# amathislab/HOISDF

Hardware: AMD Instinct MI355X
Metric: samples/sec (img + 2048 SDF queries) fwd+bwd at 1/2/4/8 MI355X (higher is better)
Workload: dtype f32 (emulated contractions, f32 accumulate, f16x2 form: operands as scaled hi + lo f16 pieces x 3 products - 22 operand bits, one power-of-two scale per ROW of a linear layer's row operand, per (sample, head) of the attention operands, per weight matrix; the attention backward's dS as three pieces x

## Files before the change

hoisdf_amd/_lib.py:

```python
from __future__ import annotations

import ctypes as C
import os
from typing import Dict, List

_HERE = os.path.dirname(os.path.abspath(__file__))
LIB_PATH = os.environ.get("HOISDF_LIB", os.path.join(_HERE, "libhoisdf_hip.so"))
HEADER_PATH = os.path.join(os.path.dirname(_HERE), "include", "hoisdf.h")
MAX_LEVELS = 8


class HoisdfLibraryError(RuntimeError):
    pass


class HoisdfError(RuntimeError):
    def __init__(self, code: int, msg: str):
        super().__init__(f"libhoisdf_hip status {code}: {msg}")
        self.code = code


class Pyramid(C.Structure):
    _fields_ = [("n_levels", C.c_int), ("B", C.c_int), ("data", C.c_void_p * MAX_LEVELS),
                ("C", C.c_int * MAX_LEVELS), ("H", C.c_int * MAX_LEVELS), ("W", C.c_int * MAX_LEVELS)]
# ... 56 lines not shown
class Mlp(C.Structure):
    _fields_ = [("n_layers", C.c_int), ("act_last", C.c_int), ("dims", C.c_int * (MLP_MAX_LAYERS + 1)),
                ("w", C.c_void_p * MLP_MAX_LAYERS), ("b", C.c_void_p * MLP_MAX_LAYERS),
                ("img", C.c_void_p * MLP_MAX_LAYERS), ("img_t", C.c_void_p * MLP_MAX_LAYERS)]


class EmuPrepItem(C.Structure):
    _fields_ = [("W", C.c_void_p), ("image", C.c_void_p), ("first_block", C.c_long), ("ldw", C.c_int), ("N", C.c_int),
                ("K", C.c_int), ("transpose", C.c_int)]


class MlpGrads(C.Structure):
    _fields_ = [("dw", C.c_void_p * MLP_MAX_LAYERS), ("db", C.c_void_p * MLP_MAX_LAYERS)]


POSE_MAX_LAYERS = 12


class PoseDesc(C.Structure):
    _fields_ = [("B", C.c_int), ("num_samp_hand", C.c_int), ("num_samp_obj", C.c_int), ("bins_n", C.c_int), ("img_h", C.c_int),
                ("img_w", C.c_int), ("hand_sdf_scale", C.c_float), ("obj_sdf_scale", C.c_float), ("clamping_distance", C.c_float),
                ("hidden_dim", C.c_int), ("nheads", C.c_int), ("dim_feedforward", C.c_int), ("enc_layers", C.c_int),
                ("dec_layers", C.c_int), ("C", C.c_int), ("use_inverse_kinematics", C.c_int), ("pre_norm", C.c_int),
                ("classifier_branch", C.c_int), ("attention", C.c_int)]


class SdfDecoderParams(C.Structure):
    _fields_ = [("weight_v", C.c_void_p * 4), ("weight_g", C.c_void_p * 4), ("bias", C.c_void_p * 4),
                ("linh4_weight", C.c_void_p), ("linh4_bias", C.c_void_p)]


class PoseWeights(C.Structure):
    _fields_ = [("linear_sdfin", Mlp), ("hand_sdf_decoder", SdfDecoderParams), ("obj_sdf_decoder", SdfDecoderParams),
                ("linear_transformerin", Mlp), ("hand_sigmoid_beta", C.c_void_p), ("obj_sigmoid_beta", C.c_void_p),
                ("hand_encoder", EncoderLayerWeights * POSE_MAX_LAYERS), ("obj_encoder", EncoderLayerWeights * POSE_MAX_LAYERS),
                ("hand_decoder", DecoderLayerWeights * POSE_MAX_LAYERS), ("mano_query_embed", C.c_void_p),
                ("linear_pose", Mlp), ("linear_shape", Mlp), ("linear_handvote", Mlp), ("linear_handcls", Mlp),
                ("linear_obj_rot", Mlp), ("linear_obj_rel_trans", Mlp),
                ("mano_shapedirs", C.c_void_p), ("mano_posedirs", C.c_void_p), ("mano_weights", C.c_void_p),
                ("mano_v_template", C.c_void_p), ("mano_j_regressor", C.c_void_p), ("mano_hands_mean", C.c_void_p)]


class EncoderDesc(C.Structure):
    _fields_ = [("B", C.c_int), ("img_h", C.c_int), ("img_w", C.c_int), ("resnet_type", C.c_int), ("big_decoder", C.c_int)]


_POSE_OUT = ("hand_joints_out", "obj_rot_out", "obj_trans_out", "mano_mesh_out", "mano_joints_out", "mano_shape_out",
             "hand_points_out", "obj_points_out", "hand_sdf_out", "obj_sdf_out")


class PoseOutputs(C.Structure):
    _fields_ = [(n, C.c_void_p) for n in _POSE_OUT]


_P, _I, _L, _F, _U64, _D = C.c_void_p, C.c_int, C.c_long, C.c_float, C.c_uint64, C.c_double
_PYR = C.POINTER(Pyramid)
_SDFW = C.POINTER(SdfWeights)

SIGNATURES: Dict[str, List] = {
    "hoisdf_project_gather_fwd": [_PYR, _P, _P, _L, _I, _P, _P, _F, _I, _I, _P, _I, _P, _P, _P],
    "hoisdf_project_gather_bwd": [_PYR, _P, _P, _L, _I, _P, _P, _F, _I, _I, _P, _I, _P],
    "hoisdf_linear_fwd": [_P, _I, _P, _I, _P, _P, _I, _L, _I, _I, _I, _F, _U64, _P, _P],
    "hoisdf_linear_bwd_input": [_P, _I, _P, _F, _P, _I, _P, _I, _L, _I, _I, _I, _P],
    "hoisdf_linear_bwd_weight": [_P, _I, _P, _F, _P, _I, _P, _I, _P, _L, _I, _I, _P, _L, _P],
    "hoisdf_linear_emu_prepare": [_P, _I, _I, _I, _I, _P, _P],
    "hoisdf_linear_emu_prepare_batch": [_P, _I, _L, _P],
    "hoisdf_linear_fwd_emu": [_P, _I, _P, _P, _P, _I, _L, _I, _I, _I, _F, _U64, _P, _P],
    "hoisdf_mag_measure": [_P, _L, _L, _I, _P, _P],
    "hoisdf_head_mag_measure": [_P, _L, _L, _I, _I, _P, _P],
    "hoisdf_linear_fwd_emu_heads": [_P, _I, _P, _P, _P, _I, _L, _I, _I, _P, _P, _P, _I, _P],
    "hoisdf_linear_bwd_input_emu_heads": [_P, _I, _P, _P, _I, _L, _I, _I, _P, _P, _P, _I, _P],
    "hoisdf_linear_fwd_emu_mag": [_P, _I, _P, _P, _P, _I, _L, _I, _I, _I, _F, _U64, _P, _P, _P, _P],
    "hoisdf_linear_bwd_input_emu": [_P, _I, _P, _F, _P, _P, _I, _L, _I, _I, _I, _P],
    "hoisdf_linear_bwd_input_emu_mag": [_P, _I, _P, _F, _P, _P, _I, _L, _I, _I, _I, _P, _P, _P],
    "hoisdf_linear_fwd_emu_small": [_P, _I, _P, _I, _P, _P, _I, _L, _I, _I, _I, _F, _U64, _P, _P],
    "hoisdf_linear_bwd_input_emu_small": [_P, _I, _P, _F, _P, _I, _P, _I, _L, _I, _I, _I, _P],
    "hoisdf_linear_bwd_weight_emu_small": [_P, _I, _P, _F, _P, _I, _P, _I, _P, _L, _I, _I, _P],
    "hoisdf_linear_bwd_weight_emu": [_P, _I, _P, _F, _P, _I, _P, _I, _P, _L, _I, _I, _P, _L, _P],
    "hoisdf_linear_bwd_weight_emu_mag": [_P, _I, _P, _F, _P, _I, _P, _I, _P, _L, _I, _I, _P, _L, _P, _P, _P],
    "hoisdf_relu_dropout_bwd": [_P, _I, _P, _I, _P, _I, _L, _I, _F, _P],
    "hoisdf_posenc_fwd": [_P, _L, _P, _I, _I, _P, _P],
    "hoisdf_sdf_query_fwd": [_PYR, _P, _P, _L, _I, _P, _P, _F, _I, _I, _P, _P, _SDFW, _F, _F, _U64, _P, _P, _P, _P, _P, _L, _P],
    "hoisdf_weightnorm_fwd": [_P, _P, _P, _I, _P, _I, _I, _P],
    "hoisdf_weightnorm_bwd": [_P, _P, _P, _I, _P, _P, _I, _I, _P],
    "hoisdf_sdf_head_fwd": [_P, _I, _P, _P, _P, _P, _L, _I, _F, _P],
    "hoisdf_sdf_head_bwd": [_P, _P, _P, _I, _P, _P, _I, _P, _P, _L, _I, _F, _P],
    "hoisdf_lattice_count": [_P, _P, _P, _F, _I, _I, _P, _P],
    "hoisdf_lattice_fill": [_P, _P, _P, _F, _I, _I, _P, _P, _P, _P, _P],
    "hoisdf_select_smallest_abs": [_P, _P, _P, _I, _I, _P, _P],
    "hoisdf_gather_rows": [_P, _I, _P, _L, _I, _P, _I, _P],
    "hoisdf_sdf_sample_keys": [_P, _I, _P, _P, _P, _P, _I, _I, _F, _U64, _P, _P, _P],
    "hoisdf_adamw_step": [_P, _I, _D, _D, _D, _D, _D, _L, _F, _P],
    "hoisdf_aux_image_losses_fwd": [_P, _L, _L, _L, _L, _P, _P, _P, _I, _I, _I, _I, _F, _P, _P, _P, _P, _P],
    "hoisdf_aux_image_losses_bwd": [_P, _L, _L, _L, _L, _P, _P, _P, _P, _P, _P, _I, _I, _I, _P, _P],
    "hoisdf_bn_stats": [_P, _L, _L, _I, _P, _P, _P, _P, _F, _F, _P, _L, _P],
    "hoisdf_bn_apply_fwd": [_P, _L, _P, _L, _P, _P, _I, _F, _P, _P, _I, _P, _P, _L, _I, _P],
    "hoisdf_bn_bwd": [_P, _L, _P, _L, _P, _P, _P, _P, _P, _P, _P, _P, _L, _I, _P, _L, _P],
    "hoisdf_token_build_fwd": [_P, _P, _P, _P, _I, _P, _P, _P, _I, _I, _I, _I, _I, _P],
    "hoisdf_token_build_bwd": [_P, _P, _I, _P, _P, _P, _I, _P, _I, _I, _I, _I, _I, _P],
    "hoisdf_token_build_bwd_ordered": [_P, _P, _I, _P, _P, _P, _I, _P, _P, _I, _I, _I, _I, _I, _P],
    "hoisdf_attention_fwd": [_P, _I, _P, _I, _P, _I, _P, _I, _P, _I, _I, _I, _I, _I, _F, _U64, _P],
    "hoisdf_attention_bwd": [_P, _I, _P, _I, _P, _I, _P, _I, _P, _I, _P, _P, _P, _P, _P, _I, _I, _I, _I,
                             _I, _F, _U64, _P],
    "hoisdf_attention_fwd_bf16x2": [_P, _I, _P, _I, _P, _I, _P, _I, _I, _I, _I, _I, _I, _P, _L, _P],
    "hoisdf_attention_fwd_emu": [_P, _I, _P, _I, _P, _I, _P, _I, _P, _I, _I, _I, _I, _I, _F, _U64, _P, _L, _I, _P],
    "hoisdf_attention_fwd_emu_mag": [_P, _I, _P, _I, _P, _I, _P, _I, _P, _I, _I, _I, _I, _I, _F, _U64, _P, _L, _I, _P, _P, _P, _P, _P],
    "hoisdf_attention_bwd_emu": [_P, _I, _P, _I, _P, _I, _P, _I, _P, _I, _P, _P, _P, _P, _P, _I, _I, _I, _I, _I, _F, _U64, _P, _P,
                                 _L, _P],
    "hoisdf_attention_bwd_emu_mag": [_P, _I, _P, _I, _P, _I, _P, _I, _P, _I, _P, _P, _P, _P, _P, _I, _I, _I, _I, _I, _F, _U64, _P, _P,
                                 _L, _P, _P, _P, _P, _P, _P],
    "hoisdf_attention_small_fwd": [_P, _I, _P, _I, _P, _I, _P, _P, _I, _P, _I, _I, _I, _I, _F, _U64, _P],
    "hoisdf_attention_small_bwd": [_P, _I, _P, _I, _P, _I, _P, _P, _I, _P, _P, _P, _I, _I, _I, _I, _F,
                                   _U64, _P],
    "hoisdf_add_layernorm_fwd": [_P, _P, _P, _P, _P, _P, _P, _L, _I, _F, _F, _U64, _P],
    "hoisdf_add_layernorm_bwd": [_P, _P, _P, _P, _P, _P, _P, _P, _P, _P, _P, _L, _I, _F, _U64, _P],
    "hoisdf_residual_dropout": [_P, _P, _P, _L, _I, _F, _U64, _P],
    "hoisdf_layernorm_rows_fwd": [_P, _P, _P, _P, _P, _P, _L, _I, _I, _I, _F, _P],
    "hoisdf_layernorm_rows_bwd": [_P, _P, _P, _P, _P, _P, _P, _P, _P, _L, _I, _I, _I, _P],
    "hoisdf_sdf_query_train_fwd": [_PYR, _P, _P, _L, _I, _P, _P, _F, _I, _I, _SDFW, _F, _F, _U64, _P, _P, _P, _P, _L, _P, _L, _P],
    "hoisdf_sdf_query_bwd": [_PYR, _P, _P, _L, _I, _P, _P, _F, _I, _I, _SDFW, _F, _F, _P, _L, _P, _P, _P, _L, _P],
    "hoisdf_sdf_infer_count": [_P, _P, _P, _F, _I, _I, _P, _P, _P, _P],
    "hoisdf_sdf_infer_count_begin": [_P, _P, _P, _F, _I, _I, _P, _P, _P],
    "hoisdf_sdf_infer": [_PYR, _P, _P, _P, _F, _I, _I, _P, _P, _I, _I, _I, _SDFW, _F, _F, _U64, _P, _P, _P, _P, _L, _P],
    "hoisdf_decoder_layer_fwd": [_P, _P, _P, _P, _P, _P, _P, _P, _P, _L, _P, _L, _P],
    "hoisdf_decoder_layer_bwd": [_P, _P, _P, _P, _P, _P, _P, _L, _P, _P, _P, _P, _I, _P, _P, _P, _L, _P],
    "hoisdf_encoder_layer_fwd": [_P, _P, _P, _P, _P, _P, _L, _P, _L, _P],
    "hoisdf_encoder_layer_bwd": [_P, _P, _P, _P, _P, _L, _P, _P, _P, _P, _P, _L, _P],
    "hoisdf_mano_prepare": [_P, _P, _P, _P, _P],
    "hoisdf_mano_head_fwd": [_P, _I, _I, _P, _I, _I, _P, _P, _P, _P, _P, _P, _P, _P, _P, _I, _I, _P, _P, _P, _P, _P],
    "hoisdf_mano_head_bwd": [_P, _P, _I, _P, _P, _P, _P, _P, _P, _P, _P, _P, _I, _I, _P, _P, _P, _P, _P, _P, _P],
    "hoisdf_vote_fwd": [_P, _P, _P, _P, _P, _I, _I, _I, _I, _P],
    "hoisdf_vote_bwd": [_P, _P, _P, _P, _P, _P, _P, _P, _I, _I, _I, _I, _P],
    "hoisdf_vote_loss_fwd": [_P, _P, _P, _P, _F, _P, _P, _P, _P, _P, _I, _I, _I, _I, _P],
    "hoisdf_vote_loss_bwd": [_P, _P, _P, _P, _F, _P, _P, _P, _P, _P, _P, _P, _I, _I, _I, _I, _P],
    "hoisdf_tokens_fwd": [_P, _P, _P, _P, _F, _I, _I, _P, _P, _P, _P, _P, _P, _P, _P, _P, _I, _I, _I, _I, _I, _P, _L, _P, _L, _P],
    "hoisdf_tokens_bwd": [_P, _P, _P, _P, _F, _I, _I, _P, _P, _P, _P, _P, _P, _L, _P, _P, _I, _P, _I, _I, _I, _I, _I, _P, _L, _P],
    "hoisdf_heads_vote_fwd": [_P, _P, _P, _P, _P, _F, _P, _P, _P, _P, _I, _I, _I, _I, _P, _L, _P, _L, _P],
    "hoisdf_heads_vote_bwd": [_P, _P, _P, _P, _P, _F, _P, _P, _L, _P, _P, _P, _P, _P, _P, _I, _I, _I, _I, _P, _L, _P],
    "hoisdf_point_loss_fwd": [_P, _P, _L, _L, _I, _L, _I, _F, _F, _F, _P, _P, _P],
    "hoisdf_point_loss_bwd": [_P, _P, _L, _L, _I, _L, _I, _F, _F, _F, _P, _P, _P],
    "hoisdf_pose_prepare": [_P, _P, _P, _L, _P],
    "hoisdf_pose_infer_begin": [_P, _P, _P, _P, _P, _P, _P, _P, _P],
    "hoisdf_pose_infer": [_P, _P, _PYR, _P, _P, _P, _P, _P, _P, _P, _P, _P, _L, _P, _P],
    "hoisdf_conv_pack_weight": [_P, _P, _P, _P, _P, _P, _F, _I, _I, _I, _I, _I, _P, _P, _P],
    "hoisdf_conv_plan": [_L, _I, _I, _I, _P, _P],
    "hoisdf_conv2d_fwd": [_P, _I, _P, _P, _P, _I, _P, _I, _I, _I, _I, _I, _I, _I, _I, _I, _I, _I, _I, _P, _L, _P],
    "hoisdf_conv_transpose2d_fwd": [_P, _I, _P, _P, _P, _I, _I, _I, _I, _I, _I, _I, _I, _P, _L, _P],
    "hoisdf_maxpool2d_fwd": [_P, _I, _P, _I, _I, _I, _I, _I, _P],
    "hoisdf_encoder_prepare": [_P, _P, _I, _P, _L, _P],
    "hoisdf_encoder_pyramid_shape": [_P, _PYR],
    "hoisdf_encoder_infer": [_P, _P, _P, _P, _P, _P, _L, _P],
}
_RET = {"hoisdf_version": C.c_char_p, "hoisdf_last_error": C.c_char_p}
_OTHER = {"hoisdf_set_deterministic": ([_I], None), "hoisdf_set_gemm_emu": ([_I], None), "hoisdf_get_gemm_emu": ([], C.c_int), "hoisdf_get_deterministic": ([], C.c_int),
          "hoisdf_mano_dirs_image_floats": ([], C.c_long),
          "hoisdf_point_loss_blocks": ([_L], C.c_int),
          "hoisdf_bn_workspace_floats": ([_L, _I], C.c_long),
          "hoisdf_token_build_bwd_partials": ([], C.c_int),
          "hoisdf_tokens_saved_bytes": ([_P, _L, _I], C.c_long),
          "hoisdf_tokens_workspace_bytes": ([_P, _L, _I], C.c_long),
          "hoisdf_heads_vote_saved_bytes": ([_P, _P, _I, _I, _I, _I], C.c_long),
          "hoisdf_heads_vote_workspace_bytes": ([_P, _P, _I, _I, _I, _I, _I], C.c_long),
          "hoisdf_sdf_infer_workspace": ([_L, _I, _I], C.c_long),
          "hoisdf_sdf_query_train_saved_bytes": ([_L, _I], C.c_long),
          "hoisdf_sdf_query_train_workspace_bytes": ([_L, _I, _I], C.c_long),
          "hoisdf_decoder_layer_saved_bytes": ([_P], C.c_long),
          "hoisdf_decoder_layer_workspace_bytes": ([_P, _I], C.c_long),
          "hoisdf_encoder_layer_saved_bytes": ([_P], C.c_long),
          "hoisdf_encoder_layer_out_mag": ([_P, _P], C.c_void_p),
          "hoisdf_encoder_layer_workspace_bytes": ([_P, _I], C.c_long),
          "hoisdf_sdf_query_workspace": ([_L, _I, _I], C.c_long),
          "hoisdf_linear_bwd_weight_workspace": ([_L, _I, _I], C.c_long),
          "hoisdf_linear_emu_image_bytes": ([_I, _I], C.c_long),
          "hoisdf_linear_emu_prepare_blocks": ([_I, _I, _I], C.c_long),
          "hoisdf_linear_bwd_weight_emu_workspace": ([_L, _I, _I], C.c_long),
          "hoisdf_linear_emu_supported": ([_P, _L, _I], C.c_int),
          "hoisdf_linear_emu_small_max_rows": ([], C.c_int),
          "hoisdf_linear_emu_pieces": ([], C.c_int),
          "hoisdf_mag_words": ([_L], C.c_long),
          "hoisdf_head_mag_words": ([_L, _I, _I], C.c_long),
          "hoisdf_linear_emu_small_supported": ([_P, _L, _P, _L, _L, _I, _I], C.c_int),
          "hoisdf_attention_bf16x2_workspace": ([_I, _I, _I, _I], C.c_long),
          "hoisdf_attention_emu_workspace": ([_I, _I, _I, _I, _I], C.c_long),
          "hoisdf_attention_bwd_emu_workspace": ([_I, _I, _I, _I, _I], C.c_long),
          "hoisdf_conv_packed_floats": ([_I, _I, _I, _I], C.c_long),
          "hoisdf_conv_workspace_bytes": ([_L, _I, _I, _I], C.c_long),
          "hoisdf_encoder_tensor_count": ([_P], C.c_int),
          "hoisdf_encoder_tensor_name": ([_P, _I], C.c_char_p),
          "hoisdf_encoder_tensor_numel": ([_P, _I], C.c_long),
          "hoisdf_encoder_prepared_bytes": ([_P], C.c_long),
          "hoisdf_encoder_infer_workspace": ([_P], C.c_long),
          "hoisdf_encoder_launch_count": ([_P], C.c_int),
          "hoisdf_pose_prepared_bytes": ([_P], C.c_long),
          "hoisdf_pose_infer_workspace": ([_P, _P], C.c_long)}

_lib = None


def lib() -> C.CDLL:
    global _lib
    if _lib is None:
        if not os.path.exists(LIB_PATH):
            raise HoisdfLibraryError(
                f"{LIB_PATH} not found: the HIP extension is not built (make -C hoisdf_amd/csrc). "
                "There is no CPU fallback for the hot path.")
        L = C.CDLL(LIB_PATH)
        for name, args in SIGNATURES.items():
            fn = getattr(L, name)
            fn.argtypes = args
            fn.restype = C.c_int
        for name, ret in _RET.items():
            fn = getattr(L, name)
            fn.argtypes = []
            fn.restype = ret
        for name, (args, ret) in _OTHER.items():
            fn = getattr(L, name)
            fn.argtypes = args
            fn.restype = ret
        _lib = L
    return _lib


_timer = None


def set_timer(timer) -> None:
    global _timer
    _timer = timer


def call(name: str, *args) -> None:
    t = _timer
    timed = t is not None and name in t.names
    if timed:
        t.begin(name, args)
    rc = getattr(lib(), name)(*args)
    if timed:
        t.end(name)
    if rc != 0:
        raise HoisdfError(rc, lib().hoisdf_last_error().decode())


def exported_symbols() -> List[str]:
    return list(SIGNATURES) + list(_RET) + list(_OTHER)
```

hoisdf_amd/csrc/attention_emu.h:

```cpp
#pragma once
#include "common.h"

namespace hoisdf {
namespace emu_attn {

struct EmuAttn {
  const __bf16 *q[3];
  const __bf16 *k[3];
  const __bf16 *v[3], *vt[3];
  const __bf16 *d[3];
  const float* lse_in; const float* delta;
  float* out; float* lse; float* dq_part; float* dk; float* dv;
  int ldo, ldk, ldv;
  int B, H, Lq, Lk, Lqp, Lkp, kv_len;
  float drop_p, inv_keep;
  uint32_t thresh;
  uint64_t seed;
  const uint32_t *q_hm, *k_hm, *v_hm, *d_hm;
  float* dq_scale;
  uint32_t* mag;
};

__device__ __forceinline__ bool emu_block(int nx, int nbh, int& tile, int& bh) {
  const int L = blockIdx.x, slot = L >> 3;
  bh = (slot / nx) * 8 + (L & 7);
  tile = slot % nx;
  return bh < nbh;
}

}

int attention_bwd4_emu_launch(const emu_attn::EmuAttn& a, hipStream_t st);
int attention_bwd4h_emu_launch(const emu_attn::EmuAttn& a, hipStream_t st);
}
```

hoisdf_amd/csrc/attention_emu.hip:

```cpp
#include <stdlib.h>

#include "attention_emu.h"

namespace hoisdf {
using emu_attn::EmuAttn;
using emu_attn::emu_block;

namespace {
typedef float f32x16 __attribute__((ext_vector_type(16)));
typedef float f32x4 __attribute__((ext_vector_type(4)));
typedef __bf16 bf16x8 __attribute__((ext_vector_type(8)));
typedef __bf16 bf16x4 __attribute__((ext_vector_type(4)));
typedef unsigned int u32x4 __attribute__((ext_vector_type(4)));
typedef unsigned int u32x2 __attribute__((ext_vector_type(2)));

constexpr int D = 64;
constexpr int RP = 72;
constexpr int TPH = 36;
constexpr int ROWS_T = 32 * RP;
constexpr int TRN_T = 64 * TPH;
constexpr float QS2 = 0.125f * 1.4426950408889634f;
#define CR(r, h) (((r) & 3) + 8 * ((r) >> 2) + 4 * (h))
#define MB(a, b, c) __builtin_amdgcn_mfma_f32_32x32x16_bf16((a), (b), (c), 0, 0, 0)
#define MB6(acc, x0, x1, x2, y0, y1, y2) \
  do {                                   \
    acc = MB(x2, y0, acc);               \
    acc = MB(x0, y2, acc);               \
    acc = MB(x1, y1, acc);               \
    acc = MB(x1, y0, acc);               \
    acc = MB(x0, y1, acc);               \
    acc = MB(x0, y0, acc);               \
  } while (0)

#define SPLIT1(x, i)                             \
  do {                                           \
    const __bf16 a_ = (__bf16)(x);               \
    const float r1_ = (x) - (float)a_;           \
    const __bf16 b_ = (__bf16)r1_;               \
    const float r2_ = r1_ - (float)b_;           \
    p0[i] = a_; p1[i] = b_; p2[i] = (__bf16)r2_; \
  } while (0)

__device__ __forceinline__ u32x4 ld_rows(const __bf16* base, size_t row0, int tid) {
  return *reinterpret_cast<const u32x4*>(base + (row0 + (tid >> 3)) * D + (tid & 7) * 8);
}
__device__ __forceinline__ void st_rows(__bf16* lds, const u32x4 v, int tid) {
  *reinterpret_cast<u32x4*>(lds + (tid >> 3) * RP + (tid & 7) * 8) = v;
}
__device__ __forceinline__ u32x4 ld_trn(const __bf16* base, size_t Lp, size_t col0, int tid) {
  return *reinterpret_cast<const u32x4*>(base + (size_t)(tid >> 2) * Lp + col0 + (tid & 3) * 8);
}
__device__ __forceinline__ void st_trn(__bf16* lds, const u32x4 v, int tid) {
  u32x2* p = reinterpret_cast<u32x2*>(lds + (tid >> 2) * TPH + (tid & 3) * 8);
  p[0] = u32x2{v.x, v.y};
  p[1] = u32x2{v.z, v.w};
}
__device__ __forceinline__ bf16x8 frag_trn(const __bf16* tile, int row, int jj, int h) {
  const bf16x4 a = *reinterpret_cast<const bf16x4*>(tile + row * TPH + 16 * jj + 4 * h);
  const bf16x4 b = *reinterpret_cast<const bf16x4*>(tile + row * TPH + 16 * jj + 8 + 4 * h);
  return bf16x8{a[0], a[1], a[2], a[3], b[0], b[1], b[2], b[3]};
}
}

typedef _Float16 f16x8 __attribute__((ext_vector_type(8)));
typedef _Float16 f16x2 __attribute__((ext_vector_type(2)));
template <bool F16>
__global__ __launch_bounds__(256) void emu_attn_convert_kernel(const float* __restrict__ src, int ld, int L, int Lp, int B, int H,
                                                               float scale, __bf16* __restrict__ r0, __bf16* __restrict__ r1,
                                                               __bf16* __restrict__ r2, __bf16* __restrict__ t0,
                                                               __bf16* __restrict__ t1, __bf16* __restrict__ t2,
                                                               const uint32_t* __restrict__ mag) {
  constexpr int TP = 72;
  __shared__ __attribute__((aligned(16))) __bf16 tile[3][64 * TP];
  const int tid = threadIdx.x;
  const int nb = Lp / 64;
  const int kb = blockIdx.x % nb, bh = blockIdx.x / nb, b = bh / H, head = bh - b * H;
  if (F16) { f16_saturate_on(); scale *= mag_scale(mag[head * B + b]); }
  const int r = tid >> 2, dc = (tid & 3) * 16;
  const int row = kb * 64 + r;
  const bool valid = row < L;
  const float* sr = src + ((size_t)b * L + (valid ? row : 0)) * ld + head * D + dc;
  bf16x8 pa[2][3];
#pragma unroll
  for (int i = 0; i < 2; ++i) {
    float4 u = valid ? *reinterpret_cast<const float4*>(sr + 8 * i) : make_float4(0.f, 0.f, 0.f, 0.f);
    float4 w = valid ? *reinterpret_cast<const float4*>(sr + 8 * i + 4) : make_float4(0.f, 0.f, 0.f, 0.f);
    u.x *= scale; u.y *= scale; u.z *= scale; u.w *= scale;
    w.x *= scale; w.y *= scale; w.z *= scale; w.w *= scale;
    if (F16) {
      const float e_[8] = {u.x, u.y, u.z, u.w, w.x, w.y, w.z, w.w};
      f16x8 hi, lo;
#pragma unroll
      for (int j = 0; j < 8; ++j) { hi[j] = (_Float16)e_[j]; lo[j] = (_Float16)(e_[j] - (float)hi[j]); }
      pa[i][0] = __builtin_bit_cast(bf16x8, hi); pa[i][1] = __builtin_bit_cast(bf16x8, lo); pa[i][2] = pa[i][1];
    } else {
      bf16x8 p0, p1, p2;
      SPLIT1(u.x, 0); SPLIT1(u.y, 1); SPLIT1(u.z, 2); SPLIT1(u.w, 3);
      SPLIT1(w.x, 4); SPLIT1(w.y, 5); SPLIT1(w.z, 6); SPLIT1(w.w, 7);
      pa[i][0] = p0; pa[i][1] = p1; pa[i][2] = p2;
    }
  }
  if (r0) {
    const size_t o = ((size_t)bh * Lp + row) * D + dc;
#pragma unroll
    for (int i = 0; i < 2; ++i) {
      *reinterpret_cast<bf16x8*>(r0 + o + 8 * i) = pa[i][0];
      *reinterpret_cast<bf16x8*>(r1 + o + 8 * i) = pa[i][1];
      if (!F16 && r2) *reinterpret_cast<bf16x8*>(r2 + o + 8 * i) = pa[i][2];
    }
  }
  if (t0) {
#pragma unroll
    for (int i = 0; i < 2; ++i)
#pragma unroll
      for (int e = 0; e < 8; ++e) {
        tile[0][(dc + 8 * i + e) * TP + r] = pa[i][0][e];
        tile[1][(dc + 8 * i + e) * TP + r] = pa[i][1][e];
        if (!F16) tile[2][(dc + 8 * i + e) * TP + r] = pa[i][2][e];
      }
    __syncthreads();
    const int d = tid >> 2, rc = (tid & 3) * 16;
    const size_t o = ((size_t)bh * D + d) * Lp + kb * 64 + rc;
#pragma unroll
    for (int i = 0; i < 2; ++i) {
      *reinterpret_cast<u32x4*>(t0 + o + 8 * i) = *reinterpret_cast<const u32x4*>(&tile[0][d * TP + rc + 8 * i]);
      *reinterpret_cast<u32x4*>(t1 + o + 8 * i) = *reinterpret_cast<const u32x4*>(&tile[1][d * TP + rc + 8 * i]);
      if (!F16 && t2) *reinterpret_cast<u32x4*>(t2 + o + 8 * i) = *reinterpret_cast<const u32x4*>(&tile[2][d * TP + rc + 8 * i]);
    }
  }
}

typedef float f32x2 __attribute__((ext_vector_type(2)));
typedef __bf16 bf16x2 __attribute__((ext_vector_type(2)));
template <bool DROP, int NPL, bool F16>
__global__ __launch_bounds__(256, 2) void emu_attn_fwd2_kernel(EmuAttn a) {
  static_assert(!F16 || NPL == 2, "the f16 form has two planes");
  __shared__ __attribute__((aligned(16))) __bf16 Kb0[3 * ROWS_T];
  __shared__ __attribute__((aligned(16))) __bf16 Kb1[3 * ROWS_T];
  __shared__ __attribute__((aligned(16))) __bf16 Vb0[3 * TRN_T];
  __shared__ __attribute__((aligned(16))) __bf16 Vb1[3 * TRN_T];
  const int tid = threadIdx.x, lane = tid & 63, wave = tid >> 6;
  const int h = lane >> 5, c = lane & 31;
  int qtile, bh;
  if (!emu_block((a.Lq + 127) / 128, a.B * a.H, qtile, bh)) return;
  const int b = bh / a.H, head = bh - b * a.H;
  const int qrow = qtile * 128 + wave * 32 + c;
  const __bf16* kp[3] = {a.k[0] + (size_t)bh * a.Lkp * D, a.k[1] + (size_t)bh * a.Lkp * D, a.k[NPL == 3 ? 2 : 1] + (size_t)bh * a.Lkp * D};
  const __bf16* vp[3] = {a.vt[0] + (size_t)bh * D * a.Lkp, a.vt[1] + (size_t)bh * D * a.Lkp, a.vt[NPL == 3 ? 2 : 1] + (size_t)bh * D * a.Lkp};
  float cs = 1.f, vinv = 1.f;
  constexpr float PB = F16 ? 6.f : 0.f;
  if (F16) {
    f16_saturate_on();
    const float iq_ = mag_inv_scale(a.q_hm[head * a.B + b]), ik_ = mag_inv_scale(a.k_hm[head * a.B + b]);
    cs = fmaxf(iq_ * ik_, 0x1p-100f); vinv = mag_inv_scale(a.v_hm[head * a.B + b]);
  }
  const float thr8 = F16 ? 8.f / cs : 8.f;
  float mneg = INFINITY;

  bf16x8 qf[4][3];
#pragma unroll
  for (int p = 0; p < NPL; ++p) {
    const __bf16* sq = a.q[p] + ((size_t)bh * a.Lqp + qrow) * D;
#pragma unroll
    for (int j = 0; j < 4; ++j) qf[j][p] = *reinterpret_cast<const bf16x8*>(sq + 16 * j + 8 * h);
  }
  const uint32_t rowkey = drop_rowkey(a.seed, (uint32_t)(bh * a.Lq + qrow));
  const uint32_t dthr = a.thresh & 0xffff0000u;
  float m = -INFINITY, lsum = 0.f, ps = 0.f;
  f32x16 o[2], s_cur, s_nxt;
  float dsc[16];
#pragma unroll
  for (int t = 0; t < 2; ++t)
#pragma unroll
    for (int r = 0; r < 16; ++r) o[t][r] = 0.f;
#pragma unroll
  for (int r = 0; r < 16; ++r) dsc[r] = 1.f;
  const int ntiles = (a.kv_len + 31) / 32;
  const int lastt = ntiles - 1;
  u32x4 rk[3], rv[3];
  bf16x8 kf[2][3], vf[2][3], pw[2][3];
  uint32_t w0[8], w1[8], w2[8], hx[8];
  f32x2 e_[8], f_[8];
  float mt = -INFINITY;
#define KFRAG(KB, p, j) (*reinterpret_cast<const bf16x8*>(&(KB)[(p) * ROWS_T + c * RP + 16 * (j) + 8 * h]))
#define VFRAG(VB, p, dt, jj) frag_trn((VB) + (p) * TRN_T, (dt) * 32 + c, jj, h)
#define SB() __builtin_amdgcn_sched_barrier(0)
#define PK_SUB(d, x, y) asm("v_pk_add_f32 %0, %1, %2 neg_lo:[0,1] neg_hi:[0,1]" : "=v"(d) : "v"(x), "v"(y))
#define PE1(pr)                                                                                                        \
  do {                                                                                                                 \
    if constexpr (F16) e_[pr] = f32x2{__builtin_amdgcn_exp2f(__builtin_fmaf(s_cur[2 * (pr)], cs, mneg)),               \
                                     __builtin_amdgcn_exp2f(__builtin_fmaf(s_cur[2 * (pr) + 1], cs, mneg))};           \
    else e_[pr] = f32x2{__builtin_amdgcn_exp2f(s_cur[2 * (pr)] - m), __builtin_amdgcn_exp2f(s_cur[2 * (pr) + 1] - m)}; \
  } while (0)
#define PE2(pr)                                                                                                        \
  do {                                                                                                                 \
    ps += e_[pr].x + e_[pr].y;                                                                                         \
    if (DROP) e_[pr] = f32x2{e_[pr].x * dsc[2 * (pr)], e_[pr].y * dsc[2 * (pr) + 1]};                                   \
    if constexpr (F16) {                                                                                               \
      const f16x2 hh_ = __builtin_convertvector(e_[pr], f16x2);                                                        \
      w0[pr] = __builtin_bit_cast(uint32_t, hh_);                                                                      \
      f_[pr] = __builtin_convertvector(hh_, f32x2);                                                                    \
    } else {                                                                                                           \
      const uint32_t h_ = __builtin_bit_cast(uint32_t, __builtin_convertvector(e_[pr], bf16x2));                       \
      w0[pr] = h_;                                                                                                     \
      f_[pr] = f32x2{__builtin_bit_cast(float, h_ << 16), __builtin_bit_cast(float, h_ & 0xffff0000u)};                \
    }                                                                                                                  \
  } while (0)
#define PE3(pr)                                                                                                        \
  do {                                                                                                                 \
    PK_SUB(e_[pr], e_[pr], f_[pr]);                                                                                    \
    const uint32_t h_ = __builtin_bit_cast(uint32_t, __builtin_convertvector(e_[pr], bf16x2));                         \
    w1[pr] = h_;                                                                                                       \
    f_[pr] = f32x2{__builtin_bit_cast(float, h_ << 16), __builtin_bit_cast(float, h_ & 0xffff0000u)};                  \
  } while (0)
#define PE4(pr)                                                                                                        \
  do {                                                                                                                 \
    f32x2 r_; PK_SUB(r_, e_[pr], f_[pr]);                                                                              \
    w2[pr] = __builtin_bit_cast(uint32_t, __builtin_convertvector(r_, bf16x2));                                        \
    if (((pr) & 3) == 3) {                                      \
      pw[(pr) >> 2][0] = __builtin_bit_cast(bf16x8, u32x4{w0[(pr) - 3], w0[(pr) - 2], w0[(pr) - 1], w0[pr]});          \
      pw[(pr) >> 2][1] = __builtin_bit_cast(bf16x8, u32x4{w1[(pr) - 3], w1[(pr) - 2], w1[(pr) - 1], w1[pr]});          \
      pw[(pr) >> 2][2] = __builtin_bit_cast(bf16x8, u32x4{w2[(pr) - 3], w2[(pr) - 2], w2[(pr) - 1], w2[pr]});          \
    }                                                                                                                  \
  } while (0)
#define PE3B(pr)                                                                                                       \
  do {                                                                                                                 \
    f32x2 r_; PK_SUB(r_, e_[pr], f_[pr]);                                                                              \
    if constexpr (F16) w1[pr] = __builtin_bit_cast(uint32_t, __builtin_convertvector(r_, f16x2));                      \
    else w1[pr] = __builtin_bit_cast(uint32_t, __builtin_convertvector(r_, bf16x2));                                   \
    if (((pr) & 3) == 3) {                                                                                             \
      pw[(pr) >> 2][0] = __builtin_bit_cast(bf16x8, u32x4{w0[(pr) - 3], w0[(pr) - 2], w0[(pr) - 1], w0[pr]});          \
      pw[(pr) >> 2][1] = __builtin_bit_cast(bf16x8, u32x4{w1[(pr) - 3], w1[(pr) - 2], w1[(pr) - 1], w1[pr]});          \
    }                                                                                                                  \
  } while (0)
#define PM(i)                                                                                                          \
  do {                                                                                                                 \
    float t_;                                                                                                          \
    asm volatile("v_max3_f32 %0, %1, %2, %3" : "=v"(t_) : "v"(s_nxt[4 * (i)]), "v"(s_nxt[4 * (i) + 1]), "v"(s_nxt[4 * (i) + 2])); \
    asm volatile("v_max3_f32 %0, %0, %1, %2" : "+v"(mt) : "v"(t_), "v"(s_nxt[4 * (i) + 3]));                           \
  } while (0)
#define PH1(pr) do { if (DROP) { uint32_t x_ = hbase + (uint32_t)(CR(2 * (pr), 0) >> 1) * 0x9E3779B9U; x_ ^= x_ >> 15; hx[pr] = x_ * 0x2C1B3C6DU; asm volatile("" : "+v"(hx[pr])); } } while (0)
#define PH2(pr) do { if (DROP) { hx[pr] ^= hx[pr] >> 12; asm volatile("" : "+v"(hx[pr])); } } while (0)
#define PH3(pr) do { if (DROP) { dsc[2 * (pr)] = (hx[pr] << 16) >= dthr ? a.inv_keep : 0.f; dsc[2 * (pr) + 1] = hx[pr] >= dthr ? a.inv_keep : 0.f; asm volatile("" : "+v"(dsc[2 * (pr)]), "+v"(dsc[2 * (pr) + 1])); } } while (0)
#define STK(p) st_rows(kw + (p) * ROWS_T, rk[p], tid)
#define STV(p) st_trn(vw + (p) * TRN_T, rv[p], tid)
#define LDK(p) rk[p] = ld_rows(kp[p], (size_t)ktn * 32, tid)
#define LDV(p) rv[p] = ld_trn(vp[p], a.Lkp, (size_t)vtn * 32, tid)
#ifndef FWD2_ABL
#define FWD2_ABL 0
#endif
#if FWD2_ABL & 1
#undef PE1
#undef PE2
#undef PE3
#undef PE4
#undef PE3B
#undef PM
#undef PH1
#undef PH2
#undef PH3
#define PE1(pr) ((void)0)
#define PE2(pr) ((void)0)
#define PE3(pr) ((void)0)
#define PE4(pr) ((void)0)
#define PE3B(pr) ((void)0)
#define PM(i) ((void)0)
#define PH1(pr) ((void)0)
#define PH2(pr) ((void)0)
#define PH3(pr) ((void)0)
#endif
#if FWD2_ABL & 8
#undef PE1
#define PE1(pr) do { e_[pr] = f32x2{s_cur[2 * (pr)], s_cur[2 * (pr) + 1]}; } while (0)
#endif
#if FWD2_ABL & 16
#undef PE2
#undef PE3
#undef PE4
#define PE2(pr) do { ps += e_[pr].x + e_[pr].y; w0[pr] = __builtin_bit_cast(uint32_t, e_[pr].x); } while (0)
#define PE3(pr) do { w1[pr] = __builtin_bit_cast(uint32_t, e_[pr].y); } while (0)
#define PE4(pr)                                                                                                        \
  do {                                                                                                                 \
    w2[pr] = w0[pr] ^ w1[pr];                                                                                          \
    if (((pr) & 3) == 3) {                                                                                             \
      pw[(pr) >> 2][0] = __builtin_bit_cast(bf16x8, u32x4{w0[(pr) - 3], w0[(pr) - 2], w0[(pr) - 1], w0[pr]});          \
      pw[(pr) >> 2][1] = __builtin_bit_cast(bf16x8, u32x4{w1[(pr) - 3], w1[(pr) - 2], w1[(pr) - 1], w1[pr]});          \
      pw[(pr) >> 2][2] = __builtin_bit_cast(bf16x8, u32x4{w2[(pr) - 3], w2[(pr) - 2], w2[(pr) - 1], w2[pr]});          \
    }                                                                                                                  \
  } while (0)
#endif
#if FWD2_ABL & 32
#undef PM
#define PM(i) ((void)0)
#endif
#if FWD2_ABL & 2
#undef STK
#undef STV
#undef LDK
#undef LDV
#define STK(p) ((void)0)
#define STV(p) ((void)0)
#define LDK(p) ((void)0)
#define LDV(p) ((void)0)
#endif
#if FWD2_ABL & 4
#define FWD2_SYNC() ((void)0)
#else
#define FWD2_SYNC() __syncthreads()
#endif
#pragma push_macro("MB")
#undef MB
#define MB(a_, b_, c_)                                                                                                             \
  (F16 ? __builtin_amdgcn_mfma_f32_32x32x16_f16(__builtin_bit_cast(f16x8, (a_)), __builtin_bit_cast(f16x8, (b_)), (c_), 0, 0, 0) \
       : __builtin_amdgcn_mfma_f32_32x32x16_bf16((a_), (b_), (c_), 0, 0, 0))
#include "attn_fwd2_phase.inc"

#pragma unroll
  for (int p = 0; p < NPL; ++p) { rk[p] = ld_rows(kp[p], 0, tid); rv[p] = ld_trn(vp[p], a.Lkp, 0, tid); }
#pragma unroll
  for (int p = 0; p < NPL; ++p) { st_rows(Kb0 + p * ROWS_T, rk[p], tid); st_trn(Vb0 + p * TRN_T, rv[p], tid); }
#pragma unroll
  for (int p = 0; p < NPL; ++p) rk[p] = ld_rows(kp[p], (size_t)min(1, lastt) * 32, tid);
#pragma unroll
  for (int p = 0; p < NPL; ++p) st_rows(Kb1 + p * ROWS_T, rk[p], tid);
#pragma unroll
  for (int p = 0; p < NPL; ++p) { rk[p] = ld_rows(kp[p], (size_t)min(2, lastt) * 32, tid); rv[p] = ld_trn(vp[p], a.Lkp, (size_t)min(1, lastt) * 32, tid); }
  __syncthreads();
#pragma unroll
  for (int r = 0; r < 16; ++r) s_nxt[r] = 0.f;
#pragma unroll
  for (int j = 0; j < 4; ++j) {
    const bf16x8 k0 = KFRAG(Kb0, 0, j), k1 = KFRAG(Kb0, 1, j);
    if constexpr (NPL == 3) {
      const bf16x8 k2 = KFRAG(Kb0, 2, j);
      MB6(s_nxt, k0, k1, k2, qf[j][0], qf[j][1], qf[j][2]);
    } else {
      s_nxt = MB(k1, qf[j][0], s_nxt); s_nxt = MB(k0, qf[j][1], s_nxt); s_nxt = MB(k0, qf[j][0], s_nxt);
    }
  }
  uint32_t hbase = rowkey + (uint32_t)(2 * h) * 0x9E3779B9U;
#define FWD2_TILE_STATS(KT, DO_HASH)                                                                                   \
  do {                                                                                                                 \
    if ((KT) == lastt) {                                                                                               \
      _Pragma("unroll") for (int r = 0; r < 16; ++r) if ((KT) * 32 + CR(r, h) >= a.kv_len) s_nxt[r] = -INFINITY;       \
      mt = -INFINITY;                                                                                                  \
      PM(0); PM(1); PM(2); PM(3);                                                                                      \
    }                                                                                                                  \
    mt = fmaxf(mt, __shfl_xor(mt, 32, 64));                                                                            \
    if (__any(mt > m + thr8)) {                                                                                        \
      const float mn = fmaxf(m, mt);                                                                                   \
      const float alpha = __builtin_amdgcn_exp2f(F16 ? (m - mn) * cs : m - mn);                                        \
      lsum *= alpha;                                                                                                   \
      m = mn;                                                                                                          \
      mneg = PB - m * cs;                                                                                              \
      _Pragma("unroll") for (int t_ = 0; t_ < 2; ++t_) _Pragma("unroll") for (int r = 0; r < 16; ++r) o[t_][r] *= alpha; \
    }                                                                                                                  \
    if (DO_HASH) { _Pragma("unroll") for (int pr = 0; pr < 8; ++pr) { PH1(pr); PH2(pr); PH3(pr); } }                    \
  } while (0)
#pragma unroll
  for (int r = 0; r < 16; ++r) mt = fmaxf(mt, s_nxt[r]);
  FWD2_TILE_STATS(0, true);
  s_cur = s_nxt;
  __syncthreads();
#define FWD2_ITER(t, KR, KW, VR, VW)                                                                                   \
  do {                                                                                                                 \
    __bf16* kw = (KW); __bf16* vw = (VW);                                                                              \
    const int ktn = min((t) + 3, lastt), vtn = min((t) + 2, lastt);                                                    \
    kf[0][0] = KFRAG(KR, 0, 0); kf[0][1] = KFRAG(KR, 1, 0); if constexpr (NPL == 3) kf[0][2] = KFRAG(KR, 2, 0);        \
    _Pragma("unroll") for (int r = 0; r < 16; ++r) s_nxt[r] = 0.f;                                                     \
    ps = 0.f;                                                                                                          \
    SB();                                                                                                              \
    if constexpr (NPL == 3) FWD2_S(KR); else FWD2_S2(KR);                                                              \
    lsum += ps;                                                                                                        \
    vf[0][0] = VFRAG(VR, 0, 0, 0); vf[0][1] = VFRAG(VR, 1, 0, 0); if constexpr (NPL == 3) vf[0][2] = VFRAG(VR, 2, 0, 0); \
    mt = -INFINITY;                                                                                                    \
    hbase += 16u * 0x9E3779B9U;                                                                                        \
    SB();                                                                                                              \
    if constexpr (NPL == 3) FWD2_PV(VR); else FWD2_PV2(VR);                                                            \
    if ((t) + 1 <= lastt) FWD2_TILE_STATS((t) + 1, false);                \
    s_cur = s_nxt;                                                                                                     \
    FWD2_SYNC();                                                                                                       \
  } while (0)
  int t = 0;
  for (; t + 1 < ntiles; t += 2) {
    FWD2_ITER(t, Kb1, Kb0, Vb0, Vb1);
    FWD2_ITER(t + 1, Kb0, Kb1, Vb1, Vb0);
  }
  if (t < ntiles) FWD2_ITER(t, Kb1, Kb0, Vb0, Vb1);
#undef KFRAG
#undef VFRAG
#undef SB
#undef PK_SUB
#undef PE1
#undef PE2
#undef PE3
#undef PE4
#undef PM
#undef PH1
#undef PH2
#undef PH3
#undef STK
#undef STV
#undef LDK
#undef LDV
#undef FWD2_S
#undef FWD2_PV
#undef FWD2_S2
#undef FWD2_PV2
#undef PE3B
#undef FWD2_TILE_STATS
#undef FWD2_ITER
  const float ltot = lsum + __shfl_xor(lsum, 32, 64);
  uint32_t omax = 0u;
  if (qrow < a.Lq) {
    const float inv = vinv / ltot;
    float* op = a.out + ((size_t)b * a.Lq + qrow) * a.ldo + head * D;
#pragma unroll
    for (int tt = 0; tt < 2; ++tt)
#pragma unroll
      for (int g = 0; g < 4; ++g) {
        const float4 ov = make_float4(o[tt][4 * g + 0] * inv, o[tt][4 * g + 1] * inv, o[tt][4 * g + 2] * inv, o[tt][4 * g + 3] * inv);
        *reinterpret_cast<float4*>(op + 32 * tt + 8 * g + 4 * h) = ov;
        omax = max(omax, mag_bits4(ov));
      }
    if (h == 0 && a.lse) a.lse[(size_t)bh * a.Lq + qrow] = (F16 ? m * cs - PB : m) + log2f(ltot);
  }
  if (a.mag) {
    omax = max(omax, (uint32_t)__shfl_xor((int)omax, 32, 64));
    if (h == 0 && qrow < a.Lq) atomicMax(a.mag + (size_t)b * a.Lq + qrow, omax);
  }
}
#pragma pop_macro("MB")

__global__ __launch_bounds__(256) void emu_attn_delta_kernel(const float* __restrict__ o, int ldo, const float* __restrict__ dout,
                                                             int lddo, float* __restrict__ delta, int B, int H, int Lq) {
  const long g = ((long)blockIdx.x * 256 + threadIdx.x) >> 4;
  const int l16 = threadIdx.x & 15;
  if (g >= (long)B * Lq * H) return;
  const int head = (int)(g % H);
  const long bq = g / H;
  const int q = (int)(bq % Lq), b = (int)(bq / Lq);
  const float4 x = *reinterpret_cast<const float4*>(o + ((size_t)b * Lq + q) * ldo + head * D + l16 * 4);
  const float4 y = *reinterpret_cast<const float4*>(dout + ((size_t)b * Lq + q) * lddo + head * D + l16 * 4);
  float s = x.x * y.x + x.y * y.y + x.z * y.z + x.w * y.w;
#pragma unroll
  for (int off = 8; off > 0; off >>= 1) s += __shfl_xor(s, off, 16);
  if (l16 == 0) delta[((size_t)b * H + head) * Lq + q] = s;
}

__global__ __launch_bounds__(256) void emu_attn_dq_reduce_kernel(const float* __restrict__ part, int nkb, float* __restrict__ dq,
                                                                 int ldq, int B, int H, int Lq, uint32_t* __restrict__ mag,
                                                                 const float* __restrict__ scale) {
  const long i = (long)(gridDim.x - 1 - blockIdx.x) * 256 + threadIdx.x;
  const long n = (long)B * H * Lq * 16;
  uint32_t qmax = 0u;
  if (i < n) {
    const int d4 = (int)(i & 15);
    const long bq = i >> 4;
    const int q = (int)(bq % Lq);
    const int bh = (int)(bq / Lq), b = bh / H, head = bh - b * H;
    const size_t stride = (size_t)B * H * Lq * D;
    const float* p = part + ((size_t)bh * Lq + q) * D + d4 * 4;
    float4 s = *reinterpret_cast<const float4*>(p);
    for (int k0 = 1; k0 < nkb; k0 += 8) {
      f32x4 v[8];
#pragma unroll
      for (int j = 0; j < 8; ++j)
        v[j] = k0 + j < nkb ? __builtin_nontemporal_load(reinterpret_cast<const f32x4*>(p + (size_t)(k0 + j) * stride)) : f32x4{0.f, 0.f, 0.f, 0.f};
#pragma unroll
      for (int j = 0; j < 8; ++j)
        if (k0 + j < nkb) { s.x += v[j].x; s.y += v[j].y; s.z += v[j].z; s.w += v[j].w; }
    }
    const float sc = scale ? scale[bh] : 0.125f;
    const float4 r = make_float4(s.x * sc, s.y * sc, s.z * sc, s.w * sc);
    *reinterpret_cast<float4*>(dq + ((size_t)b * Lq + q) * ldq + head * D + d4 * 4) = r;
    qmax = mag_bits4(r);
    if (mag) {
      qmax = group_max_u32<16>(qmax);
      if (d4 == 0) atomicMax(mag + (size_t)b * Lq + q, qmax);
    }
  }
}

}

using namespace hoisdf;

namespace {
inline long pad128(long L) { return (L + 127) / 128 * 128; }
inline size_t plane_elems(int B, int H, long Lp) { return (size_t)B * H * Lp * 64; }

struct Planes { __bf16 *r[3], *t[3]; };
inline Planes carve(__bf16*& w, size_t n, bool rows, bool trn) {
  Planes p{};
  for (int i = 0; i < 3; ++i) { p.r[i] = rows ? w : nullptr; if (rows) w += n; }
  for (int i = 0; i < 3; ++i) { p.t[i] = trn ? w : nullptr; if (trn) w += n; }
  return p;
}
int convert(const float* src, int ld, int L, int Lp, int B, int H, float scale, const Planes& p, hipStream_t st, const uint32_t* mag = nullptr) {
  const long nblk = (long)B * H * (Lp / 64);
  if (mag) hipLaunchKernelGGL(emu_attn_convert_kernel<true>, dim3((unsigned)nblk), dim3(256), 0, st, src, ld, L, Lp, B, H, scale, p.r[0], p.r[1],
                              p.r[2], p.t[0], p.t[1], p.t[2], mag);
  else hipLaunchKernelGGL(emu_attn_convert_kernel<false>, dim3((unsigned)nblk), dim3(256), 0, st, src, ld, L, Lp, B, H, scale, p.r[0], p.r[1],
                          p.r[2], p.t[0], p.t[1], p.t[2], mag);
  return check_launch("attention_emu_convert");
}
int check_emu(const void* q, const void* k, const void* v, int ldq, int ldk, int ldv, int B, int H, int Lq, int Lk, int kv_len,
              float drop_p, const char* who) {
  HOISDF_REQUIRE(q && k && v, HOISDF_ERR_INVALID, "%s: null pointer", who);
  HOISDF_REQUIRE(B > 0 && H > 0 && Lq > 0 && Lk > 0 && kv_len > 0 && kv_len <= Lk, HOISDF_ERR_INVALID,
                 "%s: bad sizes B=%d H=%d Lq=%d Lk=%d kv_len=%d", who, B, H, Lq, Lk, kv_len);
  HOISDF_REQUIRE(ldq >= H * 64 && ldk >= H * 64 && ldv >= H * 64 && ((ldq | ldk | ldv) & 3) == 0 &&
                     (((uintptr_t)q | (uintptr_t)k | (uintptr_t)v) & 15) == 0,
                 HOISDF_ERR_INVALID, "%s: leading dims must be multiples of 4 and >= H*64, pointers 16-byte aligned", who);
  HOISDF_REQUIRE(drop_p >= 0.f && drop_p < 1.f, HOISDF_ERR_INVALID, "%s: drop_p=%f", who, drop_p);
  return HOISDF_OK;
}
}

extern "C" long hoisdf_attention_emu_workspace(int B, int H, int Lq, int Lk, int mode) {
  if (B <= 0 || H <= 0 || Lq <= 0 || Lk <= 0) return 0;
  const size_t q = plane_elems(B, H, pad128(Lq)), k = plane_elems(B, H, pad128(Lk));
  const size_t planes = mode == 0 ? 3 * q + 6 * k : 3 * q + 9 * k;
  return (long)(planes * sizeof(__bf16));
}

namespace {
int fwd_over_planes(float* o, int ldo, float* lse, int B, int H, int Lq, int Lk, int kv_len, float drop_p, uint64_t seed,
                    void* workspace, int keep, hipStream_t st, uint32_t* o_mag, const uint32_t* q_hm = nullptr, const uint32_t* k_hm = nullptr,
                    const uint32_t* v_hm = nullptr) {
  const int Lqp = (int)pad128(Lq), Lkp = (int)pad128(Lk);
  __bf16* w = reinterpret_cast<__bf16*>(workspace);
  const size_t nq = plane_elems(B, H, Lqp), nk = plane_elems(B, H, Lkp);
  const Planes pq = carve(w, nq, true, false);
  const Planes pk = carve(w, nk, true, false);
  const Planes pv = carve(w, nk, keep != 0, true);
  EmuAttn a{};
  for (int i = 0; i < 3; ++i) { a.q[i] = pq.r[i]; a.k[i] = pk.r[i]; a.vt[i] = pv.t[i]; }
  a.out = o; a.lse = lse; a.ldo = ldo; a.mag = o_mag; a.q_hm = q_hm; a.k_hm = k_hm; a.v_hm = v_hm;
  a.B = B; a.H = H; a.Lq = Lq; a.Lk = Lk; a.Lqp = Lqp; a.Lkp = Lkp; a.kv_len = kv_len;
  a.drop_p = drop_p; a.inv_keep = 1.f / (1.f - drop_p); a.thresh = drop_threshold(drop_p); a.seed = seed;
  const dim3 fgrid(cdiv(Lq, 128) * 8 * cdiv(B * H, 8));
  if (q_hm) {
    HOISDF_REQUIRE(drop_p < 0.75f, HOISDF_ERR_INVALID, "attention_fwd_emu (f16x2 form): drop_p = %f, must be below 0.75", drop_p);
    if (drop_p > 0.f) hipLaunchKernelGGL((emu_attn_fwd2_kernel<true, 2, true>), fgrid, dim3(256), 0, st, a);
    else hipLaunchKernelGGL((emu_attn_fwd2_kernel<false, 2, true>), fgrid, dim3(256), 0, st, a);
  } else if (drop_p > 0.f) hipLaunchKernelGGL((emu_attn_fwd2_kernel<true, 3, false>), fgrid, dim3(256), 0, st, a);
  else hipLaunchKernelGGL((emu_attn_fwd2_kernel<false, 3, false>), fgrid, dim3(256), 0, st, a);
  return check_launch("attention_fwd_emu");
}
}

extern "C" int hoisdf_attention_fwd_emu(const float* q, int ldq, const float* k, int ldk, const float* v, int ldv, float* o,
                                        int ldo, float* lse, int B, int H, int Lq, int Lk, int kv_len, float drop_p,
                                        uint64_t seed, void* workspace, long workspace_bytes, int keep, void* stream) {
  return attention_fwd_emu_mag(q, ldq, k, ldk, v, ldv, o, ldo, lse, B, H, Lq, Lk, kv_len, drop_p, seed, workspace, workspace_bytes, keep,
                               nullptr, stream, nullptr, nullptr, nullptr);
}
extern "C" int hoisdf_attention_fwd_emu_mag(const float* q, int ldq, const float* k, int ldk, const float* v, int ldv, float* o,
                                            int ldo, float* lse, int B, int H, int Lq, int Lk, int kv_len, float drop_p,
                                            uint64_t seed, void* workspace, long workspace_bytes, int keep, const uint32_t* q_mag,
                                            const uint32_t* k_mag, const uint32_t* v_mag, uint32_t* o_mag, void* stream) {
  HOISDF_REQUIRE(q_mag && k_mag && v_mag, HOISDF_ERR_INVALID, "attention_fwd_emu_mag: the head magnitudes of q, k and v are required (hoisdf_head_mag_measure)");
  return attention_fwd_emu_mag(q, ldq, k, ldk, v, ldv, o, ldo, lse, B, H, Lq, Lk, kv_len, drop_p, seed, workspace, workspace_bytes, keep,
                               o_mag, stream, q_mag, k_mag, v_mag);
}
int hoisdf::attention_fwd_emu_mag(const float* q, int ldq, const float* k, int ldk, const float* v, int ldv, float* o, int ldo, float* lse,
                                  int B, int H, int Lq, int Lk, int kv_len, float drop_p, uint64_t seed, void* workspace,
                                  long workspace_bytes, int keep, uint32_t* o_mag, void* stream, const uint32_t* q_hm, const uint32_t* k_hm,
                                  const uint32_t* v_hm) {
  if (int rc = check_emu(q, k, v, ldq, ldk, ldv, B, H, Lq, Lk, kv_len, drop_p, "attention_fwd_emu")) return rc;
  HOISDF_REQUIRE(o && workspace && ldo >= H * 64 && (ldo & 3) == 0 && (((uintptr_t)o | (uintptr_t)workspace) & 15) == 0,
                 HOISDF_ERR_INVALID, "attention_fwd_emu: bad output / workspace");
  HOISDF_REQUIRE((!q_hm && !k_hm && !v_hm) || (q_hm && k_hm && v_hm), HOISDF_ERR_INVALID, "attention_fwd_emu: head magnitudes of all of q, k, v or of none");
  const long need = hoisdf_attention_emu_workspace(B, H, Lq, Lk, keep ? 2 : 0);
  HOISDF_REQUIRE(workspace_bytes >= need, HOISDF_ERR_WORKSPACE, "attention_fwd_emu: workspace %ld < %ld bytes", workspace_bytes, need);
  const int Lqp = (int)pad128(Lq), Lkp = (int)pad128(Lk);
  hipStream_t st = as_stream(stream);
  __bf16* w = reinterpret_cast<__bf16*>(workspace);
  const size_t nq = plane_elems(B, H, Lqp), nk = plane_elems(B, H, Lkp);
  const Planes pq = carve(w, nq, true, false);
  const Planes pk = carve(w, nk, true, false);
  const Planes pv = carve(w, nk, keep != 0, true);
  if (int rc = convert(q, ldq, Lq, Lqp, B, H, QS2, pq, st, q_hm)) return rc;
  if (int rc = convert(k, ldk, Lk, Lkp, B, H, 1.f, pk, st, k_hm)) return rc;
  if (int rc = convert(v, ldv, Lk, Lkp, B, H, 1.f, pv, st, v_hm)) return rc;
  return fwd_over_planes(o, ldo, lse, B, H, Lq, Lk, kv_len, drop_p, seed, workspace, keep, st, o_mag, q_hm, k_hm, v_hm);
}

extern "C" long hoisdf_attention_bf16x2_workspace(int B, int H, int Lq, int Lk) {
  if (B <= 0 || H <= 0 || Lq <= 0 || Lk <= 0) return 0;
  return (long)((2 * plane_elems(B, H, pad128(Lq)) + 4 * plane_elems(B, H, pad128(Lk))) * sizeof(__bf16));
}

extern "C" int hoisdf_attention_fwd_bf16x2(const float* q, int ldq, const float* k, int ldk, const float* v, int ldv, float* o, int ldo,
                                           int B, int H, int Lq, int Lk, int kv_len, void* workspace, long workspace_bytes, void* stream) {
  if (int rc = check_emu(q, k, v, ldq, ldk, ldv, B, H, Lq, Lk, kv_len, 0.f, "attention_fwd_bf16x2")) return rc;
  HOISDF_REQUIRE(o && workspace && ldo >= H * 64 && (ldo & 3) == 0 && (((uintptr_t)o | (uintptr_t)workspace) & 15) == 0,
                 HOISDF_ERR_INVALID, "attention_fwd_bf16x2: bad output / workspace");
  const long need = hoisdf_attention_bf16x2_workspace(B, H, Lq, Lk);
  HOISDF_REQUIRE(workspace_bytes >= need, HOISDF_ERR_WORKSPACE, "attention_fwd_bf16x2: workspace %ld < %ld bytes", workspace_bytes, need);
  const int Lqp = (int)pad128(Lq), Lkp = (int)pad128(Lk);
  hipStream_t st = as_stream(stream);
  __bf16* w = reinterpret_cast<__bf16*>(workspace);
  const size_t nq = plane_elems(B, H, Lqp), nk = plane_elems(B, H, Lkp);
  Planes pq{}, pk{}, pv{};
  pq.r[0] = w; pq.r[1] = w + nq; w += 2 * nq;
  pk.r[0] = w; pk.r[1] = w + nk; w += 2 * nk;
  pv.t[0] = w; pv.t[1] = w + nk;
  if (int rc = convert(q, ldq, Lq, Lqp, B, H, QS2, pq, st)) return rc;
  if (int rc = convert(k, ldk, Lk, Lkp, B, H, 1.f, pk, st)) return rc;
  if (int rc = convert(v, ldv, Lk, Lkp, B, H, 1.f, pv, st)) return rc;
  EmuAttn a{};
  for (int i = 0; i < 2; ++i) { a.q[i] = pq.r[i]; a.k[i] = pk.r[i]; a.vt[i] = pv.t[i]; }
  a.out = o; a.lse = nullptr; a.ldo = ldo;
  a.B = B; a.H = H; a.Lq = Lq; a.Lk = Lk; a.Lqp = Lqp; a.Lkp = Lkp; a.kv_len = kv_len;
  a.drop_p = 0.f; a.inv_keep = 1.f; a.thresh = 0; a.seed = 0;
  const dim3 fgrid(cdiv(Lq, 128) * 8 * cdiv(B * H, 8));
  hipLaunchKernelGGL((emu_attn_fwd2_kernel<false, 2, false>), fgrid, dim3(256), 0, st, a);
  return check_launch("attention_fwd_bf16x2");
}

void hoisdf::attention_emu_plane_targets(void* workspace, int B, int H, int Lq, int Lk, int keep, QkvPlanes& qp, QkvPlanes& kvp) {
  const int Lqp = (int)pad128(Lq), Lkp = (int)pad128(Lk);
  __bf16* w = reinterpret_cast<__bf16*>(workspace);
  const size_t nq = plane_elems(B, H, Lqp), nk = plane_elems(B, H, Lkp);
  const Planes pq = carve(w, nq, true, false);
  const Planes pk = carve(w, nk, true, false);
  const Planes pv = carve(w, nk, keep != 0, true);
  qp = QkvPlanes{}; kvp = QkvPlanes{};
  qp.on = kvp.on = 1; qp.H = kvp.H = H; qp.E = kvp.E = H * 64; qp.qscale = kvp.qscale = QS2;
  qp.L = Lq; qp.Lp = Lqp; kvp.L = Lk; kvp.Lp = Lkp;
  for (int i = 0; i < 3; ++i) {
    qp.r[0][i] = pq.r[i];
    kvp.r[1][i] = pk.r[i]; kvp.r[2][i] = pv.r[i]; kvp.vt[i] = pv.t[i];
    if (Lq == Lk) { kvp.r[0][i] = pq.r[i]; qp.r[1][i] = pk.r[i]; qp.r[2][i] = pv.r[i]; qp.vt[i] = pv.t[i]; }
  }
}

int hoisdf::attention_fwd_emu_planes(float* o, int ldo, float* lse, int B, int H, int Lq, int Lk, int kv_len, float drop_p,
                                     uint64_t seed, void* workspace, int keep, void* stream, uint32_t* o_mag) {
  HOISDF_REQUIRE(o && workspace && ldo >= H * 64 && (ldo & 3) == 0 && (((uintptr_t)o | (uintptr_t)workspace) & 15) == 0 && B > 0 &&
                     H > 0 && Lq > 0 && Lk > 0 && kv_len > 0 && kv_len <= Lk && drop_p >= 0.f && drop_p < 1.f,
                 HOISDF_ERR_INVALID, "attention_fwd_emu_planes: bad arguments");
  return fwd_over_planes(o, ldo, lse, B, H, Lq, Lk, kv_len, drop_p, seed, workspace, keep, as_stream(stream), o_mag);
}

extern "C" long hoisdf_attention_bwd_emu_workspace(int B, int H, int Lq, int Lk, int kept) {
  if (B <= 0 || H <= 0 || Lq <= 0 || Lk <= 0) return 0;
  const size_t q = plane_elems(B, H, pad128(Lq)), k = plane_elems(B, H, pad128(Lk));
  size_t bytes = 3 * q * sizeof(__bf16) + (size_t)cdiv(Lk, 128) * B * H * Lq * 64 * sizeof(float);
  if (!kept) bytes += (3 * q + 6 * k) * sizeof(__bf16);
  return (long)bytes;
}

extern "C" int hoisdf_attention_bwd_emu(const float* q, int ldq, const float* k, int ldk, const float* v, int ldv, const float* o,
                                        int ldo, const float* dout, int lddo, const float* lse, float* delta, float* dq, float* dk,
                                        float* dv, int B, int H, int Lq, int Lk, int kv_len, float drop_p, uint64_t seed,
                                        const void* fwd_workspace, void* workspace, long workspace_bytes, void* stream) {
  return attention_bwd_emu_mag(q, ldq, k, ldk, v, ldv, o, ldo, dout, lddo, lse, delta, dq, dk, dv, B, H, Lq, Lk, kv_len, drop_p, seed,
                               fwd_workspace, workspace, workspace_bytes, nullptr, stream, nullptr, nullptr, nullptr, nullptr);
}
extern "C" int hoisdf_attention_bwd_emu_mag(const float* q, int ldq, const float* k, int ldk, const float* v, int ldv, const float* o,
                                            int ldo, const float* dout, int lddo, const float* lse, float* delta, float* dq, float* dk,
                                            float* dv, int B, int H, int Lq, int Lk, int kv_len, float drop_p, uint64_t seed,
                                            const void* fwd_workspace, void* workspace, long workspace_bytes, const uint32_t* q_mag,
                                            const uint32_t* k_mag, const uint32_t* v_mag, const uint32_t* do_mag, uint32_t* g_mag, void* stream) {
  HOISDF_REQUIRE(q_mag && k_mag && v_mag && do_mag, HOISDF_ERR_INVALID, "attention_bwd_emu_mag: the head magnitudes of q, k, v and of dout are required");
  return attention_bwd_emu_mag(q, ldq, k, ldk, v, ldv, o, ldo, dout, lddo, lse, delta, dq, dk, dv, B, H, Lq, Lk, kv_len, drop_p, seed,
                               fwd_workspace, workspace, workspace_bytes, g_mag, stream, q_mag, k_mag, v_mag, do_mag);
}
int hoisdf::attention_bwd_emu_mag(const float* q, int ldq, const float* k, int ldk, const float* v, int ldv, const float* o, int ldo,
                                  const float* dout, int lddo, const float* lse, float* delta, float* dq, float* dk, float* dv, int B,
                                  int H, int Lq, int Lk, int kv_len, float drop_p, uint64_t seed, const void* fwd_workspace,
                                  void* workspace, long workspace_bytes, uint32_t* g_mag, void* stream, const uint32_t* q_hm,
                                  const uint32_t* k_hm, const uint32_t* v_hm, const uint32_t* do_hm) {
  const bool h2 = q_hm && k_hm && v_hm && do_hm;
  HOISDF_REQUIRE(h2 || (!q_hm && !k_hm && !v_hm && !do_hm), HOISDF_ERR_INVALID, "attention_bwd_emu: head magnitudes of all of q, k, v, dout or of none");
  HOISDF_REQUIRE(!g_mag || Lq == Lk, HOISDF_ERR_INVALID, "attention_bwd_emu: one row-magnitude array for dq, dk, dv needs Lq == Lk");
  HOISDF_REQUIRE(!h2 || drop_p < 0.75f, HOISDF_ERR_INVALID, "attention_bwd_emu (f16x2 form): drop_p = %f, must be below 0.75 (as in the forward)", drop_p);
  if (int rc = check_emu(fwd_workspace && !q ? o : q, fwd_workspace && !k ? o : k, fwd_workspace && !v ? o : v, ldq, ldk, ldv, B, H, Lq,
                         Lk, kv_len, drop_p, "attention_bwd_emu")) return rc;
  HOISDF_REQUIRE(o && dout && lse && delta && dq && dk && dv && workspace, HOISDF_ERR_INVALID, "attention_bwd_emu: null pointer");
  HOISDF_REQUIRE(ldo >= H * 64 && lddo >= H * 64 && ((ldo | lddo) & 3) == 0 &&
                     (((uintptr_t)o | (uintptr_t)dout | (uintptr_t)dq | (uintptr_t)dk | (uintptr_t)dv | (uintptr_t)workspace |
                       (uintptr_t)fwd_workspace) & 15) == 0,
                 HOISDF_ERR_INVALID, "attention_bwd_emu: bad leading dims / alignment");
  const long need = hoisdf_attention_bwd_emu_workspace(B, H, Lq, Lk, fwd_workspace ? 1 : 0);
  HOISDF_REQUIRE(workspace_bytes >= need, HOISDF_ERR_WORKSPACE, "attention_bwd_emu: workspace %ld < %ld bytes", workspace_bytes, need);
  const int Lqp = (int)pad128(Lq), Lkp = (int)pad128(Lk);
  hipStream_t st = as_stream(stream);
  const size_t nq = plane_elems(B, H, Lqp), nk = plane_elems(B, H, Lkp);
  __bf16* w = reinterpret_cast<__bf16*>(workspace);
  const Planes pd = carve(w, nq, true, false);
  float* part = reinterpret_cast<float*>(w);
  w += (size_t)cdiv(Lk, 128) * B * H * Lq * 64 * 2;
  Planes pq, pk, pv;
  if (fwd_workspace) {
    __bf16* f = reinterpret_cast<__bf16*>(const_cast<void*>(fwd_workspace));
    pq = carve(f, nq, true, false); pk = carve(f, nk, true, false); pv = carve(f, nk, true, true);
  } else {
    pq = carve(w, nq, true, false); pk = carve(w, nk, true, false); pv = carve(w, nk, true, false);
    if (int rc = convert(q, ldq, Lq, Lqp, B, H, QS2, pq, st, q_hm)) return rc;
    if (int rc = convert(k, ldk, Lk, Lkp, B, H, 1.f, pk, st, k_hm)) return rc;
    if (int rc = convert(v, ldv, Lk, Lkp, B, H, 1.f, pv, st, v_hm)) return rc;
  }
  if (int rc = convert(dout, lddo, Lq, Lqp, B, H, 1.f, pd, st, do_hm)) return rc;
  const long ng = (long)B * Lq * H;
  hipLaunchKernelGGL(emu_attn_delta_kernel, dim3((unsigned)((ng * 16 + 255) / 256)), dim3(256), 0, st, o, ldo, dout, lddo, delta, B, H, Lq);
  if (int rc = check_launch("attention_emu_delta")) return rc;
  EmuAttn a{};
  for (int i = 0; i < 3; ++i) {
    a.q[i] = pq.r[i]; a.k[i] = pk.r[i]; a.v[i] = pv.r[i]; a.d[i] = pd.r[i];
  }
  a.lse_in = lse; a.delta = delta; a.dq_part = part; a.dk = dk; a.dv = dv; a.ldk = ldk; a.ldv = ldv; a.mag = g_mag;
  a.B = B; a.H = H; a.Lq = Lq; a.Lk = Lk; a.Lqp = Lqp; a.Lkp = Lkp; a.kv_len = kv_len;
  a.drop_p = drop_p; a.inv_keep = 1.f / (1.f - drop_p); a.thresh = drop_threshold(drop_p); a.seed = seed;
  if (h2) {
    a.q_hm = q_hm; a.k_hm = k_hm; a.v_hm = v_hm; a.d_hm = do_hm;
    a.dq_scale = reinterpret_cast<float*>(pd.r[2]);
    if (int rc = attention_bwd4h_emu_launch(a, st)) return rc;
    const long n4h = (long)B * H * Lq * 16;
    hipLaunchKernelGGL(emu_attn_dq_reduce_kernel, dim3((unsigned)((n4h + 255) / 256)), dim3(256), 0, st, part, cdiv(kv_len, 128), dq, ldq,
                       B, H, Lq, g_mag, (const float*)a.dq_scale);
    return check_launch("attention_bwd_emu dq reduce");
  }
  if (int rc = attention_bwd4_emu_launch(a, st)) return rc;
  const long n4 = (long)B * H * Lq * 16;
  hipLaunchKernelGGL(emu_attn_dq_reduce_kernel, dim3((unsigned)((n4 + 255) / 256)), dim3(256), 0, st, part, cdiv(kv_len, 128), dq, ldq,
                     B, H, Lq, g_mag, (const float*)nullptr);
  return check_launch("attention_bwd_emu dq reduce");
}
```

hoisdf_amd/csrc/attention_emu_bwd4h.hip:

```cpp
#include <stdlib.h>

#include "attention_emu.h"

namespace hoisdf {
using emu_attn::EmuAttn;
using emu_attn::emu_block;

namespace {
typedef float f32x16 __attribute__((ext_vector_type(16)));
typedef float f32x4 __attribute__((ext_vector_type(4)));
typedef float f32x2 __attribute__((ext_vector_type(2)));
typedef __bf16 bf16x8 __attribute__((ext_vector_type(8)));
typedef __bf16 bf16x2 __attribute__((ext_vector_type(2)));
typedef unsigned int u32x4 __attribute__((ext_vector_type(4)));
typedef unsigned int u32x2 __attribute__((ext_vector_type(2)));
typedef short s16x4 __attribute__((ext_vector_type(4)));

constexpr int D = 64;
constexpr float LN2 = 0.6931471805599453f;
constexpr int QD_PLANE = 32 * 64;
constexpr int QD_BUF = 4 * QD_PLANE;
constexpr int TT_PLANE = 128 * 32;
constexpr int TT_BUF = 3 * TT_PLANE;
constexpr int X_BUF = 2 * 32 * 64;
constexpr int TT0 = 3 * QD_BUF;
constexpr int X0_BYTES = (3 * QD_BUF + 2 * TT_BUF) * 2;
constexpr int ST0_BYTES = X0_BYTES + 2 * X_BUF * 4;
constexpr unsigned B4H_LDS_BYTES = ST0_BYTES + 3 * 64 * 4;

#define SB() __builtin_amdgcn_sched_barrier(0)

__device__ __forceinline__ int qd_swz(int r) { return ((r >> 1) & 3) | ((((r >> 1) ^ (r >> 3)) & 1) << 2); }
__device__ __forceinline__ int qd_off(int r, int ch) { return r * 64 + ((ch ^ qd_swz(r)) << 3); }

__device__ __forceinline__ bf16x8 tr8(const __bf16* lo, const __bf16* hi) {
  const s16x4 x = __builtin_amdgcn_ds_read_tr16_b64_v4i16((s16x4 __attribute__((address_space(3)))*)(lo));
  const s16x4 y = __builtin_amdgcn_ds_read_tr16_b64_v4i16((s16x4 __attribute__((address_space(3)))*)(hi));
  return __builtin_bit_cast(bf16x8, __builtin_shufflevector(x, y, 0, 1, 2, 3, 4, 5, 6, 7));
}
typedef _Float16 f16x2 __attribute__((ext_vector_type(2)));
__device__ __forceinline__ uint32_t cvt2(f32x2 v) { return __builtin_bit_cast(uint32_t, __builtin_convertvector(v, f16x2)); }
__device__ __forceinline__ f32x2 unpack2(uint32_t w) { return __builtin_convertvector(__builtin_bit_cast(f16x2, w), f32x2); }
}

template <bool DROP>
__global__ __launch_bounds__(256, 1) void emu_attn_bwd4h_kernel(EmuAttn a) {
  extern __shared__ __attribute__((aligned(16))) __bf16 lds[];
  float* const xbuf = reinterpret_cast<float*>(reinterpret_cast<char*>(lds) + X0_BYTES);
  float* const stats = reinterpret_cast<float*>(reinterpret_cast<char*>(lds) + ST0_BYTES);
  const int tid = threadIdx.x, lane = tid & 63, wave = tid >> 6;
  const int c = lane & 31, h = lane >> 5, jq = lane & 15, b1 = (jq >> 3) & 1;
  int ktile, bh;
  const int nkb = (a.Lk + 127) / 128;
  if (!emu_block(nkb, a.B * a.H, ktile, bh)) return;
  const int b = bh / a.H, head = bh - b * a.H;
  const int key = ktile * 128 + wave * 32 + c;
  const bool kvalid = key < a.kv_len;
  const int nq = ktile * 128 < a.kv_len ? (a.Lq + 31) / 32 : 0;
  const int dhalf = wave & 1, khalf = wave >> 1;
  f16_saturate_on();
  const int hw_ = head * a.B + b;
  const uint32_t aq_ = a.q_hm[hw_], ak_ = a.k_hm[hw_], av_ = a.v_hm[hw_], ad_ = a.d_hm[hw_];
  const float iq = mag_inv_scale(aq_), ik = mag_inv_scale(ak_), iv = mag_inv_scale(av_), id = mag_inv_scale(ad_);
  const float cs = fmaxf(iq * ik, 0x1p-100f);
  constexpr float PBIAS = 13.f;
  constexpr float K1 = 0x1p-36f;
  const float k2a = mag_scale(ad_) * 0x1p-18f, k2b = mag_scale(av_) * 0x1p-18f;
  const float dk_scale = (LN2 * 0x1p23f * id) * (iv * iq);
  const float dv_scale = 0x1p-13f * id;
  if (ktile == 0 && tid == 0 && a.dq_scale) a.dq_scale[bh] = (0.125f * 0x1p23f * id) * (ik * iv);

  bf16x8 kf[4][2], vf[4][2], ktf[4][2];
  {
    const size_t ro = ((size_t)bh * a.Lkp + key) * D;
#pragma unroll
    for (int p = 0; p < 2; ++p)
#pragma unroll
      for (int j = 0; j < 4; ++j) {
        kf[j][p] = *reinterpret_cast<const bf16x8*>(a.k[p] + ro + 16 * j + 8 * h);
        vf[j][p] = *reinterpret_cast<const bf16x8*>(a.v[p] + ro + 16 * j + 8 * h);
      }
    const size_t ko = ((size_t)bh * a.Lkp + ktile * 128 + 64 * khalf + 8 * h) * D + 32 * dhalf + c;
#pragma unroll
    for (int p = 0; p < 2; ++p)
#pragma unroll
      for (int ks = 0; ks < 4; ++ks) {
        bf16x8 t;
#pragma unroll
        for (int i = 0; i < 8; ++i)
          t[i] = ktile * 128 + 64 * khalf + 16 * ks + 8 * h + i < a.kv_len ? a.k[p][ko + (size_t)(16 * ks + i) * D] : (__bf16)0.f;
        ktf[ks][p] = t;
      }
  }
#pragma unroll
  for (int p = 0; p < 2; ++p)
#pragma unroll
    for (int j = 0; j < 4; ++j) {
      asm volatile("" : "+a"(kf[j][p]));
      asm volatile("" : "+a"(vf[j][p]));
      asm volatile("" : "+a"(ktf[j][p]));
    }
  f32x16 dk[2], dv[2];
#pragma unroll
  for (int t = 0; t < 2; ++t)
#pragma unroll
    for (int r = 0; r < 16; ++r) { dk[t][r] = 0.f; dv[t][r] = 0.f; }

  const int fswz = qd_swz(c);
  int aoff[4];
#pragma unroll
  for (int j = 0; j < 4; ++j) aoff[j] = c * 64 + (((2 * j + h) ^ fswz) << 3);
  int trb[2];
  {
    const int low2 = ((((c >> 4) ^ h) & 1) << 1) | ((((jq >> 1) & 1) ^ b1) & 1);
#pragma unroll
    for (int e = 0; e < 2; ++e) trb[e] = (4 * h + (jq >> 2)) * 64 + ((e ^ b1) << 5) + (low2 << 3) + (jq & 1) * 4;
  }
  int tqb[2];
#pragma unroll
  for (int s2 = 0; s2 < 2; ++s2) {
    const int kr = 64 * khalf + 8 * h + 4 * s2 + (jq >> 2);
    tqb[s2] = kr * 32 + (((4 * (c >> 4) + (jq & 3)) ^ ((kr >> 1) & 7)) << 2);
  }
  const int tw0 = (32 * wave + c) * 32 + ((h ^ ((c >> 1) & 7)) << 2);
  const int xw0 = khalf * 2048 + c * 64 + (8 * dhalf << 2) + ((h ^ (c & 7)) << 2);
  const int xr0 = (8 * wave + (lane >> 4)) * 64 + (((lane & 15) ^ (lane >> 4)) << 2);
  const int xr1 = (xr0 + 256) ^ 16;
  const int st_o = qd_off(tid >> 3, tid & 7);

  u32x4 sg[4];
  float rstat = 0.f;
  const size_t rowbase = (size_t)bh * a.Lqp * D;
  const __bf16* const qb0 = a.q[0] + rowbase; const __bf16* const qb1 = a.q[1] + rowbase;
  const __bf16* const db0 = a.d[0] + rowbase; const __bf16* const db1 = a.d[1] + rowbase;
  unsigned goff = (unsigned)((tid >> 3) * D + (tid & 7) * 8);
  const float* const stat_src = (tid < 32 ? a.lse_in : a.delta) + (size_t)bh * a.Lq;
#define B4_LOADP(i_) do { sg[i_] = *reinterpret_cast<const u32x4*>(((i_) == 0 ? qb0 : (i_) == 1 ? qb1 : (i_) == 2 ? db0 : db1) + goff); } while (0)
#define B4_LOADS(QT_, GHOST_)                                                                                          \
  do {                                                                                                                 \
    if (tid < 64) {                                                                                                    \
      const int q_ = (QT_) * 32 + (tid & 31);                                                                          \
      rstat = (q_ < a.Lq && !(GHOST_)) ? stat_src[q_] : (tid < 32 ? INFINITY : 0.f);                                   \
    }                                                                                                                  \
  } while (0)
#define B4_STOREP(i_, BUF_) do { *reinterpret_cast<u32x4*>(lds + (BUF_) + (i_) * QD_PLANE + st_o) = sg[i_]; } while (0)
#define B4_STORES(SB_) do { if (tid < 64) stats[(SB_) + tid] = rstat; } while (0)

  float* const part = a.dq_part + ((size_t)ktile * a.B * a.H + bh) * a.Lq * D;
  if (nq > 0) {
#pragma unroll
    for (int pt = 0; pt < 2; ++pt) {
      const int qt = min(pt, nq - 1);
      goff = (unsigned)(qt * 32 * D + (tid >> 3) * D + (tid & 7) * 8);
#pragma unroll
      for (int i = 0; i < 4; ++i) B4_LOADP(i);
      B4_LOADS(qt, pt >= nq);
#pragma unroll
      for (int i = 0; i < 4; ++i) B4_STOREP(i, pt * QD_BUF);
      B4_STORES(pt * 64);
    }
    int qt_next = min(2, nq - 1);
    goff = (unsigned)(qt_next * 32 * D + (tid >> 3) * D + (tid & 7) * 8);
#pragma unroll
    for (int i = 0; i < 4; ++i) B4_LOADP(i);
    B4_LOADS(qt_next, 2 >= nq);
    __syncthreads();

    int qd_cur = 0, qd_nxt = QD_BUF, qd_fre = 2 * QD_BUF;
    int st_cur = 0, st_nxt = 64, st_fre = 128;
    int tt_w = TT0, tt_r = TT0 + TT_BUF;
    int x_a = 0, x_b = X_BUF;
    uint32_t hb = 0;
    const uint32_t dthr = a.thresh & 0xffff0000u;
    const int hsh = (key & 1) ? 0 : 16;
    const bool kodd = (key & 1) != 0;
    if (DROP) hb = drop_rowkey(a.seed, (uint32_t)(bh * a.Lq + 4 * h)) + (uint32_t)(key >> 1) * 0x9E3779B9U + (kodd ? 16u * 0x85EBCA77U : 0u);

    f32x16 s, dp, dq;
    f32x4 xo0[2], xo1[2];
    bf16x8 fr[2][2], ft[4][3];
    u32x4 pwv[2][2], gwv[3][2];
    f32x2 pe[8], pd[8], xx[8], ff[8];
    float dsc[16], lq[16], dl[16];
    uint32_t hy[8];
    float dmine[8], dsend[8];
#pragma unroll
    for (int r = 0; r < 16; ++r) dsc[r] = 1.f;
#pragma unroll
    for (int p = 0; p < 3; ++p)
#pragma unroll
      for (int i = 0; i < 2; ++i) { if (p < 2) pwv[p][i] = u32x4{0u, 0u, 0u, 0u}; gwv[p][i] = u32x4{0u, 0u, 0u, 0u}; }

#define MFMA_SP(acc_, a_, b_) asm volatile("v_mfma_f32_32x32x16_f16 %0, %1, %2, %0" : "+v"(acc_) : "v"(a_), "a"(b_))
#define MFMA_SP0(acc_, a_, b_) asm volatile("v_mfma_f32_32x32x16_f16 %0, %1, %2, 0" : "=&v"(acc_) : "v"(a_), "a"(b_))
#define MFMA_Q(acc_, a_, b_) asm volatile("v_mfma_f32_32x32x16_f16 %0, %1, %2, %0" : "+v"(acc_) : "a"(a_), "v"(b_))
#define MFMA_Q0(acc_, a_, b_) asm volatile("v_mfma_f32_32x32x16_f16 %0, %1, %2, 0" : "=&v"(acc_) : "a"(a_), "v"(b_))
#define MFMA_VK(acc_, a_, b_) asm volatile("v_mfma_f32_32x32x16_f16 %0, %1, %2, %0" : "+a"(acc_) : "v"(a_), "v"(b_))
#define FRQ(p_, j_) (*reinterpret_cast<const bf16x8*>(lds + qd_cur + aoff[j_] + (p_) * QD_PLANE))
#define FRD(p_, j_) (*reinterpret_cast<const bf16x8*>(lds + qd_cur + aoff[j_] + (2 + (p_)) * QD_PLANE))
#define FRQN(p_, j_) (*reinterpret_cast<const bf16x8*>(lds + qd_nxt + aoff[j_] + (p_) * QD_PLANE))
#define FRDN(p_, j_) (*reinterpret_cast<const bf16x8*>(lds + qd_nxt + aoff[j_] + (2 + (p_)) * QD_PLANE))
#define FRA(pl_, jj_, mt_) tr8(lds + qd_cur + trb[(mt_)] + (pl_) * QD_PLANE + (16 * (jj_)) * 64, \
                               lds + qd_cur + trb[(mt_) ^ 1] + (pl_) * QD_PLANE + (16 * (jj_) + 8) * 64)
#define FRT(p_, ks_) tr8(lds + tt_r + tqb[0] + (p_) * TT_PLANE + (16 * (ks_)) * 32, lds + tt_r + tqb[1] + (p_) * TT_PLANE + (16 * (ks_)) * 32)
#define PWF(p_, jj_) __builtin_bit_cast(bf16x8, pwv[p_][jj_])
#define GWF(p_, jj_) __builtin_bit_cast(bf16x8, gwv[p_][jj_])
#define PIN2(x_) asm volatile("" : "+v"(x_))
#define XOL(i_)                                                                                                        \
  do {                                                                                                                 \
    xo0[i_] = *reinterpret_cast<const f32x4*>(xbuf + x_a + ((i_) ? xr1 : xr0));                                        \
    xo1[i_] = *reinterpret_cast<const f32x4*>(xbuf + x_a + 2048 + ((i_) ? xr1 : xr0));                                 \
  } while (0)
#define XOS(i_)                                                                                                        \
  do {                                                                                                                 \
    const int q_ = (t - 2) * 32 + 8 * wave + 4 * (i_) + (lane >> 4);                                                   \
    if (t >= 2 && q_ < a.Lq) *reinterpret_cast<f32x4*>(part + (unsigned)(q_ * D + 4 * (lane & 15))) = xo0[i_] + xo1[i_]; \
  } while (0)
#define CRC(r_) (((r_) & 3) + 8 * ((r_) >> 2))
#define HA(q_) do { if (DROP) { _Pragma("unroll") for (int i_ = 0; i_ < 4; ++i_) { const int e_ = 4 * (q_) + i_; uint32_t x_ = hbn + (uint32_t)CRC(e_) * 0x85EBCA77U; x_ ^= x_ >> 15; hy[e_] = x_; PIN2(hy[e_]); } } } while (0)
#define HB(q_) do { if (DROP) { _Pragma("unroll") for (int i_ = 0; i_ < 4; ++i_) { const int e_ = 4 * (q_) + i_; hy[e_] *= 0x2C1B3C6DU; PIN2(hy[e_]); } } } while (0)
#define HC(q_)                                                                                                         \
  do {                                                                                                                 \
    if (DROP) {                                                                                                        \
      _Pragma("unroll") for (int i_ = 0; i_ < 4; ++i_) {                                                               \
        const int e_ = 4 * (q_) + i_;                                                                                  \
        const uint32_t x_ = hy[e_] ^ (hy[e_] >> 12);                                                                   \
        dmine[e_] = (x_ << hsh) >= dthr ? a.inv_keep : 0.f;                                                            \
        dsend[e_] = (x_ << (hsh ^ 16)) >= dthr ? a.inv_keep : 0.f;                                                     \
        PIN2(dmine[e_]); PIN2(dsend[e_]);                                                                              \
      }                                                                                                                \
    }                                                                                                                  \
  } while (0)
#define HD(q_)                                                                                                         \
  do {                                                                                                                 \
    if (DROP) {                                                                                                        \
      _Pragma("unroll") for (int i_ = 0; i_ < 4; ++i_) {                                                               \
        const int e_ = 4 * (q_) + i_;                                                                                  \
        const float got_ = __builtin_bit_cast(float, __builtin_amdgcn_mov_dpp(__builtin_bit_cast(int, dsend[e_]), 0xB1, 0xF, 0xF, true));    \
        dsc[e_] = kodd ? got_ : dmine[e_];                                                                             \
        dsc[8 + e_] = kodd ? dmine[e_] : got_;                                                                         \
        PIN2(dsc[e_]); PIN2(dsc[8 + e_]);                                                                              \
      }                                                                                                                \
    }                                                                                                                  \
  } while (0)
#define LQ(g_) do { const f32x4 v_ = *reinterpret_cast<const f32x4*>(stats + st_cur + 8 * (g_) + 4 * h); lq[4 * (g_)] = PBIAS - v_.x; lq[4 * (g_) + 1] = PBIAS - v_.y; lq[4 * (g_) + 2] = PBIAS - v_.z; lq[4 * (g_) + 3] = PBIAS - v_.w; } while (0)
#define DL(g_) do { const f32x4 v_ = *reinterpret_cast<const f32x4*>(stats + st_cur + 32 + 8 * (g_) + 4 * h); dl[4 * (g_)] = v_.x * k2a * k2b; dl[4 * (g_) + 1] = v_.y * k2a * k2b; dl[4 * (g_) + 2] = v_.z * k2a * k2b; dl[4 * (g_) + 3] = v_.w * k2a * k2b; } while (0)
#define PA(q_)                                                                                                         \
  do {                                                                                                                 \
    _Pragma("unroll") for (int i_ = 0; i_ < 2; ++i_) {                                                                 \
      const int m_ = 2 * (q_) + i_;                                                                                    \
      const float e0_ = __builtin_amdgcn_exp2f(__builtin_fmaf(s[2 * m_], cs, lq[2 * m_])), e1_ = __builtin_amdgcn_exp2f(__builtin_fmaf(s[2 * m_ + 1], cs, lq[2 * m_ + 1])); \
      pe[m_] = f32x2{e0_, e1_};                                                                                        \
      PIN2(pe[m_]);                                                                                                    \
    }                                                                                                                  \
  } while (0)
#define PB(q_)                                                                                                         \
  do {                                                                                                                 \
    _Pragma("unroll") for (int i_ = 0; i_ < 2; ++i_) {                                                                 \
      const int m_ = 2 * (q_) + i_;                                                                                    \
      pd[m_] = DROP ? f32x2{pe[m_].x * dsc[2 * m_], pe[m_].y * dsc[2 * m_ + 1]} : pe[m_];                              \
      const uint32_t w_ = cvt2(pd[m_]);                                                                                \
      pwv[0][m_ >> 2][m_ & 3] = w_;                                                                                    \
      PIN2(pwv[0][m_ >> 2][m_ & 3]);                                                                                   \
    }                                                                                                                  \
  } while (0)
#define PC(q_)                                                                                                         \
  do {                                                                                                                 \
    _Pragma("unroll") for (int i_ = 0; i_ < 2; ++i_) {                                                                 \
      const int m_ = 2 * (q_) + i_;                                                                                    \
      xx[m_] = pd[m_] - unpack2(pwv[0][m_ >> 2][m_ & 3]);                                                              \
      PIN2(xx[m_]);                                                                                                    \
    }                                                                                                                  \
  } while (0)
#define PD(q_)                                                                                                         \
  do {                                                                                                                 \
    _Pragma("unroll") for (int i_ = 0; i_ < 2; ++i_) {                                                                 \
      const int m_ = 2 * (q_) + i_;                                                                                    \
      pwv[1][m_ >> 2][m_ & 3] = cvt2(xx[m_]);                                                                          \
      PIN2(pwv[1][m_ >> 2][m_ & 3]);                                                                                   \
    }                                                                                                                  \
  } while (0)
#define QA(q_)                                                                                                         \
  do {                                                                                                                 \
    _Pragma("unroll") for (int i_ = 0; i_ < 2; ++i_) {                                                                 \
      const int m_ = 2 * (q_) + i_;                                                                                    \
      const f32x2 t_ = pe[m_] * f32x2{dl[2 * m_], dl[2 * m_ + 1]};                                                     \
      xx[m_] = pd[m_] * (f32x2{dp[2 * m_], dp[2 * m_ + 1]} * K1) - t_;                                                 \
      const uint32_t w_ = cvt2(xx[m_]);                                                                                \
      gwv[0][m_ >> 2][m_ & 3] = w_;                                                                                    \
      PIN2(gwv[0][m_ >> 2][m_ & 3]);                                                                                   \
    }                                                                                                                  \
  } while (0)
#define QB(q_)                                                                                                         \
  do {                                                                                                                 \
    _Pragma("unroll") for (int i_ = 0; i_ < 2; ++i_) {                                                                 \
      const int m_ = 2 * (q_) + i_;                                                                                    \
      xx[m_] = xx[m_] - unpack2(gwv[0][m_ >> 2][m_ & 3]);                                                              \
      PIN2(xx[m_]);                                                                                                    \
    }                                                                                                                  \
  } while (0)
#define QC(q_)                                                                                                         \
  do {                                                                                                                 \
    _Pragma("unroll") for (int i_ = 0; i_ < 2; ++i_) {                                                                 \
      const int m_ = 2 * (q_) + i_;                                                                                    \
      const uint32_t w_ = cvt2(xx[m_]);                                                                                \
      gwv[1][m_ >> 2][m_ & 3] = w_;                                                                                    \
      ff[m_] = unpack2(w_);                                                                                            \
      PIN2(ff[m_]);                                                                                                    \
    }                                                                                                                  \
  } while (0)
#define QD(q_)                                                                                                         \
  do {                                                                                                                 \
    _Pragma("unroll") for (int i_ = 0; i_ < 2; ++i_) {                                                                 \
      const int m_ = 2 * (q_) + i_;                                                                                    \
      gwv[2][m_ >> 2][m_ & 3] = cvt2(xx[m_] - ff[m_]);                                                                 \
      PIN2(gwv[2][m_ >> 2][m_ & 3]);                                                                                   \
    }                                                                                                                  \
  } while (0)
#define TW(g_)                                                                                                         \
  do {                                                                                                                 \
    _Pragma("unroll") for (int p_ = 0; p_ < 3; ++p_)                                                                   \
      *reinterpret_cast<u32x2*>(lds + tt_w + p_ * TT_PLANE + (tw0 ^ (8 * (g_)))) =                                      \
          u32x2{gwv[p_][(g_) >> 1][2 * ((g_) & 1)], gwv[p_][(g_) >> 1][2 * ((g_) & 1) + 1]};                            \
  } while (0)
#define STQ(i_) B4_STOREP(i_, qd_fre)
#define STS() do { B4_STORES(st_fre); qt_next = min(t + 3, nq - 1); goff = (unsigned)(qt_next * 32 * D + (tid >> 3) * D + (tid & 7) * 8); } while (0)
#define LDG(i_) B4_LOADP(i_)
#define LDS_() B4_LOADS(qt_next, t + 3 >= nq)
#define XW(g_) do { *reinterpret_cast<f32x4*>(xbuf + x_b + (xw0 ^ (8 * (g_)))) = f32x4{dq[4 * (g_)], dq[4 * (g_) + 1], dq[4 * (g_) + 2], dq[4 * (g_) + 3]}; } while (0)
#define B4_SYNC() __syncthreads()
#ifndef BWD4H_INC
#define BWD4H_INC "attn_bwd4h_phase.inc"
#endif
#include BWD4H_INC

    uint32_t hbn = hb;
    HA(0); HA(1); HB(0); HB(1); HC(0); HC(1); HD(0); HD(1);
#pragma unroll
    for (int p = 0; p < 2; ++p) fr[0][p] = FRQ(p, 0);
    for (int t = 0; t <= nq; ++t) {
      hbn += 32u * 0x85EBCA77U;
      SB();
      BWD4H_ITER();
      { const int t_ = qd_cur; qd_cur = qd_nxt; qd_nxt = qd_fre; qd_fre = t_; }
      { const int t_ = st_cur; st_cur = st_nxt; st_nxt = st_fre; st_fre = t_; }
      { const int t_ = tt_w; tt_w = tt_r; tt_r = t_; }
      { const int t_ = x_a; x_a = x_b; x_b = t_; }
      B4_SYNC();
    }
    {
      const int t = nq + 1;
      XOL(0); XOL(1);
      XOS(0); XOS(1);
    }
  }
  uint32_t gmax = 0u;
  if (key < a.Lk) {
    float* pk = a.dk + ((size_t)b * a.Lk + key) * a.ldk + head * D;
    float* pv = a.dv + ((size_t)b * a.Lk + key) * a.ldv + head * D;
#pragma unroll
    for (int mt = 0; mt < 2; ++mt)
#pragma unroll
      for (int g = 0; g < 4; ++g) {
        const float zk = kvalid ? dk_scale : 0.f, zv = kvalid ? dv_scale : 0.f;
        const float4 gk = make_float4(dk[mt][4 * g] * zk, dk[mt][4 * g + 1] * zk, dk[mt][4 * g + 2] * zk, dk[mt][4 * g + 3] * zk);
        const float4 gv = make_float4(dv[mt][4 * g] * zv, dv[mt][4 * g + 1] * zv, dv[mt][4 * g + 2] * zv, dv[mt][4 * g + 3] * zv);
        *reinterpret_cast<float4*>(pk + 32 * mt + 8 * g + 4 * h) = gk;
        *reinterpret_cast<float4*>(pv + 32 * mt + 8 * g + 4 * h) = gv;
        gmax = max(gmax, max(mag_bits4(gk), mag_bits4(gv)));
      }
  }
  if (a.mag) {
    gmax = max(gmax, (uint32_t)__shfl_xor((int)gmax, 32, 64));
    if (h == 0 && key < a.Lk) atomicMax(a.mag + (size_t)b * a.Lk + key, gmax);
  }
}

int attention_bwd4h_emu_launch(const EmuAttn& a, hipStream_t st) {
  static bool attr_set = false;
  if (!attr_set) {
    const void* ks[2] = {reinterpret_cast<const void*>(emu_attn_bwd4h_kernel<true>), reinterpret_cast<const void*>(emu_attn_bwd4h_kernel<false>)};
    for (const void* kf : ks)
      if (hipFuncSetAttribute(kf, hipFuncAttributeMaxDynamicSharedMemorySize, (int)B4H_LDS_BYTES) != hipSuccess) {
        set_error("attention_bwd_emu (f16x2): cannot raise the dynamic LDS limit to %u bytes", B4H_LDS_BYTES);
        return HOISDF_ERR_LAUNCH;
      }
    attr_set = true;
  }
  const dim3 grid(cdiv(a.Lk, 128) * 8 * cdiv(a.B * a.H, 8));
  if (a.drop_p > 0.f) hipLaunchKernelGGL((emu_attn_bwd4h_kernel<true>), grid, dim3(256), B4H_LDS_BYTES, st, a);
  else hipLaunchKernelGGL((emu_attn_bwd4h_kernel<false>), grid, dim3(256), B4H_LDS_BYTES, st, a);
  return check_launch("attention_bwd_emu (bwd4h)");
}

}
```

hoisdf_amd/csrc/attn_bwd4h_phase.inc:

```
#define BWD4H_ITER()                                                                          \
  do {                                                                                        \
    MFMA_SP0(s, fr[0][0], kf[0][1]); XOL(0); SB();                                            \
    MFMA_SP(s, fr[0][1], kf[0][0]); fr[1][0] = FRQ(0, 1); XOL(1); SB();                       \
    MFMA_SP(s, fr[0][0], kf[0][0]); fr[1][1] = FRQ(1, 1); SB();                               \
    MFMA_SP(s, fr[1][0], kf[1][1]); STQ(0); SB();                                             \
    MFMA_SP(s, fr[1][1], kf[1][0]); fr[0][0] = FRQ(0, 2); SB();                               \
    MFMA_SP(s, fr[1][0], kf[1][0]); fr[0][1] = FRQ(1, 2); SB();                               \
    MFMA_SP(s, fr[0][0], kf[2][1]); STQ(1); SB();                                             \
    MFMA_SP(s, fr[0][1], kf[2][0]); fr[1][0] = FRQ(0, 3); STQ(2); SB();                       \
    MFMA_SP(s, fr[0][0], kf[2][0]); fr[1][1] = FRQ(1, 3); LQ(0); SB();                        \
    MFMA_SP(s, fr[1][0], kf[3][1]); fr[0][0] = FRD(0, 0); LQ(1); SB();                        \
    MFMA_SP(s, fr[1][1], kf[3][0]); fr[0][1] = FRD(1, 0); LQ(2); LQ(3); SB();                 \
    MFMA_SP(s, fr[1][0], kf[3][0]); STQ(3); STS(); SB();                                      \
    MFMA_SP0(dp, fr[0][1], vf[0][0]); ft[0][0] = FRT(0, 0); LDG(0); SB();                     \
    MFMA_SP(dp, fr[0][0], vf[0][1]); fr[1][0] = FRD(0, 1); ft[0][1] = FRT(1, 0); SB();        \
    MFMA_SP(dp, fr[0][0], vf[0][0]); fr[1][1] = FRD(1, 1); ft[0][2] = FRT(2, 0); PA(0); SB(); \
    MFMA_SP(dp, fr[1][1], vf[1][0]); ft[1][0] = FRT(0, 1); LDG(1); SB();                      \
    MFMA_SP(dp, fr[1][0], vf[1][1]); fr[0][0] = FRD(0, 2); ft[1][1] = FRT(1, 1); PA(1); SB(); \
    MFMA_SP(dp, fr[1][0], vf[1][0]); fr[0][1] = FRD(1, 2); ft[1][2] = FRT(2, 1); PB(0); SB(); \
    MFMA_SP(dp, fr[0][1], vf[2][0]); ft[2][0] = FRT(0, 2); LDG(2); SB();                      \
    MFMA_SP(dp, fr[0][0], vf[2][1]); fr[1][0] = FRD(0, 3); ft[2][1] = FRT(1, 2); PB(1); SB(); \
    MFMA_SP(dp, fr[0][0], vf[2][0]); fr[1][1] = FRD(1, 3); ft[2][2] = FRT(2, 2); SB();        \
    MFMA_SP(dp, fr[1][1], vf[3][0]); ft[3][0] = FRT(0, 3); LDG(3); SB();                      \
    MFMA_SP(dp, fr[1][0], vf[3][1]); ft[3][1] = FRT(1, 3); LDS_(); SB();                      \
    MFMA_SP(dp, fr[1][0], vf[3][0]); ft[3][2] = FRT(2, 3); DL(0); SB();                       \
    MFMA_Q0(dq, ktf[0][1], ft[0][1]); PC(0); DL(1); DL(2); DL(3); SB();                       \
    MFMA_Q(dq, ktf[0][0], ft[0][2]); XOS(0); SB();                                            \
    MFMA_Q(dq, ktf[0][1], ft[0][0]); fr[0][0] = FRA(2 + 0, 0, 0); SB();                       \
    MFMA_Q(dq, ktf[0][0], ft[0][1]); fr[0][1] = FRA(2 + 1, 0, 0); SB();                       \
    MFMA_Q(dq, ktf[1][1], ft[1][1]); XOS(1); SB();                                            \
    MFMA_Q(dq, ktf[1][0], ft[1][2]); PC(1); SB();                                             \
    MFMA_Q(dq, ktf[1][1], ft[1][0]); PD(0); SB();                                             \
    MFMA_Q(dq, ktf[1][0], ft[1][1]); PD(1); QA(0); SB();                                      \
    MFMA_Q(dq, ktf[2][1], ft[2][1]); PA(2); SB();                                             \
    MFMA_Q(dq, ktf[2][0], ft[2][2]); PA(3); SB();                                             \
    MFMA_Q(dq, ktf[2][1], ft[2][0]); PB(2); SB();                                             \
    MFMA_Q(dq, ktf[2][0], ft[2][1]); PB(3); SB();                                             \
    MFMA_Q(dq, ktf[3][1], ft[3][1]); PC(2); QA(1); SB();                                      \
    MFMA_Q(dq, ktf[3][0], ft[3][2]); PC(3); QB(0); SB();                                      \
    MFMA_Q(dq, ktf[3][1], ft[3][0]); PD(2); QB(1); SB();                                      \
    MFMA_Q(dq, ktf[3][0], ft[3][1]); PD(3); QC(0); SB();                                      \
    MFMA_Q(dq, ktf[0][0], ft[0][0]); QC(1); SB();                                             \
    MFMA_Q(dq, ktf[1][0], ft[1][0]); QD(0); SB();                                             \
    MFMA_Q(dq, ktf[2][0], ft[2][0]); QD(1); SB();                                             \
    MFMA_Q(dq, ktf[3][0], ft[3][0]); TW(0); SB();                                             \
    MFMA_VK(dv[0], fr[0][1], PWF(0, 0)); TW(1); SB();                                         \
    MFMA_VK(dv[0], fr[0][0], PWF(1, 0)); fr[1][0] = FRA(2 + 0, 0, 1); QA(2); SB();            \
    MFMA_VK(dv[0], fr[0][0], PWF(0, 0)); fr[1][1] = FRA(2 + 1, 0, 1); QA(3); SB();            \
    MFMA_VK(dv[1], fr[1][1], PWF(0, 0)); QB(2); XW(0); SB();                                  \
    MFMA_VK(dv[1], fr[1][0], PWF(1, 0)); fr[0][0] = FRA(2 + 0, 1, 0); QB(3); SB();            \
    MFMA_VK(dv[1], fr[1][0], PWF(0, 0)); fr[0][1] = FRA(2 + 1, 1, 0); QC(2); SB();            \
    MFMA_VK(dv[0], fr[0][1], PWF(0, 1)); QC(3); XW(1); SB();                                  \
    MFMA_VK(dv[0], fr[0][0], PWF(1, 1)); fr[1][0] = FRA(2 + 0, 1, 1); QD(2); XW(2); SB();     \
    MFMA_VK(dv[0], fr[0][0], PWF(0, 1)); fr[1][1] = FRA(2 + 1, 1, 1); QD(3); SB();            \
    MFMA_VK(dv[1], fr[1][1], PWF(0, 1)); fr[0][0] = FRA(0, 0, 0); TW(2); SB();                \
    MFMA_VK(dv[1], fr[1][0], PWF(1, 1)); fr[0][1] = FRA(1, 0, 0); TW(3); SB();                \
    MFMA_VK(dv[1], fr[1][0], PWF(0, 1)); XW(3); SB();                                         \
    MFMA_VK(dk[0], fr[0][1], GWF(1, 0)); SB();                                                \
    MFMA_VK(dk[0], fr[0][0], GWF(2, 0)); fr[1][0] = FRA(0, 0, 1); SB();                       \
    MFMA_VK(dk[0], fr[0][1], GWF(0, 0)); fr[1][1] = FRA(1, 0, 1); SB();                       \
    MFMA_VK(dk[0], fr[0][0], GWF(1, 0)); HA(0); SB();                                         \
    MFMA_VK(dk[0], fr[0][0], GWF(0, 0)); HA(1); SB();                                         \
    MFMA_VK(dk[1], fr[1][1], GWF(1, 0)); HB(0); SB();                                         \
    MFMA_VK(dk[1], fr[1][0], GWF(2, 0)); fr[0][0] = FRA(0, 1, 0); SB();                       \
    MFMA_VK(dk[1], fr[1][1], GWF(0, 0)); fr[0][1] = FRA(1, 1, 0); SB();                       \
    MFMA_VK(dk[1], fr[1][0], GWF(1, 0)); HB(1); SB();                                         \
    MFMA_VK(dk[1], fr[1][0], GWF(0, 0)); HC(0); SB();                                         \
    MFMA_VK(dk[0], fr[0][1], GWF(1, 1)); HC(1); SB();                                         \
    MFMA_VK(dk[0], fr[0][0], GWF(2, 1)); fr[1][0] = FRA(0, 1, 1); SB();                       \
    MFMA_VK(dk[0], fr[0][1], GWF(0, 1)); fr[1][1] = FRA(1, 1, 1); SB();                       \
    MFMA_VK(dk[0], fr[0][0], GWF(1, 1)); HD(0); SB();                                         \
    MFMA_VK(dk[0], fr[0][0], GWF(0, 1)); HD(1); SB();                                         \
    MFMA_VK(dk[1], fr[1][1], GWF(1, 1)); SB();                                                \
    MFMA_VK(dk[1], fr[1][0], GWF(2, 1)); fr[0][0] = FRQN(0, 0); SB();                         \
    MFMA_VK(dk[1], fr[1][1], GWF(0, 1)); fr[0][1] = FRQN(1, 0); SB();                         \
    MFMA_VK(dk[1], fr[1][0], GWF(1, 1)); SB();                                                \
    MFMA_VK(dk[1], fr[1][0], GWF(0, 1)); SB();                                                \
  } while (0)
```

hoisdf_amd/csrc/layers.hip:

```cpp
#include <stdlib.h>

#include <mutex>
#include <unordered_map>

#include "chain.h"

namespace hoisdf {
namespace {

__global__ void rows_copy_add_kernel(float* __restrict__ dst, long dst_gs, const float* __restrict__ src, long src_gs, int rows, int E4,
                                     long total, int add) {
  const long i = (long)blockIdx.x * blockDim.x + threadIdx.x;
  if (i >= total) return;
  const long per = (long)rows * E4;
  const long g = i / per, r = i - g * per;
  float4* d = reinterpret_cast<float4*>(dst + g * dst_gs) + r;
  const float4 s = reinterpret_cast<const float4*>(src + g * src_gs)[r];
  if (add) { float4 t = *d; t.x += s.x; t.y += s.y; t.z += s.z; t.w += s.w; *d = t; }
  else *d = s;
}
int rows_copy_add(float* dst, long dst_gs, const float* src, long src_gs, int groups, int rows, int E, int add, hipStream_t st) {
  const long total = (long)groups * rows * (E / 4);
  if (total == 0) return HOISDF_OK;
  hipLaunchKernelGGL(rows_copy_add_kernel, dim3((unsigned)cdiv(total, 256)), dim3(256), 0, st, dst, dst_gs, src, src_gs, rows, E / 4, total, add);
// ... 49 lines not shown
  void* planes; long planes_bytes;
  uint32_t* mag; long mag_bytes;
};
enum { MAG_O = 0, MAG_X1 = 1, MAG_H = 2, MAG_XOUT = 3, MAG_ROWS = 4 };
void carve_saved(const Geo& g, Bump& b, Saved& s) {
  const int E = g.E;
  s.qkv = s.qbuf = s.kvbuf = s.xq = nullptr;
  if (g.full) { if (!g.fused_qkv) s.qkv = b.floats(g.Ms * 3 * E); }
  else {
    if (!g.fused_qkv) { s.qbuf = b.floats(g.M * E); s.kvbuf = b.floats(g.Ms * 2 * E); }
    s.xq = b.floats(g.M * E);
  }
  s.o = b.floats(g.M * E); s.lse = b.floats((long)g.B * g.H * g.nq); s.a = b.floats(g.M * E); s.x1 = b.floats(g.M * E);
  s.h = b.floats(g.M * g.F); s.bits = static_cast<uint32_t*>(b.take(g.M * ((g.F + 31) / 32) * 4)); s.f = b.floats(g.M * E);
  s.st = b.floats(6 * g.M);
  s.planes_bytes = g.att_bwd_emu ? hoisdf_attention_emu_workspace(g.B, g.H, g.nq, g.S, 2) : 0;
  s.planes = s.planes_bytes ? b.take(s.planes_bytes) : nullptr;
  s.mag_bytes = ((long)MAG_ROWS * g.M + 3L * g.H * g.B) * 4;
  s.mag = static_cast<uint32_t*>(b.take(s.mag_bytes));
}
uint32_t* head_q(const Geo& g, uint32_t* mag) { return mag ? mag + (long)MAG_ROWS * g.M : nullptr; }
uint32_t* head_k(const Geo& g, uint32_t* mag) { return mag ? head_q(g, mag) + (long)g.H * g.B : nullptr; }
uint32_t* head_v(const Geo& g, uint32_t* mag) { return mag ? head_q(g, mag) + 2L * g.H * g.B : nullptr; }
bool layer_mags(const Ctx& c, const Geo& g) { return c.emu && emu_form_h2() && g.M >= EMU_MIN_ROWS; }

int forward(const float* x, const hoisdf_encoder_layer_weights* w, const hoisdf_encoder_layer_desc* d, const Geo& g, float* x_out, float* y_out,
            Bump& saved, Bump& ws, bool dry, void* stream) {
  Ctx c{as_stream(stream), stream, &ws, dry, gemm_emu_mode()};
  Saved s;
  carve_saved(g, d->training ? saved : ws, s);
  const int E = g.E, F = g.F;
  const float *q = nullptr, *k = nullptr, *v = nullptr; int ldq = 0, ldkv = 0;
  const float* xq2 = x;
  void* aw = s.planes; long ab = s.planes_bytes;
  if (g.att == 2 && !aw) { ab = hoisdf_attention_emu_workspace(g.B, g.H, g.nq, g.S, 0); aw = ws.take(ab); }
  const bool mags = layer_mags(c, g) && (dry || s.mag);
  auto mg = [&](int i) -> uint32_t* { return mags && s.mag ? s.mag + (long)i * g.M : nullptr; };
  uint32_t* const smag = mags ? s.mag : nullptr;
  const uint32_t* xm = mags ? d->x_mag : nullptr;
  if (mags && !dry && c.ok() && hipMemsetAsync(s.mag, 0, (size_t)s.mag_bytes, c.st) != hipSuccess) c.rc = HOISDF_ERR_LAUNCH;
  if (g.fused_qkv) {
    QkvPlanes pq{}, pkv{};
    const void* im = nullptr; const void* im_q = nullptr; const void* im_kv = nullptr;
    if (g.full) im = image_of(c, w->img_in, w->w_in, E, 3 * E, E, 0);
    else {
      if (!dry && c.ok()) c.rc = rows_copy_add(s.xq, (long)g.nq * E, x, (long)g.S * E, g.B, g.nq, E, 0, c.st);
      xq2 = s.xq;
      im_q = image_of(c, w->img_in_q, w->w_in, E, E, E, 0);
      im_kv = image_of(c, w->img_in_kv, w->w_in + (size_t)E * E, E, 2 * E, E, 0);
    }
    if (!dry && c.ok()) {
      if (!aw) c.rc = HOISDF_ERR_WORKSPACE;
      else {
        attention_emu_plane_targets(aw, g.B, g.H, g.nq, g.S, s.planes ? 1 : 0, pq, pkv);
        if (g.full) c.rc = linear_fwd_emu_qkv(x, E, im, w->b_in, g.Ms, 3 * E, E, pq, stream, xm);
        else {
          c.rc = linear_fwd_emu_qkv(s.xq, E, im_q, w->b_in, g.M, E, E, pq, stream, nullptr);
          pkv.col0 = E;
          if (c.ok()) c.rc = linear_fwd_emu_qkv(x, E, im_kv, w->b_in ? w->b_in + E : nullptr, g.Ms, 2 * E, E, pkv, stream, xm);
        }
      }
    }
  } else if (g.full) {
    lin_fwd(c, x, E, w->w_in, E, w->img_in, w->b_in, s.qkv, 3 * E, g.Ms, 3 * E, E, 0, 0.f, 0, nullptr, 0, xm, nullptr,
            g.att_h2 ? head_q(g, smag) : nullptr, g.S);
    q = s.qkv; k = s.qkv + E; v = s.qkv + 2 * E; ldq = ldkv = 3 * E;
  } else {
    if (!dry && c.ok()) c.rc = rows_copy_add(s.xq, (long)g.nq * E, x, (long)g.S * E, g.B, g.nq, E, 0, c.st);
    xq2 = s.xq;
    lin_fwd(c, s.xq, E, w->w_in, E, w->img_in_q, w->b_in, s.qbuf, E, g.M, E, E, 0, 0.f, 0, nullptr, 0, nullptr, nullptr,
            g.att_h2 ? head_q(g, smag) : nullptr, g.nq);
    lin_fwd(c, x, E, w->w_in + (size_t)E * E, E, w->img_in_kv, w->b_in ? w->b_in + E : nullptr, s.kvbuf, 2 * E, g.Ms, 2 * E, E, 0, 0.f, 0, nullptr, 0, xm, nullptr,
            g.att_h2 ? head_k(g, smag) : nullptr, g.S);
    q = s.qbuf; k = s.kvbuf; v = s.kvbuf + E; ldq = E; ldkv = 2 * E;
  }
  const uint32_t* o_mag = g.att == 2 ? mg(MAG_O) : nullptr;
  if (g.fused_qkv) {
    if (!dry && c.ok())
      c.rc = attention_fwd_emu_planes(s.o, E, s.lse, g.B, g.H, g.nq, g.S, g.S, g.p, d->seed[0], aw, s.planes ? 1 : 0, stream, mg(MAG_O));
  } else if (g.att == 2) {
    if (!dry && c.ok()) {
      if (!aw) c.rc = HOISDF_ERR_WORKSPACE;
      else {
        const bool hm = g.att_h2 && smag;
        c.rc = attention_fwd_emu_mag(q, ldq, k, ldkv, v, ldkv, s.o, E, s.lse, g.B, g.H, g.nq, g.S, g.S, g.p, d->seed[0], aw, ab,
                                     s.planes ? 1 : 0, mg(MAG_O), stream, hm ? head_q(g, smag) : nullptr, hm ? head_k(g, smag) : nullptr,
                                     hm ? head_v(g, smag) : nullptr);
      }
    }
  } else if (!dry && c.ok()) {
    c.rc = hoisdf_attention_fwd(q, ldq, k, ldkv, v, ldkv, s.o, E, s.lse, g.B, g.H, g.nq, g.S, g.S, g.p, d->seed[0], stream);
  }
  lin_fwd(c, s.o, E, w->w_out, E, w->img_out, w->b_out, s.a, E, g.M, E, E, 0, 0.f, 0, nullptr, 0, o_mag, nullptr);
  float* st = s.st;
  if (!dry && c.ok()) c.rc = add_layernorm_fwd_mag(xq2, s.a, w->g1, w->be1, s.x1, st, st + g.M, g.M, E, g.eps, g.p, d->seed[1], mg(MAG_X1), stream);
  lin_fwd(c, s.x1, E, w->w1, E, w->img_1, w->b1, s.h, F, g.M, F, E, 1, g.p, d->seed[2], s.bits, 0, mg(MAG_X1), mg(MAG_H));
  lin_fwd(c, s.h, F, w->w2, F, w->img_2, w->b2, s.f, E, g.M, E, F, 0, 0.f, 0, nullptr, 0, mg(MAG_H), nullptr);
  if (!dry && c.ok()) c.rc = add_layernorm_fwd_mag(s.x1, s.f, w->g2, w->be2, x_out, st + 2 * g.M, st + 3 * g.M, g.M, E, g.eps, g.p, d->seed[3], mg(MAG_XOUT), stream);
  if (w->g3 && !dry && c.ok()) {
    if (g.ni == g.nq) c.rc = hoisdf_add_layernorm_fwd(x_out, nullptr, w->g3, w->be3, y_out, st + 4 * g.M, st + 5 * g.M, g.M, E, g.eps, 0.f, 0, stream);
    else c.rc = hoisdf_layernorm_rows_fwd(x_out, w->g3, w->be3, y_out, st + 4 * g.M, st + 5 * g.M, g.B, g.nq, g.ni, E, g.eps, stream);
  }
  if (c.ok() && !dry && (ws.overflow || saved.overflow)) { set_error("encoder_layer_fwd: workspace / saved buffer too small"); return HOISDF_ERR_WORKSPACE; }
  return c.rc;
}

int backward(const float* x, const float* x_out, const hoisdf_encoder_layer_weights* w, const hoisdf_encoder_layer_desc* d, const Geo& g,
             Bump& saved, const float* g_x_out, const float* g_y, float* dx, const hoisdf_encoder_layer_grads* G, Bump& ws, bool dry,
             void* stream, bool fwd_mags = true) {
  Ctx c{as_stream(stream), stream, &ws, dry, gemm_emu_mode()};
  Saved s;
  carve_saved(g, saved, s);
  const int E = g.E, F = g.F;
  const long M = g.M, Ms = g.Ms;
  const float* st = s.st;
  const float* dx2 = g_x_out;
  if (g_y && w->g3) {
    float* t = ws.floats(M * E);
    if (!dry && c.ok()) {
      if (!t) c.rc = HOISDF_ERR_WORKSPACE;
      else if (g.ni == g.nq) c.rc = hoisdf_add_layernorm_bwd(g_y, x_out, nullptr, w->g3, st + 4 * M, st + 5 * M, g_x_out, t, nullptr, G->dg3, G->dbe3, M, E, 0.f, 0, stream);
      else c.rc = hoisdf_layernorm_rows_bwd(g_y, x_out, w->g3, st + 4 * M, st + 5 * M, g_x_out, t, G->dg3, G->dbe3, g.B, g.nq, g.ni, E, stream);
    }
    dx2 = t;
  }
  float* dx1 = ws.floats(M * E); float* df = ws.floats(M * E); float* dh = ws.floats(M * F);
  float* dxq = g.full ? dx : ws.floats(M * E);
  float* da = ws.floats(M * E); float* dO = ws.floats(M * E);
  float* delta = ws.floats((long)g.B * g.H * g.nq);
  if (!dry && (!dx1 || !df || !dh || !dxq || !da || !dO || !delta)) { set_error("encoder_layer_bwd: workspace too small"); return HOISDF_ERR_WORKSPACE; }
  if (!dry && !dx2) { set_error("encoder_layer_bwd: no upstream gradient (g_x_out and g_y both null)"); return HOISDF_ERR_INVALID; }
  enum { MAG_DF = 0, MAG_DH = 1, MAG_DA = 2, MAG_BROWS = 3 };
  const long bmag_bytes = ((long)MAG_BROWS * M + Ms + (long)g.H * g.B) * 4;
  uint32_t* bmag = static_cast<uint32_t*>(ws.take(bmag_bytes));
  const bool mags = layer_mags(c, g) && (dry || bmag);
  auto mg = [&](int i) -> uint32_t* { return mags && bmag ? bmag + (long)i * M : nullptr; };
  uint32_t* const mag_dqkv = mags && bmag ? bmag + (long)MAG_BROWS * M : nullptr;
  uint32_t* const head_do = mags && bmag ? bmag + (long)MAG_BROWS * M + Ms : nullptr;
  auto fm = [&](int i) -> const uint32_t* { return mags && fwd_mags && s.mag ? s.mag + (long)i * M : nullptr; };
  uint32_t* const smag = mags && fwd_mags ? s.mag : nullptr;
  if (mags && !dry && c.ok() && hipMemsetAsync(bmag, 0, (size_t)bmag_bytes, c.st) != hipSuccess) c.rc = HOISDF_ERR_LAUNCH;
  if (!dry && c.ok()) c.rc = add_layernorm_bwd_mag(dx2, s.x1, s.f, w->g2, st + 2 * M, st + 3 * M, nullptr, dx1, df, G->dg2, G->dbe2, M, E, g.p, d->seed[3], nullptr, mg(MAG_DF), stream);
  lin_bwd_input(c, df, E, nullptr, 0.f, w->w2, F, w->img_t_2, dh, F, M, E, F, 0, mg(MAG_DF), mg(MAG_DH));
  lin_bwd_weight(c, df, E, nullptr, 0.f, s.h, F, G->dw2, G->db2, M, E, F, 0, mg(MAG_DF), fm(MAG_H));
  lin_bwd_input(c, dh, F, s.bits, g.p, w->w1, E, w->img_t_1, dx1, E, M, F, E, 1, mg(MAG_DH), nullptr);
  lin_bwd_weight(c, dh, F, s.bits, g.p, s.x1, E, G->dw1, G->db1, M, F, E, 0, mg(MAG_DH), fm(MAG_X1));
  const float* xq2 = g.full ? x : s.xq;
  if (!dry && c.ok()) c.rc = add_layernorm_bwd_mag(dx1, xq2, s.a, w->g1, st, st + M, nullptr, dxq, da, G->dg1, G->dbe1, M, E, g.p, d->seed[1], nullptr, mg(MAG_DA), stream);
  lin_bwd_input(c, da, E, nullptr, 0.f, w->w_out, E, w->img_t_out, dO, E, M, E, E, 0, mg(MAG_DA), nullptr, g.att_h2 ? head_do : nullptr, g.nq);
  lin_bwd_weight(c, da, E, nullptr, 0.f, s.o, E, G->dw_out, G->db_out, M, E, E, 0, mg(MAG_DA), g.att == 2 ? fm(MAG_O) : nullptr);
  const bool amag = mags && g.att_bwd_emu && g.full;
  auto attn_bwd = [&](const float* q, int ldq, const float* k, const float* v, int ldkv, float* dq, float* dk, float* dv) {
    if (g.att_bwd_emu) {
      const long ab = hoisdf_attention_bwd_emu_workspace(g.B, g.H, g.nq, g.S, s.planes ? 1 : 0);
      void* aw = ws.take(ab);
      if (dry || !c.ok()) return;
      if (!aw) { c.rc = HOISDF_ERR_WORKSPACE; return; }
      const bool hm = g.att_h2 && smag && head_do;
      if (g.att_h2 && !hm) { set_error("encoder_layer_bwd: the forward ran the f16x2 attention but the head magnitudes are not available"); c.rc = HOISDF_ERR_INVALID; return; }
      c.rc = attention_bwd_emu_mag(q, ldq, k, ldkv, v, ldkv, s.o, E, dO, E, s.lse, delta, dq, dk, dv, g.B, g.H, g.nq, g.S, g.S, g.p, d->seed[0],
                                   s.planes, aw, ab, amag ? mag_dqkv : nullptr, stream, hm ? head_q(g, smag) : nullptr,
                                   hm ? head_k(g, smag) : nullptr, hm ? head_v(g, smag) : nullptr, hm ? head_do : nullptr);
    } else if (!dry && c.ok()) {
      c.rc = hoisdf_attention_bwd(q, ldq, k, ldkv, v, ldkv, s.o, E, dO, E, s.lse, delta, dq, dk, dv, g.B, g.H, g.nq, g.S, g.S, g.p, d->seed[0], stream);
    }
  };
  if (g.full) {
    float* dqkv = ws.floats(Ms * 3 * E);
    if (!dry && !dqkv) { set_error("encoder_layer_bwd: workspace too small"); return HOISDF_ERR_WORKSPACE; }
    if (g.fused_qkv) attn_bwd(nullptr, 3 * E, nullptr, nullptr, 3 * E, dqkv, dqkv + E, dqkv + 2 * E);
    else attn_bwd(s.qkv, 3 * E, s.qkv + E, s.qkv + 2 * E, 3 * E, dqkv, dqkv + E, dqkv + 2 * E);
    lin_bwd_input(c, dqkv, 3 * E, nullptr, 0.f, w->w_in, E, w->img_t_in, dxq, E, Ms, 3 * E, E, 1, amag ? mag_dqkv : nullptr, nullptr);
    lin_bwd_weight(c, dqkv, 3 * E, nullptr, 0.f, x, E, G->dw_in, G->db_in, Ms, 3 * E, E, 0, amag ? mag_dqkv : nullptr, amag ? d->x_mag : nullptr);
  } else {
    float* dq = ws.floats(M * E); float* dkv = ws.floats(Ms * 2 * E);
    if (!dry && (!dq || !dkv)) { set_error("encoder_layer_bwd: workspace too small"); return HOISDF_ERR_WORKSPACE; }
    if (g.fused_qkv) attn_bwd(nullptr, E, nullptr, nullptr, 2 * E, dq, dkv, dkv + E);
    else attn_bwd(s.qbuf, E, s.kvbuf, s.kvbuf + E, 2 * E, dq, dkv, dkv + E);
    lin_bwd_input(c, dq, E, nullptr, 0.f, w->w_in, E, w->img_t_in_q, dxq, E, M, E, E, 1);
    lin_bwd_weight(c, dq, E, nullptr, 0.f, s.xq, E, G->dw_in, G->db_in, M, E, E);
    lin_bwd_input(c, dkv, 2 * E, nullptr, 0.f, w->w_in + (size_t)E * E, E, w->img_t_in_kv, dx, E, Ms, 2 * E, E, 0);
    lin_bwd_weight(c, dkv, 2 * E, nullptr, 0.f, x, E, G->dw_in + (size_t)E * E, G->db_in ? G->db_in + E : nullptr, Ms, 2 * E, E);
    if (!dry && c.ok()) c.rc = rows_copy_add(dx, (long)g.S * E, dxq, (long)g.nq * E, g.B, g.nq, E, 1, c.st);
  }
  if (c.ok() && !dry && ws.overflow) { set_error("encoder_layer_bwd: workspace too small"); return HOISDF_ERR_WORKSPACE; }
  return c.rc;
}

}
}

using namespace hoisdf;

extern "C" long hoisdf_encoder_layer_saved_bytes(const hoisdf_encoder_layer_desc* d) {
  Geo g;
  if (geometry(d, g) != HOISDF_OK) return -1;
  Bump b(nullptr, 0); Saved s;
  carve_saved(g, b, s);
  return b.off + 256;
}

extern "C" const uint32_t* hoisdf_encoder_layer_out_mag(const hoisdf_encoder_layer_desc* d, const void* saved) {
  Geo g;
  if (!saved || geometry(d, g) != HOISDF_OK || !d->training) return nullptr;
  Ctx c{nullptr, nullptr, nullptr, false, gemm_emu_mode()};
  if (!layer_mags(c, g)) return nullptr;
  Bump b(const_cast<void*>(saved), 1L << 62); Saved s;
  carve_saved(g, b, s);
  return s.mag ? s.mag + (long)MAG_XOUT * g.M : nullptr;
}

extern "C" long hoisdf_encoder_layer_workspace_bytes(const hoisdf_encoder_layer_desc* d, int backward_pass) {
  Geo g;
  if (geometry(d, g) != HOISDF_OK) return -1;
  hoisdf_encoder_layer_weights w{};
  hoisdf_encoder_layer_grads G{};
  float dummy = 0.f;
  w.g3 = &dummy;
  Bump saved(nullptr, 0), ws(nullptr, 0);
  if (backward_pass) (void)backward(nullptr, nullptr, &w, d, g, saved, &dummy, &dummy, nullptr, &G, ws, true, nullptr);
  else (void)forward(nullptr, &w, d, g, nullptr, nullptr, saved, ws, true, nullptr);
  return ws.off + 256;
}

extern "C" int hoisdf_encoder_layer_fwd(const float* x, const hoisdf_encoder_layer_weights* w, const hoisdf_encoder_layer_desc* d, float* x_out,
                                        float* y_out, void* saved, long saved_bytes, void* workspace, long workspace_bytes, void* stream) {
  Geo g;
  if (int rc = geometry(d, g)) return rc;
  HOISDF_REQUIRE(x && w && x_out && w->w_in && w->w_out && w->w1 && w->w2 && w->g1 && w->be1 && w->g2 && w->be2, HOISDF_ERR_INVALID,
                 "encoder_layer_fwd: null pointer");
  HOISDF_REQUIRE(!w->g3 || (w->be3 && y_out), HOISDF_ERR_INVALID, "encoder_layer_fwd: inter_norm needs be3 and y_out");
  HOISDF_REQUIRE(!d->training || saved, HOISDF_ERR_WORKSPACE, "encoder_layer_fwd: training needs the saved buffer (hoisdf_encoder_layer_saved_bytes)");
  HOISDF_REQUIRE(workspace || workspace_bytes == 0, HOISDF_ERR_WORKSPACE, "encoder_layer_fwd: null workspace");
  HOISDF_REQUIRE(al16(x) && al16(x_out) && al16(saved) && al16(workspace), HOISDF_ERR_INVALID, "encoder_layer_fwd: buffers must be 16-byte aligned");
  Bump sv(saved, saved_bytes), ws(workspace, workspace_bytes);
  static char none;
  if (!sv.base) { sv.base = &none; sv.cap = 0; }
  if (!ws.base) { ws.base = &none; ws.cap = 0; }
  if (d->training) {
    Ctx c0{nullptr, nullptr, nullptr, false, gemm_emu_mode()};
    saved_forms().put(saved, (g.fused_qkv ? 1 : 0) | (g.att_h2 ? 2 : 0) | (layer_mags(c0, g) ? 4 : 0));
  }
  const int rc = forward(x, w, d, g, x_out, y_out, sv, ws, false, stream);
  if (rc == HOISDF_ERR_WORKSPACE) set_error("encoder_layer_fwd: workspace (%ld bytes) or saved buffer (%ld bytes) too small", workspace_bytes, saved_bytes);
  return rc;
}

extern "C" int hoisdf_encoder_layer_bwd(const float* x, const float* x_out, const hoisdf_encoder_layer_weights* w, const hoisdf_encoder_layer_desc* d,
                                        const void* saved, long saved_bytes, const float* g_x_out, const float* g_y, float* dx,
                                        const hoisdf_encoder_layer_grads* grads, void* workspace, long workspace_bytes, void* stream) {
  Geo g;
  if (int rc = geometry(d, g)) return rc;
  HOISDF_REQUIRE(x && x_out && w && saved && dx && grads && workspace, HOISDF_ERR_INVALID, "encoder_layer_bwd: null pointer");
  HOISDF_REQUIRE(grads->dw_in && grads->db_in && grads->dw_out && grads->db_out && grads->dg1 && grads->dbe1 && grads->dw1 && grads->db1 &&
                     grads->dw2 && grads->db2 && grads->dg2 && grads->dbe2 && (!w->g3 || !g_y || (grads->dg3 && grads->dbe3)),
                 HOISDF_ERR_INVALID, "encoder_layer_bwd: every parameter gradient buffer is required (zero-filled)");
  HOISDF_REQUIRE(d->training, HOISDF_ERR_INVALID, "encoder_layer_bwd: the forward call must have run with training = 1");
  HOISDF_REQUIRE(al16(x) && al16(dx) && al16(saved) && al16(workspace), HOISDF_ERR_INVALID, "encoder_layer_bwd: buffers must be 16-byte aligned");
  const int recorded = saved_forms().take(saved);
  if (recorded >= 0) { g.fused_qkv = (recorded & 1) != 0; g.att_h2 = (recorded & 2) != 0; }
  const bool fwd_mags = recorded < 0 || (recorded & 4) != 0;
  Bump sv(const_cast<void*>(saved), saved_bytes), ws(workspace, workspace_bytes);
  const int rc = backward(x, x_out, w, d, g, sv, g_x_out, g_y, dx, grads, ws, false, stream, fwd_mags);
  if (rc == HOISDF_OK && sv.overflow) { set_error("encoder_layer_bwd: saved buffer too small"); return HOISDF_ERR_WORKSPACE; }
  if (rc == HOISDF_ERR_WORKSPACE) set_error("encoder_layer_bwd: workspace (%ld bytes) too small", workspace_bytes);
  return rc;
}

namespace hoisdf {
namespace {

__global__ void add_bcast_kernel(float* __restrict__ out, const float* __restrict__ a, const float* __restrict__ p, int rows_p, int E4, long total) {
  const long i = (long)blockIdx.x * blockDim.x + threadIdx.x;
  if (i >= total) return;
  const long per = (long)rows_p * E4;
  const float4 x = reinterpret_cast<const float4*>(a)[i], y = reinterpret_cast<const float4*>(p)[i % per];
  reinterpret_cast<float4*>(out)[i] = make_float4(x.x + y.x, x.y + y.y, x.z + y.z, x.w + y.w);
}
__global__ void sum_bcast_grad_kernel(float* __restrict__ dp, const float* __restrict__ g1, const float* __restrict__ g2, int B, int rows_p, int E4) {
  const int i = blockIdx.x * blockDim.x + threadIdx.x;
  if (i >= rows_p * E4) return;
  float4 acc = reinterpret_cast<float4*>(dp)[i];
  for (int b = 0; b < B; ++b) {
    const float4 x = reinterpret_cast<const float4*>(g1)[(long)b * rows_p * E4 + i], y = reinterpret_cast<const float4*>(g2)[(long)b * rows_p * E4 + i];
    acc.x += x.x + y.x; acc.y += x.y + y.y; acc.z += x.z + y.z; acc.w += x.w + y.w;
  }
  reinterpret_cast<float4*>(dp)[i] = acc;
}

struct DGeo { int B, Q, S, E, F, H, kv; long M, Ms; float eps, p; };
int dgeometry(const hoisdf_decoder_layer_desc* d, DGeo& g) {
  HOISDF_REQUIRE(d, HOISDF_ERR_INVALID, "decoder_layer: null descriptor");
  HOISDF_REQUIRE(d->B > 0 && d->Q > 0 && d->Q <= 64 && d->S > 0 && d->E > 0 && d->F > 0 && d->H > 0 && d->E % d->H == 0 && d->E % 4 == 0 &&
                     d->F % 4 == 0 && d->kv_len > 0 && d->kv_len <= d->S,
                 HOISDF_ERR_INVALID, "decoder_layer: bad sizes B=%d Q=%d S=%d E=%d F=%d H=%d kv_len=%d", d->B, d->Q, d->S, d->E, d->F, d->H, d->kv_len);
  HOISDF_REQUIRE(d->drop_p >= 0.f && d->drop_p < 1.f, HOISDF_ERR_INVALID, "decoder_layer: drop_p=%f", d->drop_p);
  g.B = d->B; g.Q = d->Q; g.S = d->S; g.E = d->E; g.F = d->F; g.H = d->H; g.kv = d->kv_len;
  g.M = (long)d->B * d->Q; g.Ms = (long)d->B * d->S; g.eps = d->eps; g.p = d->drop_p;
  return HOISDF_OK;
}
struct DSaved {
  float *tq1, *qk, *v, *probs, *o1, *a1, *x1, *tq2, *q2, *kv, *o2, *lse2, *a2, *x2, *h, *f, *st; uint32_t* bits;
};
void dcarve(const DGeo& g, Bump& b, DSaved& s) {
  const long M = g.M; const int E = g.E;
  s.tq1 = b.floats(M * E); s.qk = b.floats(M * 2 * E); s.v = b.floats(M * E); s.probs = b.floats((long)g.B * g.H * g.Q * g.Q);
  s.o1 = b.floats(M * E); s.a1 = b.floats(M * E); s.x1 = b.floats(M * E); s.tq2 = b.floats(M * E); s.q2 = b.floats(M * E);
// ... 175 lines not shown
```

hoisdf_amd/ops.py:

```python
from __future__ import annotations

import ctypes as C
import math
import os
from typing import Optional, Sequence

import torch

from . import _lib
from ._lib import (_DEC_W, _SDF_G, MLP_MAX_LAYERS, DecoderLayerDesc, DecoderLayerGrads, DecoderLayerWeights, EncoderLayerDesc,
                   EncoderLayerGrads, EncoderLayerWeights, Mlp, MlpGrads, PoseOutputs, Pyramid, SdfWeightGrads, SdfWeights, call, lib)
from .emu_images import WeightImageCache, prepare_batch_table

_SEED = [0x9E3779B97F4A7C15, 0]
_WEIGHT_GEN = [0]


def deterministic() -> bool:
    return bool(lib().hoisdf_get_deterministic())


def set_deterministic(on: bool) -> None:
    lib().hoisdf_set_deterministic(int(bool(on)))

# ... 718 lines not shown
    center, cam_intr, bbox = center.contiguous(), cam_intr.contiguous(), bbox.contiguous()
    _chk(center, cam_intr, bbox)
    if counts is None or not counts.matches(center, cam_intr, bbox, scale, bins_n):
        counts = SdfInferCounts(center, cam_intr, bbox, scale, bins_n)
    cl = counts.wait()
    n = sum(cl)
    short = [b for b in range(B) if cl[b] < num_points]
    if short:
        raise ValueError(f"sdf_infer: sample {short[0]} has only {cl[short[0]]} lattice points inside its bbox, fewer "
                         f"than num_points={num_points} (the reference fails at main/model.py:348)")
    counts_h = (C.c_int32 * B)(*cl)
    w = weights.get()
    assert w.C == pyr.C
    nbytes = lib().hoisdf_sdf_infer_workspace(n, B, w.C)
    ws = torch.empty(nbytes, device=dev, dtype=torch.uint8)
    pts = torch.empty(B, num_points, 3, device=dev)
    sdf = torch.empty(B, num_points, device=dev)
    pe = torch.empty(B, num_points, 30, device=dev)
    s = pyr.struct()
    call("hoisdf_sdf_infer", C.byref(s), _p(center), _p(cam_intr), _p(bbox), float(scale), bins_n, B, _p(counts.counts),
         C.addressof(counts_h), num_points, img_hw[0], img_hw[1], C.byref(w), float(clamp), float(drop_p),
         next_seed() if drop_p > 0 else 0, _p(pts), _p(sdf), _p(pe), _p(ws), nbytes, _st())
    return pts, sdf, pe


def select_smallest_abs(sdf_raw, offsets, counts, k: int):
    B = offsets.shape[0]
    sel = torch.empty(B, k, device=sdf_raw.device, dtype=torch.int32)
    call("hoisdf_select_smallest_abs", _p(sdf_raw), _p(offsets), _p(counts), B, k, _p(sel), _st())
    return sel


def gather_rows(src, sel):
    src2 = _rows(src) if src.dim() > 1 else src.reshape(-1, 1)
    n = sel.numel()
    out = torch.empty(n, src2.shape[1], device=src.device, dtype=torch.float32)
    call("hoisdf_gather_rows", _p(src2), src2.stride(0), _p(sel.reshape(-1).contiguous()), n, src2.shape[1], _p(out),
         src2.shape[1], _st())
    return out


class _TokenBuild(torch.autograd.Function):
    @staticmethod
    def forward(ctx, tok, cam, center, pe, feat, sdf, beta, row0):
        B, S, D = tok.shape
        P = cam.shape[0] // B
        feat2 = _rows(feat)
        cam, pe, sdf = cam.contiguous(), pe.reshape(-1, 30).contiguous(), sdf.reshape(-1).contiguous()
        _chk(tok, cam, center, pe, feat2, sdf, beta)
        call("hoisdf_token_build_fwd", _p(cam), _p(center), _p(pe), _p(feat2), feat2.stride(0), _p(sdf), _p(beta),
             _p(tok), B, P, S, row0, D, _st())
        ctx.save_for_backward(feat2, sdf, beta)
        ctx.meta = (B, P, S, row0, D, feat.shape)
        ctx.mark_dirty(tok)
        return tok

    @staticmethod
    def backward(ctx, dtok):
        feat2, sdf, beta = ctx.saved_tensors
        B, P, S, row0, D, fshape = ctx.meta
        dtok = dtok.contiguous()
        dfeat = torch.empty(B * P, D - 33, device=dtok.device, dtype=torch.float32)
        dbeta = _zeros(1, dtok.device)
        part = torch.empty(lib().hoisdf_token_build_bwd_partials(), device=dtok.device, dtype=torch.float32)
        call("hoisdf_token_build_bwd_ordered", _p(dtok), _p(feat2), feat2.stride(0), _p(sdf), _p(beta), _p(dfeat), D - 33,
             _p(dbeta), _p(part), B, P, S, row0, D, _st())
        dtok_in = dtok.clone()
        dtok_in[:, row0:row0 + P] = 0
        return dtok_in, None, None, None, dfeat.view(fshape), None, dbeta, None


def token_build(tok, cam, center, pe, feat, sdf, beta, row0: int):
    return _TokenBuild.apply(tok, cam, center.contiguous(), pe, feat, sdf, beta, row0)


def _attn_out(q, k, v, H, want_lse=True):
    B, Lq, E = q.shape
    Lk = k.shape[1]
    for t, L in ((q, Lq), (k, Lk), (v, Lk)):
        assert t.stride(2) == 1 and t.stride(0) == L * t.stride(1), "attention operands must be row-uniform views"
    o = torch.empty(B, Lq, E, device=q.device, dtype=torch.float32)
    lse = torch.empty(B, H, Lq, device=q.device, dtype=torch.float32) if want_lse else None
    return B, Lq, Lk, E, o, lse


def _attn_fwd(q, k, v, H, kv_len, drop_p, seed):
    B, Lq, Lk, E, o, lse = _attn_out(q, k, v, H)
    call("hoisdf_attention_fwd", _p(q), q.stride(1), _p(k), k.stride(1), _p(v), v.stride(1), _p(o), E, _p(lse),
         B, H, Lq, Lk, kv_len, float(drop_p), seed, _st())
    return o, lse


def _attn_bwd(q, k, v, o, lse, do, dq, dk, dv, H, kv_len, drop_p, seed):
    B, Lq, E = q.shape
    Lk = k.shape[1]
    assert dq.stride(1) == q.stride(1) and dk.stride(1) == k.stride(1) and dv.stride(1) == v.stride(1)
    delta = torch.empty(B, H, Lq, device=q.device, dtype=torch.float32)
    call("hoisdf_attention_bwd", _p(q), q.stride(1), _p(k), k.stride(1), _p(v), v.stride(1), _p(o), E, _p(do), E,
         _p(lse), _p(delta), _p(dq), _p(dk), _p(dv), B, H, Lq, Lk, kv_len, drop_p, seed, _st())


_ATTENTION_EMU = os.environ.get("HOISDF_ATTENTION", "emu") != "f32"


def set_attention_emu(on: bool) -> None:
    global _ATTENTION_EMU
    _ATTENTION_EMU = bool(on)


def attention_emu() -> bool:
    return _ATTENTION_EMU


def _attn_emulated(Lq: int) -> bool:
    return Lq >= 32 and _ATTENTION_EMU


_EMU_PLANES = {}


def _planes_key(q, k, v, H, kv_len):
    return (q.data_ptr(), k.data_ptr(), v.data_ptr(), tuple(q.shape), k.shape[1], H, kv_len)


_ATTN_FORM_H2 = os.environ.get("HOISDF_ATTN_FORM", "h2")[:1].lower() != "b"


def _attn_h2(rows: int) -> bool:
    return _ATTN_FORM_H2 and _GEMM_EMU and _h2() and rows >= _GEMM_EMU_MIN_ROWS


def _attn_fwd_emu(q, k, v, H, kv_len, drop_p, seed, keep=False, heads=None):
    B, Lq, Lk, E, o, lse = _attn_out(q, k, v, H)
    nbytes = lib().hoisdf_attention_emu_workspace(B, H, Lq, Lk, 2 if keep else 0)
    ws = torch.empty(nbytes, device=q.device, dtype=torch.uint8)
    if heads is not None:
        call("hoisdf_attention_fwd_emu_mag", _p(q), q.stride(1), _p(k), k.stride(1), _p(v), v.stride(1), _p(o), E, _p(lse), B, H, Lq, Lk,
             kv_len, float(drop_p), seed, _p(ws), nbytes, 0, _p(heads[0]), _p(heads[1]), _p(heads[2]), None, _st())
        return o, lse
    call("hoisdf_attention_fwd_emu", _p(q), q.stride(1), _p(k), k.stride(1), _p(v), v.stride(1), _p(o), E, _p(lse), B, H, Lq, Lk,
         kv_len, float(drop_p), seed, _p(ws), nbytes, int(keep), _st())
    if keep:
        if len(_EMU_PLANES) >= 64:
            _EMU_PLANES.clear()
        _EMU_PLANES[_planes_key(q, k, v, H, kv_len)] = ws
    return o, lse


def _attn_bwd_emu(q, k, v, o, lse, do, dq, dk, dv, H, kv_len, drop_p, seed, heads=None):
    B, Lq, E = q.shape
    Lk = k.shape[1]
    assert dq.stride(1) == q.stride(1) and dk.stride(1) == k.stride(1) and dv.stride(1) == v.stride(1)
    kept = _EMU_PLANES.pop(_planes_key(q, k, v, H, kv_len), None)
    nbytes = lib().hoisdf_attention_bwd_emu_workspace(B, H, Lq, Lk, int(kept is not None))
    ws = torch.empty(nbytes, device=q.device, dtype=torch.uint8)
    delta = torch.empty(B, H, Lq, device=q.device, dtype=torch.float32)
    if kept is not None:
        kept.record_stream(torch.cuda.current_stream(q.device))
    if heads is not None:
        do_hm = _head_measure(do, E, B * Lq, H, Lq)
        call("hoisdf_attention_bwd_emu_mag", _p(q), q.stride(1), _p(k), k.stride(1), _p(v), v.stride(1), _p(o), E, _p(do), E, _p(lse),
             _p(delta), _p(dq), _p(dk), _p(dv), B, H, Lq, Lk, kv_len, float(drop_p), seed, _p(kept), _p(ws), nbytes, _p(heads[0]),
             _p(heads[1]), _p(heads[2]), _p(do_hm), None, _st())
        return
    call("hoisdf_attention_bwd_emu", _p(q), q.stride(1), _p(k), k.stride(1), _p(v), v.stride(1), _p(o), E, _p(do), E, _p(lse),
         _p(delta), _p(dq), _p(dk), _p(dv), B, H, Lq, Lk, kv_len, float(drop_p), seed, _p(kept), _p(ws), nbytes, _st())


_ATTN_BWD_EMU = os.environ.get("HOISDF_ATTN_BWD", "emu") != "f32"


def _emu_bwd() -> bool:
    return _ATTN_BWD_EMU or deterministic()


def _attn_fwd_mode(emulated, q, k, v, H, kv_len, drop_p, seed, keep=False, heads=None):
    if emulated and heads is not None:
        return _attn_fwd_emu(q, k, v, H, kv_len, drop_p, seed, heads=heads)
    if emulated:
        return _attn_fwd_emu(q, k, v, H, kv_len, drop_p, seed, keep=keep and _emu_bwd())
    return _attn_fwd(q, k, v, H, kv_len, drop_p, seed)


def _attn_bwd_mode(emulated, *a, heads=None):
    if emulated and _emu_bwd():
        return _attn_bwd_emu(*a, heads=heads)
    return _attn_bwd(*a)


class _AttentionSelf(torch.autograd.Function):

    @staticmethod
    def forward(ctx, qkv, H, kv_len, drop_p, seed):
        qkv = qkv.contiguous()
        _chk(qkv)
        E = qkv.shape[2] // 3
        emulated = _attn_emulated(qkv.shape[1])
        o, lse = _attn_fwd_mode(emulated, qkv[:, :, :E], qkv[:, :, E:2 * E], qkv[:, :, 2 * E:], H, kv_len, drop_p, seed,
                                keep=any(ctx.needs_input_grad))
        ctx.save_for_backward(qkv, o, lse)
        ctx.meta = (H, kv_len, float(drop_p), seed, emulated)
        return o

    @staticmethod
    def backward(ctx, do):
        qkv, o, lse = ctx.saved_tensors
        H, kv_len, drop_p, seed, emulated = ctx.meta
        E = qkv.shape[2] // 3
        d = torch.empty_like(qkv)
        _attn_bwd_mode(emulated, qkv[:, :, :E], qkv[:, :, E:2 * E], qkv[:, :, 2 * E:], o, lse, do.contiguous(), d[:, :, :E],
                       d[:, :, E:2 * E], d[:, :, 2 * E:], H, kv_len, drop_p, seed)
        return d, None, None, None, None


class _AttentionCross(torch.autograd.Function):

    @staticmethod
    def forward(ctx, q, kv, H, kv_len, drop_p, seed):
        q, kv = q.contiguous(), kv.contiguous()
        _chk(q, kv)
        E = q.shape[2]
        emulated = _attn_emulated(q.shape[1])
        o, lse = _attn_fwd_mode(emulated, q, kv[:, :, :E], kv[:, :, E:], H, kv_len, drop_p, seed, keep=any(ctx.needs_input_grad))
        ctx.save_for_backward(q, kv, o, lse)
        ctx.meta = (H, kv_len, float(drop_p), seed, emulated)
        return o

    @staticmethod
    def backward(ctx, do):
        q, kv, o, lse = ctx.saved_tensors
        H, kv_len, drop_p, seed, emulated = ctx.meta
        E = q.shape[2]
        dq = torch.empty_like(q)
        dkv = torch.empty_like(kv)
        _attn_bwd_mode(emulated, q, kv[:, :, :E], kv[:, :, E:], o, lse, do.contiguous(), dq, dkv[:, :, :E], dkv[:, :, E:], H, kv_len,
                       drop_p, seed)
        return dq, dkv, None, None, None, None


_ATTENTION_F16_EVAL = False


def set_attention_f16_eval(on: bool) -> None:
    global _ATTENTION_F16_EVAL
    _ATTENTION_F16_EVAL = bool(on)


def _attn_fwd_f16(q, k, v, H, kv_len):
    B, Lq, Lk, E, o, _ = _attn_out(q, k, v, H, want_lse=False)
    nbytes = lib().hoisdf_attention_bf16x2_workspace(B, H, Lq, Lk)
    ws = torch.empty(nbytes, device=q.device, dtype=torch.uint8)
    call("hoisdf_attention_fwd_bf16x2", _p(q), q.stride(1), _p(k), k.stride(1), _p(v), v.stride(1), _p(o), E, B, H, Lq, Lk,
         kv_len, _p(ws), nbytes, _st())
    return o


def _use_f16(drop_p, *tensors) -> bool:
    return _ATTENTION_F16_EVAL and drop_p == 0.0 and not (torch.is_grad_enabled() and any(t.requires_grad for t in tensors))


def attention_self(qkv, H: int, kv_len: Optional[int] = None, drop_p: float = 0.0):
    kv_len = qkv.shape[1] if kv_len is None else kv_len
    if _use_f16(drop_p, qkv):
        qkv = qkv.contiguous()
        E = qkv.shape[2] // 3
        return _attn_fwd_f16(qkv[:, :, :E], qkv[:, :, E:2 * E], qkv[:, :, 2 * E:], H, kv_len)
    seed = next_seed() if drop_p > 0 else 0
    return _AttentionSelf.apply(qkv, H, kv_len, drop_p, seed)


def attention_cross(q, kv, H: int, kv_len: Optional[int] = None, drop_p: float = 0.0):
    kv_len = kv.shape[1] if kv_len is None else kv_len
    if _use_f16(drop_p, q, kv):
        q, kv = q.contiguous(), kv.contiguous()
        E = q.shape[2]
        return _attn_fwd_f16(q, kv[:, :, :E], kv[:, :, E:], H, kv_len)
    seed = next_seed() if drop_p > 0 else 0
    return _AttentionCross.apply(q, kv, H, kv_len, drop_p, seed)


class _AttentionSmall(torch.autograd.Function):
    @staticmethod
    def forward(ctx, q, k, v, mask_u8, H, drop_p, seed):
        q, k, v = q.contiguous(), k.contiguous(), v.contiguous()
        _chk(q, k, v)
        B, Lq, E = q.shape
        Lk = k.shape[1]
        o = torch.empty(B, Lq, E, device=q.device, dtype=torch.float32)
        probs = torch.empty(B, H, Lq, Lk, device=q.device, dtype=torch.float32)
        call("hoisdf_attention_small_fwd", _p(q), E, _p(k), E, _p(v), E, _p(mask_u8), _p(o), E, _p(probs), B, H, Lq,
             Lk, float(drop_p), seed, _st())
        ctx.save_for_backward(q, k, v, probs)
        ctx.meta = (H, float(drop_p), seed)
        return o

    @staticmethod
    def backward(ctx, do):
        q, k, v, probs = ctx.saved_tensors
        H, drop_p, seed = ctx.meta
        B, Lq, E = q.shape
        Lk = k.shape[1]
        do = do.contiguous()
        dq = torch.empty_like(q)
        dk = torch.zeros_like(k)
        dv = torch.zeros_like(v)
        call("hoisdf_attention_small_bwd", _p(q), E, _p(k), E, _p(v), E, _p(probs), _p(do), E, _p(dq), _p(dk), _p(dv),
             B, H, Lq, Lk, drop_p, seed, _st())
# ... 1012 lines not shown
```

include/hoisdf.h:

```cpp
#ifndef HOISDF_H_
#define HOISDF_H_

#include <stdint.h>

#ifdef __cplusplus
extern "C" {
#endif

#define HOISDF_VERSION_MAJOR 0
#define HOISDF_VERSION_MINOR 1

typedef enum hoisdf_status {
  HOISDF_OK = 0,
  HOISDF_ERR_INVALID = -1,
  HOISDF_ERR_LAUNCH = -2,
  HOISDF_ERR_TOO_FEW = -3,
  HOISDF_ERR_WORKSPACE = -4
} hoisdf_status;

#define HOISDF_MAX_LEVELS 8

typedef struct hoisdf_pyramid {
  int n_levels;
  int B;
// ... 41 lines not shown
                             const float* x, int ldx, float* dW, int lddw, float* db, long M, int N,
                             int K, float* workspace, long workspace_floats, void* stream);
long hoisdf_linear_emu_image_bytes(int rows, int K);
int hoisdf_linear_emu_prepare(const float* W, int ldw, int N, int K, int transpose, void* image, void* stream);
typedef struct hoisdf_emu_prep_item {
  const float* W;
  void* image;
  long first_block;
  int ldw, N, K, transpose;
} hoisdf_emu_prep_item;
long hoisdf_linear_emu_prepare_blocks(int N, int K, int transpose);
int hoisdf_linear_emu_prepare_batch(const hoisdf_emu_prep_item* d_items, int n, long total_blocks, void* stream);
int hoisdf_linear_emu_supported(const float* a, long lda, int contraction);
int hoisdf_linear_emu_pieces(void);
long hoisdf_mag_words(long rows);
int hoisdf_mag_measure(const float* x, long ldx, long M, int K, uint32_t* words, void* stream);
long hoisdf_head_mag_words(long M, int groups, int L);
int hoisdf_head_mag_measure(const float* x, long ldx, long M, int groups, int L, uint32_t* words, void* stream);
int hoisdf_linear_fwd_emu_heads(const float* x, int ldx, const void* w_image, const float* bias, float* y, int ldy, long M, int N,
                                int K, const uint32_t* x_mag, uint32_t* y_mag, uint32_t* y_heads, int L, void* stream);
int hoisdf_linear_bwd_input_emu_heads(const float* dy, int lddy, const void* wt_image, float* dx, int lddx, long M, int N, int K,
                                      const uint32_t* dy_mag, uint32_t* dx_mag, uint32_t* dx_heads, int L, void* stream);
int hoisdf_linear_fwd_emu_mag(const float* x, int ldx, const void* w_image, const float* bias, float* y, int ldy, long M, int N,
                              int K, int act, float drop_p, uint64_t seed, uint32_t* relu_bits, const uint32_t* x_mag,
                              uint32_t* y_mag, void* stream);
int hoisdf_linear_bwd_input_emu_mag(const float* dy, int lddy, const uint32_t* relu_bits, float drop_p, const void* wt_image,
                                    float* dx, int lddx, long M, int N, int K, int accumulate, const uint32_t* dy_mag,
                                    uint32_t* dx_mag, void* stream);
int hoisdf_linear_bwd_weight_emu_mag(const float* dy, int lddy, const uint32_t* relu_bits, float drop_p, const float* x, int ldx,
                                     float* dW, int lddw, float* db, long M, int N, int K, float* workspace, long workspace_floats,
                                     const uint32_t* dy_mag, const uint32_t* x_mag, void* stream);
int hoisdf_linear_fwd_emu(const float* x, int ldx, const void* w_image, const float* bias, float* y, int ldy, long M, int N,
                          int K, int act, float drop_p, uint64_t seed, uint32_t* relu_bits, void* stream);
int hoisdf_linear_bwd_input_emu(const float* dy, int lddy, const uint32_t* relu_bits, float drop_p, const void* wt_image,
                                float* dx, int lddx, long M, int N, int K, int accumulate, void* stream);
int hoisdf_linear_emu_small_max_rows(void);
int hoisdf_linear_emu_small_supported(const float* a, long lda, const float* W, long ldw, long M, int N, int K);
int hoisdf_linear_fwd_emu_small(const float* x, int ldx, const float* W, int ldw, const float* bias, float* y, int ldy, long M,
                                int N, int K, int act, float drop_p, uint64_t seed, uint32_t* relu_bits, void* stream);
int hoisdf_linear_bwd_input_emu_small(const float* dy, int lddy, const uint32_t* relu_bits, float drop_p, const float* W, int ldw,
                                      float* dx, int lddx, long M, int N, int K, int accumulate, void* stream);
int hoisdf_linear_bwd_weight_emu_small(const float* dy, int lddy, const uint32_t* relu_bits, float drop_p, const float* x, int ldx,
                                       float* dW, int lddw, float* db, long M, int N, int K, void* stream);
long hoisdf_linear_bwd_weight_emu_workspace(long M, int N, int K);
int hoisdf_linear_bwd_weight_emu(const float* dy, int lddy, const uint32_t* relu_bits, float drop_p, const float* x, int ldx,
                                 float* dW, int lddw, float* db, long M, int N, int K, float* workspace, long workspace_floats,
                                 void* stream);
int hoisdf_relu_dropout_bwd(const float* y, int ldy, const float* dy, int lddy, float* dpre,
                            int ldd, long M, int N, float drop_p, void* stream);

int hoisdf_posenc_fwd(const float* points, long n_rows, float* x0, int ldx0, int col0,
                      float* pe, void* stream);
int hoisdf_weightnorm_fwd(const float* v, const float* g, float* W, int ldw, float* norms,
                          int out, int in, void* stream);
int hoisdf_weightnorm_bwd(const float* v, const float* g, const float* dW, int ldw, float* dv,
                          float* dg, int out, int in, void* stream);
int hoisdf_sdf_head_fwd(const float* h, int ldh, const float* w, const float* b, float* sdf_raw,
                        float* sdf, long n_rows, int K, float clamp, void* stream);
int hoisdf_sdf_head_bwd(const float* dsdf, const float* sdf_raw, const float* h, int ldh,
                        const float* w, float* dh, int lddh, float* dw, float* db, long n_rows,
                        int K, float clamp, void* stream);

typedef struct hoisdf_sdf_weights {
  int C;
  const float *sdfin_w0, *sdfin_b0;
  const float *sdfin_w1, *sdfin_b1;
  const float *dec_w0, *dec_b0;
  int dec_ld0;
  const float *dec_w1, *dec_b1;
  const float *dec_w2, *dec_b2;
  const float *dec_w3, *dec_b3;
  const float *dec_w4, *dec_b4;
  const void* emu_img[6];
  const void* emu_img_t[6];
} hoisdf_sdf_weights;
long hoisdf_sdf_query_workspace(long n_rows, int C, int need_feat);
int hoisdf_sdf_query_fwd(const hoisdf_pyramid* pyr, const float* points, const int32_t* sample_idx, long n_rows,
                         int rows_per_sample, const float* center, const float* cam_intr, float scale, int img_h,
                         int img_w, const float* feat_in, float* feat_out, const hoisdf_sdf_weights* w, float clamp,
                         float drop_p, uint64_t seed, float* sdf, float* sdf_raw, float* pe, float* cam_out,
                         void* workspace, long workspace_bytes, void* stream);

int hoisdf_lattice_count(const float* center, const float* cam_intr, const float* bbox, float scale,
                         int bins_n, int B, int32_t* counts, void* stream);
int hoisdf_lattice_fill(const float* center, const float* cam_intr, const float* bbox, float scale,
                        int bins_n, int B, const int32_t* offsets, float* points,
                        int32_t* sample_idx, int32_t* lattice_idx, void* stream);
int hoisdf_select_smallest_abs(const float* sdf_raw, const int32_t* offsets, const int32_t* counts,
                               int B, int k, int32_t* sel, void* stream);
int hoisdf_gather_rows(const float* src, int lds, const int32_t* sel, long n_sel, int width,
                       float* out, int ldo, void* stream);
typedef struct hoisdf_sdf_weight_grads {
  float *d_sdfin_w0, *d_sdfin_b0, *d_sdfin_w1, *d_sdfin_b1;
  float *d_dec_w0, *d_dec_b0, *d_dec_w1, *d_dec_b1, *d_dec_w2, *d_dec_b2, *d_dec_w3, *d_dec_b3, *d_dec_w4, *d_dec_b4;
} hoisdf_sdf_weight_grads;
long hoisdf_sdf_query_train_saved_bytes(long n_rows, int C);
long hoisdf_sdf_query_train_workspace_bytes(long n_rows, int C, int backward_pass);
int hoisdf_sdf_query_train_fwd(const hoisdf_pyramid* pyr, const float* points, const int32_t* sample_idx, long n_rows,
                               int rows_per_sample, const float* center, const float* cam_intr, float scale, int img_h, int img_w,
                               const hoisdf_sdf_weights* w, float clamp, float drop_p, uint64_t seed, float* sdf, float* pe,
                               float* cam_out, void* saved, long saved_bytes, void* workspace, long workspace_bytes, void* stream);
int hoisdf_sdf_query_bwd(const hoisdf_pyramid_grad* dpyr, const float* points, const int32_t* sample_idx, long n_rows,
                         int rows_per_sample, const float* center, const float* cam_intr, float scale, int img_h, int img_w,
                         const hoisdf_sdf_weights* w, float clamp, float drop_p, const void* saved, long saved_bytes,
                         const float* d_sdf, const hoisdf_sdf_weight_grads* grads, void* workspace, long workspace_bytes,
                         void* stream);

int hoisdf_sdf_infer_count_begin(const float* center, const float* cam_intr, const float* bbox, float scale, int bins_n,
                                 int B, int32_t* counts_device, int32_t* counts_host, void* stream);
int hoisdf_sdf_infer_count(const float* center, const float* cam_intr, const float* bbox, float scale, int bins_n, int B,
                           int32_t* counts_device, int32_t* counts_host, long* n_rows, void* stream);
long hoisdf_sdf_infer_workspace(long n_rows, int B, int C);
int hoisdf_sdf_infer(const hoisdf_pyramid* pyr, const float* center, const float* cam_intr, const float* bbox, float scale,
                     int bins_n, int B, const int32_t* counts_device, const int32_t* counts_host, int num_points, int img_h,
                     int img_w, const hoisdf_sdf_weights* w, float clamp, float drop_p, uint64_t seed, float* points_out,
                     float* sdf_out, float* pe_out, void* workspace, long workspace_bytes, void* stream);

int hoisdf_sdf_sample_keys(const float* rows, int ld, const int64_t* seg_row0, const int32_t* seg_len,
                           const int32_t* seg_off, const int32_t* seg_col, int n_seg, int max_len, float dist,
                           uint64_t seed, float* keys, int32_t* eligible, void* stream);

int hoisdf_token_build_fwd(const float* cam, const float* center, const float* pe,
                           const float* feat, int ldfeat, const float* sdf, const float* beta_ptr,
                           float* tok, int B, int P, int S, int row0, int D, void* stream);
int hoisdf_token_build_bwd(const float* dtok, const float* feat, int ldfeat, const float* sdf,
                           const float* beta_ptr, float* dfeat, int lddfeat, float* dbeta, int B,
                           int P, int S, int row0, int D, void* stream);

int hoisdf_token_build_bwd_partials(void);
int hoisdf_token_build_bwd_ordered(const float* dtok, const float* feat, int ldfeat, const float* sdf, const float* beta_ptr,
                                   float* dfeat, int lddfeat, float* dbeta, float* partials, int B, int P, int S, int row0,
                                   int D, void* stream);

int hoisdf_attention_fwd(const float* q, int ldq, const float* k, int ldk, const float* v, int ldv,
                         float* o, int ldo, float* lse, int B, int H, int Lq, int Lk, int kv_len,
                         float drop_p, uint64_t seed, void* stream);
int hoisdf_attention_bwd(const float* q, int ldq, const float* k, int ldk, const float* v, int ldv,
                         const float* o, int ldo, const float* dout, int lddo, const float* lse,
                         float* delta, float* dq, float* dk, float* dv, int B, int H, int Lq, int Lk,
                         int kv_len, float drop_p, uint64_t seed, void* stream);
long hoisdf_attention_bf16x2_workspace(int B, int H, int Lq, int Lk);
int hoisdf_attention_fwd_bf16x2(const float* q, int ldq, const float* k, int ldk, const float* v, int ldv, float* o, int ldo,
                                int B, int H, int Lq, int Lk, int kv_len, void* workspace, long workspace_bytes, void* stream);

long hoisdf_attention_emu_workspace(int B, int H, int Lq, int Lk, int mode);
int hoisdf_attention_fwd_emu(const float* q, int ldq, const float* k, int ldk, const float* v, int ldv, float* o, int ldo,
                             float* lse, int B, int H, int Lq, int Lk, int kv_len, float drop_p, uint64_t seed, void* workspace,
                             long workspace_bytes, int keep, void* stream);
int hoisdf_attention_fwd_emu_mag(const float* q, int ldq, const float* k, int ldk, const float* v, int ldv, float* o, int ldo,
                                 float* lse, int B, int H, int Lq, int Lk, int kv_len, float drop_p, uint64_t seed, void* workspace,
                                 long workspace_bytes, int keep, const uint32_t* q_mag, const uint32_t* k_mag, const uint32_t* v_mag,
                                 uint32_t* o_mag, void* stream);
long hoisdf_attention_bwd_emu_workspace(int B, int H, int Lq, int Lk, int kept);
int hoisdf_attention_bwd_emu(const float* q, int ldq, const float* k, int ldk, const float* v, int ldv, const float* o, int ldo,
                             const float* dout, int lddo, const float* lse, float* delta, float* dq, float* dk, float* dv, int B,
                             int H, int Lq, int Lk, int kv_len, float drop_p, uint64_t seed, const void* fwd_workspace,
                             void* workspace, long workspace_bytes, void* stream);
int hoisdf_attention_bwd_emu_mag(const float* q, int ldq, const float* k, int ldk, const float* v, int ldv, const float* o, int ldo,
                                 const float* dout, int lddo, const float* lse, float* delta, float* dq, float* dk, float* dv, int B,
                                 int H, int Lq, int Lk, int kv_len, float drop_p, uint64_t seed, const void* fwd_workspace,
                                 void* workspace, long workspace_bytes, const uint32_t* q_mag, const uint32_t* k_mag,
                                 const uint32_t* v_mag, const uint32_t* do_mag, uint32_t* g_mag, void* stream);
int hoisdf_attention_small_fwd(const float* q, int ldq, const float* k, int ldk, const float* v,
                               int ldv, const uint8_t* mask, float* o, int ldo, float* probs, int B,
                               int H, int Lq, int Lk, float drop_p, uint64_t seed, void* stream);
int hoisdf_attention_small_bwd(const float* q, int ldq, const float* k, int ldk, const float* v,
                               int ldv, const float* probs, const float* dout, int lddo, float* dq,
                               float* dk, float* dv, int B, int H, int Lq, int Lk, float drop_p,
                               uint64_t seed, void* stream);

int hoisdf_add_layernorm_fwd(const float* x, const float* r, const float* gamma, const float* beta,
                             float* y, float* mean, float* rstd, long M, int D, float eps,
                             float drop_p, uint64_t seed, void* stream);
int hoisdf_add_layernorm_bwd(const float* dy, const float* x, const float* r, const float* gamma,
                             const float* mean, const float* rstd,
                             const float* dx_add ,
                             float* dx, float* dr, float* dgamma, float* dbeta, long M, int D, float drop_p,
                             uint64_t seed, void* stream);

int hoisdf_residual_dropout(const float* x, const float* r, float* y, long M, int D, float drop_p, uint64_t seed, void* stream);

int hoisdf_layernorm_rows_fwd(const float* x, const float* gamma, const float* beta, float* y, float* mean, float* rstd,
                              long groups, int rows_per_group, int take, int D, float eps, void* stream);
int hoisdf_layernorm_rows_bwd(const float* dy, const float* x, const float* gamma, const float* mean, const float* rstd,
                              const float* dx_add, float* dx, float* dgamma, float* dbeta, long groups, int rows_per_group,
                              int take, int D, void* stream);

typedef struct hoisdf_encoder_layer_desc {
  int B, S, E, F, H;
  int n_query;
  int n_inter;
  float eps, drop_p;
  uint64_t seed[4];
  int attention;
  int attention_bwd_emulated;
  int training;
  const uint32_t* x_mag;
} hoisdf_encoder_layer_desc;
const uint32_t* hoisdf_encoder_layer_out_mag(const hoisdf_encoder_layer_desc* d, const void* saved);
typedef struct hoisdf_encoder_layer_weights {
  const float *w_in, *b_in;
  const float *w_out, *b_out;
  const float *g1, *be1;
  const float *w1, *b1;
  const float *w2, *b2;
  const float *g2, *be2;
  const float *g3, *be3;
  const void *img_in, *img_in_q, *img_in_kv, *img_out, *img_1, *img_2;
  const void *img_t_in, *img_t_in_q, *img_t_in_kv, *img_t_out, *img_t_1, *img_t_2;
} hoisdf_encoder_layer_weights;
typedef struct hoisdf_encoder_layer_grads {
  float *dw_in, *db_in, *dw_out, *db_out, *dg1, *dbe1, *dw1, *db1, *dw2, *db2, *dg2, *dbe2, *dg3, *dbe3;
} hoisdf_encoder_layer_grads;
long hoisdf_encoder_layer_saved_bytes(const hoisdf_encoder_layer_desc* desc);
long hoisdf_encoder_layer_workspace_bytes(const hoisdf_encoder_layer_desc* desc, int backward_pass);
int hoisdf_encoder_layer_fwd(const float* x, const hoisdf_encoder_layer_weights* weights, const hoisdf_encoder_layer_desc* desc,
                             float* x_out, float* y_out, void* saved, long saved_bytes, void* workspace, long workspace_bytes,
                             void* stream);
int hoisdf_encoder_layer_bwd(const float* x, const float* x_out, const hoisdf_encoder_layer_weights* weights,
                             const hoisdf_encoder_layer_desc* desc, const void* saved, long saved_bytes, const float* g_x_out,
                             const float* g_y, float* dx, const hoisdf_encoder_layer_grads* grads, void* workspace,
                             long workspace_bytes, void* stream);

typedef struct hoisdf_decoder_layer_desc {
  int B, Q, S, E, F, H, kv_len;
  float eps, drop_p;
  uint64_t seed[6];
  int training;
} hoisdf_decoder_layer_desc;
typedef struct hoisdf_decoder_layer_weights {
  const float *sa_w_in, *sa_b_in, *sa_w_out, *sa_b_out;
  const float *ca_w_in, *ca_b_in, *ca_w_out, *ca_b_out;
  const float *w1, *b1, *w2, *b2;
  const float *g1, *be1, *g2, *be2, *g3, *be3;
  const float *g4, *be4;
  const void *img_ca_kv, *img_t_ca_kv;
} hoisdf_decoder_layer_weights;
typedef struct hoisdf_decoder_layer_grads {
  float *dsa_w_in, *dsa_b_in, *dsa_w_out, *dsa_b_out, *dca_w_in, *dca_b_in, *dca_w_out, *dca_b_out, *dw1, *db1, *dw2, *db2,
      *dg1, *dbe1, *dg2, *dbe2, *dg3, *dbe3, *dg4, *dbe4;
} hoisdf_decoder_layer_grads;
long hoisdf_decoder_layer_saved_bytes(const hoisdf_decoder_layer_desc* desc);
long hoisdf_decoder_layer_workspace_bytes(const hoisdf_decoder_layer_desc* desc, int backward_pass);
int hoisdf_decoder_layer_fwd(const float* tgt, const float* memory, const float* query_pos, const uint8_t* tgt_mask,
                             const hoisdf_decoder_layer_weights* weights, const hoisdf_decoder_layer_desc* desc, float* out,
                             float* y_out, void* saved, long saved_bytes, void* workspace, long workspace_bytes, void* stream);
int hoisdf_decoder_layer_bwd(const float* tgt, const float* memory, const uint8_t* tgt_mask, const float* out,
                             const hoisdf_decoder_layer_weights* weights, const hoisdf_decoder_layer_desc* desc, const void* saved,
                             long saved_bytes, const float* g_out, const float* g_y, float* d_tgt, float* d_memory,
                             int accumulate_memory, float* d_query_pos, const hoisdf_decoder_layer_grads* grads, void* workspace,
                             long workspace_bytes, void* stream);

int hoisdf_vote_fwd(const float* off, const float* cls, const float* pts, float* joints, float* stats,
                    int L, int B, int P, int J, void* stream);
int hoisdf_vote_bwd(const float* off, const float* cls, const float* pts, const float* joints,
                    const float* stats, const float* djoints, float* doff, float* dcls, int L, int B,
                    int P, int J, void* stream);

int hoisdf_vote_loss_fwd(const float* off, const float* cls, const float* pts, const float* joint_gt_mm,
                         float radius, float* joints, float* stats, float* l3d_sum, float* bce_sum,
                         float* near_sum, int L, int B, int P, int J, void* stream);
int hoisdf_vote_loss_bwd(const float* off, const float* cls, const float* pts, const float* joint_gt_mm,
                         float radius, const float* joints, const float* stats, const float* djoints,
                         const float* dl3d_sum, const float* dbce_sum, float* doff, float* dcls, int L,
                         int B, int P, int J, void* stream);

#define HOISDF_MLP_MAX_LAYERS 4
typedef struct hoisdf_mlp {
  int n_layers, act_last;
  int dims[HOISDF_MLP_MAX_LAYERS + 1];
  const float* w[HOISDF_MLP_MAX_LAYERS];
  const float* b[HOISDF_MLP_MAX_LAYERS];
  const void* img[HOISDF_MLP_MAX_LAYERS];
  const void* img_t[HOISDF_MLP_MAX_LAYERS];
} hoisdf_mlp;
typedef struct hoisdf_mlp_grads {
  float* dw[HOISDF_MLP_MAX_LAYERS];
  float* db[HOISDF_MLP_MAX_LAYERS];
} hoisdf_mlp_grads;
long hoisdf_tokens_saved_bytes(const hoisdf_mlp* mlp, long n_rows, int gather_inside);
long hoisdf_tokens_workspace_bytes(const hoisdf_mlp* mlp, long n_rows, int backward_pass);
int hoisdf_tokens_fwd(const hoisdf_pyramid* pyr, const float* points, const float* center, const float* cam_intr, float scale,
                      int img_h, int img_w, const float* feat_in, const float* cam_in, const hoisdf_mlp* mlp, const float* pe,
                      const float* sdf, const float* beta_ptr, float* tok, float* fea_out, float* cam_out, int B, int P, int S,
                      int row0, int D, void* saved, long saved_bytes, void* workspace, long workspace_bytes, void* stream);
int hoisdf_tokens_bwd(const hoisdf_pyramid_grad* dpyr, const float* points, const float* center, const float* cam_intr,
                      float scale, int img_h, int img_w, const float* feat_in, const hoisdf_mlp* mlp, const float* sdf,
                      const float* beta_ptr, const float* dtok, const void* saved, long saved_bytes,
                      const hoisdf_mlp_grads* grads, float* dfeat, int accumulate_dfeat, float* dbeta, int B, int P, int S,
                      int row0, int D, void* workspace, long workspace_bytes, void* stream);
long hoisdf_heads_vote_saved_bytes(const hoisdf_mlp* vote, const hoisdf_mlp* cls, int L, int B, int P, int J);
long hoisdf_heads_vote_workspace_bytes(const hoisdf_mlp* vote, const hoisdf_mlp* cls, int L, int B, int P, int J,
                                       int backward_pass);
int hoisdf_heads_vote_fwd(const float* enc, const hoisdf_mlp* vote, const hoisdf_mlp* cls, const float* pts,
                          const float* joint_gt_mm, float radius, float* joints, float* l3d_sum, float* bce_sum,
                          float* near_sum, int L, int B, int P, int J, void* saved, long saved_bytes, void* workspace,
                          long workspace_bytes, void* stream);
int hoisdf_heads_vote_bwd(const float* enc, const hoisdf_mlp* vote, const hoisdf_mlp* cls, const float* pts,
                          const float* joint_gt_mm, float radius, const float* joints, const void* saved, long saved_bytes,
                          const float* djoints, const float* dl3d_sum, const float* dbce_sum,
                          const hoisdf_mlp_grads* vote_grads, const hoisdf_mlp_grads* cls_grads, float* denc, int L, int B,
                          int P, int J, void* workspace, long workspace_bytes, void* stream);

int hoisdf_point_loss_blocks(long n);
int hoisdf_point_loss_fwd(const float* pred, const float* target, long n, long rep, int C, long Bt, int kind,
                          float clamp, float pred_scale, float out_scale, float* partials, float* loss, void* stream);
// ... 144 lines not shown
```

Before: 452.9.

## Group key tiles per block in f16x2 attention backward and fuse delta into convert

The f16x2 attention backward kernel now loops over a group of key tiles per block and accumulates partial dQ in place, reading back the previous partial with nontemporal loads. The group size is chosen from the CU count so the grid still gives at least two blocks per CU. This shrinks the dQ partial workspace and the work of the reduce kernel. Separately, the delta (rowsum of O·dO) computation is fused into the dout convert kernel, removing one launch and one extra read of dout. The cost is less parallelism across key tiles and serialized read-modify-write traffic on the partial buffer.

Result: no change. 455.2 (median of 6 runs) (+0.5%).

```diff
diff --git a/hoisdf_amd/_lib.py b/hoisdf_amd/_lib.py
--- a/hoisdf_amd/_lib.py
+++ b/hoisdf_amd/_lib.py
@@ -232,7 +232,7 @@
     "hoisdf_encoder_infer": [_P, _P, _P, _P, _P, _P, _L, _P],
 }
 _RET = {"hoisdf_version": C.c_char_p, "hoisdf_last_error": C.c_char_p}
-_OTHER = {"hoisdf_set_deterministic": ([_I], None), "hoisdf_set_gemm_emu": ([_I], None), "hoisdf_get_gemm_emu": ([], C.c_int), "hoisdf_get_deterministic": ([], C.c_int),
+_OTHER = {"hoisdf_set_deterministic": ([_I], None), "hoisdf_set_gemm_emu": ([_I], None), "hoisdf_set_attention_bwd_kgroup": ([_I], None), "hoisdf_get_gemm_emu": ([], C.c_int), "hoisdf_get_deterministic": ([], C.c_int),
           "hoisdf_mano_dirs_image_floats": ([], C.c_long),
           "hoisdf_point_loss_blocks": ([_L], C.c_int),
           "hoisdf_bn_workspace_floats": ([_L, _I], C.c_long),
diff --git a/hoisdf_amd/csrc/attention_emu.h b/hoisdf_amd/csrc/attention_emu.h
--- a/hoisdf_amd/csrc/attention_emu.h
+++ b/hoisdf_amd/csrc/attention_emu.h
@@ -19,7 +19,10 @@
   const uint32_t *q_hm, *k_hm, *v_hm, *d_hm;
   float* dq_scale;
   uint32_t* mag;
+  int kgroup;
 };
+
+int emu_attn_kgroup(int B, int H, int Lk);
 
 __device__ __forceinline__ bool emu_block(int nx, int nbh, int& tile, int& bh) {
   const int L = blockIdx.x, slot = L >> 3;
diff --git a/hoisdf_amd/csrc/attention_emu.hip b/hoisdf_amd/csrc/attention_emu.hip
--- a/hoisdf_amd/csrc/attention_emu.hip
+++ b/hoisdf_amd/csrc/attention_emu.hip
@@ -69,7 +69,8 @@
                                                                float scale, __bf16* __restrict__ r0, __bf16* __restrict__ r1,
                                                                __bf16* __restrict__ r2, __bf16* __restrict__ t0,
                                                                __bf16* __restrict__ t1, __bf16* __restrict__ t2,
-                                                               const uint32_t* __restrict__ mag) {
+                                                               const uint32_t* __restrict__ mag, const float* __restrict__ o,
+                                                               int ldo, float* __restrict__ delta) {
   constexpr int TP = 72;
   __shared__ __attribute__((aligned(16))) __bf16 tile[3][64 * TP];
   const int tid = threadIdx.x;
@@ -81,10 +82,18 @@
   const bool valid = row < L;
   const float* sr = src + ((size_t)b * L + (valid ? row : 0)) * ld + head * D + dc;
   bf16x8 pa[2][3];
+  float dsum[4];
 #pragma unroll
   for (int i = 0; i < 2; ++i) {
     float4 u = valid ? *reinterpret_cast<const float4*>(sr + 8 * i) : make_float4(0.f, 0.f, 0.f, 0.f);
     float4 w = valid ? *reinterpret_cast<const float4*>(sr + 8 * i + 4) : make_float4(0.f, 0.f, 0.f, 0.f);
+    if (delta) {
+      const float* po = o + ((size_t)b * L + (valid ? row : 0)) * ldo + head * D + dc + 8 * i;
+      const float4 x = valid ? *reinterpret_cast<const float4*>(po) : make_float4(0.f, 0.f, 0.f, 0.f);
+      const float4 y = valid ? *reinterpret_cast<const float4*>(po + 4) : make_float4(0.f, 0.f, 0.f, 0.f);
+      dsum[2 * i] = x.x * u.x + x.y * u.y + x.z * u.z + x.w * u.w;
+      dsum[2 * i + 1] = y.x * w.x + y.y * w.y + y.z * w.z + y.w * w.w;
+    }
     u.x *= scale; u.y *= scale; u.z *= scale; u.w *= scale;
     w.x *= scale; w.y *= scale; w.z *= scale; w.w *= scale;
     if (F16) {
@@ -100,13 +109,21 @@
       pa[i][0] = p0; pa[i][1] = p1; pa[i][2] = p2;
     }
   }
+  if (delta) {
+#pragma unroll
+    for (int i = 0; i < 4; ++i) {
+      dsum[i] += __shfl_xor(dsum[i], 2, 4);
+      dsum[i] += __shfl_xor(dsum[i], 1, 4);
+    }
+    if ((tid & 3) == 0 && valid) delta[(size_t)bh * L + row] = (dsum[0] + dsum[2]) + (dsum[1] + dsum[3]);
+  }
   if (r0) {
-    const size_t o = ((size_t)bh * Lp + row) * D + dc;
+    const size_t ro = ((size_t)bh * Lp + row) * D + dc;
 #pragma unroll
     for (int i = 0; i < 2; ++i) {
-      *reinterpret_cast<bf16x8*>(r0 + o + 8 * i) = pa[i][0];
-      *reinterpret_cast<bf16x8*>(r1 + o + 8 * i) = pa[i][1];
-      if (!F16 && r2) *reinterpret_cast<bf16x8*>(r2 + o + 8 * i) = pa[i][2];
+      *reinterpret_cast<bf16x8*>(r0 + ro + 8 * i) = pa[i][0];
+      *reinterpret_cast<bf16x8*>(r1 + ro + 8 * i) = pa[i][1];
+      if (!F16 && r2) *reinterpret_cast<bf16x8*>(r2 + ro + 8 * i) = pa[i][2];
     }
   }
   if (t0) {
@@ -120,12 +137,12 @@
       }
     __syncthreads();
     const int d = tid >> 2, rc = (tid & 3) * 16;
-    const size_t o = ((size_t)bh * D + d) * Lp + kb * 64 + rc;
+    const size_t to = ((size_t)bh * D + d) * Lp + kb * 64 + rc;
 #pragma unroll
     for (int i = 0; i < 2; ++i) {
-      *reinterpret_cast<u32x4*>(t0 + o + 8 * i) = *reinterpret_cast<const u32x4*>(&tile[0][d * TP + rc + 8 * i]);
-      *reinterpret_cast<u32x4*>(t1 + o + 8 * i) = *reinterpret_cast<const u32x4*>(&tile[1][d * TP + rc + 8 * i]);
-      if (!F16 && t2) *reinterpret_cast<u32x4*>(t2 + o + 8 * i) = *reinterpret_cast<const u32x4*>(&tile[2][d * TP + rc + 8 * i]);
+      *reinterpret_cast<u32x4*>(t0 + to + 8 * i) = *reinterpret_cast<const u32x4*>(&tile[0][d * TP + rc + 8 * i]);
+      *reinterpret_cast<u32x4*>(t1 + to + 8 * i) = *reinterpret_cast<const u32x4*>(&tile[1][d * TP + rc + 8 * i]);
+      if (!F16 && t2) *reinterpret_cast<u32x4*>(t2 + to + 8 * i) = *reinterpret_cast<const u32x4*>(&tile[2][d * TP + rc + 8 * i]);
     }
   }
 }
@@ -432,22 +449,6 @@
 }
 #pragma pop_macro("MB")
 
-__global__ __launch_bounds__(256) void emu_attn_delta_kernel(const float* __restrict__ o, int ldo, const float* __restrict__ dout,
-                                                             int lddo, float* __restrict__ delta, int B, int H, int Lq) {
-  const long g = ((long)blockIdx.x * 256 + threadIdx.x) >> 4;
-  const int l16 = threadIdx.x & 15;
-  if (g >= (long)B * Lq * H) return;
-  const int head = (int)(g % H);
-  const long bq = g / H;
-  const int q = (int)(bq % Lq), b = (int)(bq / Lq);
-  const float4 x = *reinterpret_cast<const float4*>(o + ((size_t)b * Lq + q) * ldo + head * D + l16 * 4);
-  const float4 y = *reinterpret_cast<const float4*>(dout + ((size_t)b * Lq + q) * lddo + head * D + l16 * 4);
-  float s = x.x * y.x + x.y * y.y + x.z * y.z + x.w * y.w;
-#pragma unroll
-  for (int off = 8; off > 0; off >>= 1) s += __shfl_xor(s, off, 16);
-  if (l16 == 0) delta[((size_t)b * H + head) * Lq + q] = s;
-}
-
 __global__ __launch_bounds__(256) void emu_attn_dq_reduce_kernel(const float* __restrict__ part, int nkb, float* __restrict__ dq,
                                                                  int ldq, int B, int H, int Lq, uint32_t* __restrict__ mag,
                                                                  const float* __restrict__ scale) {
@@ -497,12 +498,13 @@
   for (int i = 0; i < 3; ++i) { p.t[i] = trn ? w : nullptr; if (trn) w += n; }
   return p;
 }
-int convert(const float* src, int ld, int L, int Lp, int B, int H, float scale, const Planes& p, hipStream_t st, const uint32_t* mag = nullptr) {
+int convert(const float* src, int ld, int L, int Lp, int B, int H, float scale, const Planes& p, hipStream_t st, const uint32_t* mag = nullptr,
+            const float* o = nullptr, int ldo = 0, float* delta = nullptr) {
   const long nblk = (long)B * H * (Lp / 64);
   if (mag) hipLaunchKernelGGL(emu_attn_convert_kernel<true>, dim3((unsigned)nblk), dim3(256), 0, st, src, ld, L, Lp, B, H, scale, p.r[0], p.r[1],
-                              p.r[2], p.t[0], p.t[1], p.t[2], mag);
+                              p.r[2], p.t[0], p.t[1], p.t[2], mag, o, ldo, delta);
   else hipLaunchKernelGGL(emu_attn_convert_kernel<false>, dim3((unsigned)nblk), dim3(256), 0, st, src, ld, L, Lp, B, H, scale, p.r[0], p.r[1],
-                          p.r[2], p.t[0], p.t[1], p.t[2], mag);
+                          p.r[2], p.t[0], p.t[1], p.t[2], mag, o, ldo, delta);
   return check_launch("attention_emu_convert");
 }
 int check_emu(const void* q, const void* k, const void* v, int ldq, int ldk, int ldv, int B, int H, int Lq, int Lk, int kv_len,
@@ -646,11 +648,35 @@
   return fwd_over_planes(o, ldo, lse, B, H, Lq, Lk, kv_len, drop_p, seed, workspace, keep, as_stream(stream), o_mag);
 }
 
+namespace {
+int g_kgroup = 0;
+int device_cus() {
+  static int cus[64];
+  int dev = 0, n = 0;
+  if (hipGetDevice(&dev) != hipSuccess || dev < 0 || dev >= 64) { (void)hipGetLastError(); return 0; }
+  if (cus[dev] == 0) {
+    if (hipDeviceGetAttribute(&n, hipDeviceAttributeMultiprocessorCount, dev) != hipSuccess) { (void)hipGetLastError(); return 0; }
+    cus[dev] = n;
+  }
+  return cus[dev];
+}
+}
+extern "C" void hoisdf_set_attention_bwd_kgroup(int g) { g_kgroup = g > 0 ? g : 0; }
+int hoisdf::emu_attn::emu_attn_kgroup(int B, int H, int Lk) {
+  if (g_kgroup > 0) return g_kgroup;
+  const long cus = device_cus(), nkb = cdiv(Lk, 128);
+  if (cus > 0)
+    for (int g = 8; g > 1; g >>= 1)
+      if ((long)B * H * cdiv(nkb, (long)g) >= 2 * cus) return g;
+  return 1;
+}
+
 extern "C" long hoisdf_attention_bwd_emu_workspace(int B, int H, int Lq, int Lk, int kept) {
   if (B <= 0 || H <= 0 || Lq <= 0 || Lk <= 0) return 0;
   const size_t q = plane_elems(B, H, pad128(Lq)), k = plane_elems(B, H, pad128(Lk));
-  size_t bytes = 3 * q * sizeof(__bf16) + (size_t)cdiv(Lk, 128) * B * H * Lq * 64 * sizeof(float);
-  if (!kept) bytes += (3 * q + 6 * k) * sizeof(__bf16);
+  const int parts = (kept & 2) ? cdiv(cdiv(Lk, 128), emu_attn::emu_attn_kgroup(B, H, Lk)) : cdiv(Lk, 128);
+  size_t bytes = 3 * q * sizeof(__bf16) + (size_t)parts * B * H * Lq * 64 * sizeof(float);
+  if (!(kept & 1)) bytes += (3 * q + 6 * k) * sizeof(__bf16);
   return (long)bytes;
 }
 
@@ -686,15 +712,16 @@
                      (((uintptr_t)o | (uintptr_t)dout | (uintptr_t)dq | (uintptr_t)dk | (uintptr_t)dv | (uintptr_t)workspace |
                        (uintptr_t)fwd_workspace) & 15) == 0,
                  HOISDF_ERR_INVALID, "attention_bwd_emu: bad leading dims / alignment");
-  const long need = hoisdf_attention_bwd_emu_workspace(B, H, Lq, Lk, fwd_workspace ? 1 : 0);
+  const long need = hoisdf_attention_bwd_emu_workspace(B, H, Lq, Lk, (fwd_workspace ? 1 : 0) | (h2 ? 2 : 0));
   HOISDF_REQUIRE(workspace_bytes >= need, HOISDF_ERR_WORKSPACE, "attention_bwd_emu: workspace %ld < %ld bytes", workspace_bytes, need);
   const int Lqp = (int)pad128(Lq), Lkp = (int)pad128(Lk);
   hipStream_t st = as_stream(stream);
   const size_t nq = plane_elems(B, H, Lqp), nk = plane_elems(B, H, Lkp);
+  const int kgroup = h2 ? emu_attn::emu_attn_kgroup(B, H, Lk) : 1;
   __bf16* w = reinterpret_cast<__bf16*>(workspace);
   const Planes pd = carve(w, nq, true, false);
   float* part = reinterpret_cast<float*>(w);
-  w += (size_t)cdiv(Lk, 128) * B * H * Lq * 64 * 2;
+  w += (size_t)cdiv(cdiv(Lk, 128), kgroup) * B * H * Lq * 64 * 2;
   Planes pq, pk, pv;
   if (fwd_workspace) {
     __bf16* f = reinterpret_cast<__bf16*>(const_cast<void*>(fwd_workspace));
@@ -705,23 +732,20 @@
     if (int rc = convert(k, ldk, Lk, Lkp, B, H, 1.f, pk, st, k_hm)) return rc;
     if (int rc = convert(v, ldv, Lk, Lkp, B, H, 1.f, pv, st, v_hm)) return rc;
   }
-  if (int rc = convert(dout, lddo, Lq, Lqp, B, H, 1.f, pd, st, do_hm)) return rc;
-  const long ng = (long)B * Lq * H;
-  hipLaunchKernelGGL(emu_attn_delta_kernel, dim3((unsigned)((ng * 16 + 255) / 256)), dim3(256), 0, st, o, ldo, dout, lddo, delta, B, H, Lq);
-  if (int rc = check_launch("attention_emu_delta")) return rc;
+  if (int rc = convert(dout, lddo, Lq, Lqp, B, H, 1.f, pd, st, do_hm, o, ldo, delta)) return rc;
   EmuAttn a{};
   for (int i = 0; i < 3; ++i) {
     a.q[i] = pq.r[i]; a.k[i] = pk.r[i]; a.v[i] = pv.r[i]; a.d[i] = pd.r[i];
   }
   a.lse_in = lse; a.delta = delta; a.dq_part = part; a.dk = dk; a.dv = dv; a.ldk = ldk; a.ldv = ldv; a.mag = g_mag;
   a.B = B; a.H = H; a.Lq = Lq; a.Lk = Lk; a.Lqp = Lqp; a.Lkp = Lkp; a.kv_len = kv_len;
-  a.drop_p = drop_p; a.inv_keep = 1.f / (1.f - drop_p); a.thresh = drop_threshold(drop_p); a.seed = seed;
+  a.drop_p = drop_p; a.inv_keep = 1.f / (1.f - drop_p); a.thresh = drop_threshold(drop_p); a.seed = seed; a.kgroup = kgroup;
   if (h2) {
     a.q_hm = q_hm; a.k_hm = k_hm; a.v_hm = v_hm; a.d_hm = do_hm;
     a.dq_scale = reinterpret_cast<float*>(pd.r[2]);
     if (int rc = attention_bwd4h_emu_launch(a, st)) return rc;
     const long n4h = (long)B * H * Lq * 16;
-    hipLaunchKernelGGL(emu_attn_dq_reduce_kernel, dim3((unsigned)((n4h + 255) / 256)), dim3(256), 0, st, part, cdiv(kv_len, 128), dq, ldq,
+    hipLaunchKernelGGL(emu_attn_dq_reduce_kernel, dim3((unsigned)((n4h + 255) / 256)), dim3(256), 0, st, part, cdiv(cdiv(kv_len, 128), kgroup), dq, ldq,
                        B, H, Lq, g_mag, (const float*)a.dq_scale);
     return check_launch("attention_bwd_emu dq reduce");
   }
diff --git a/hoisdf_amd/csrc/attention_emu_bwd4h.hip b/hoisdf_amd/csrc/attention_emu_bwd4h.hip
--- a/hoisdf_amd/csrc/attention_emu_bwd4h.hip
+++ b/hoisdf_amd/csrc/attention_emu_bwd4h.hip
@@ -50,13 +50,10 @@
   float* const stats = reinterpret_cast<float*>(reinterpret_cast<char*>(lds) + ST0_BYTES);
   const int tid = threadIdx.x, lane = tid & 63, wave = tid >> 6;
   const int c = lane & 31, h = lane >> 5, jq = lane & 15, b1 = (jq >> 3) & 1;
-  int ktile, bh;
+  int grp, bh;
   const int nkb = (a.Lk + 127) / 128;
-  if (!emu_block(nkb, a.B * a.H, ktile, bh)) return;
+  if (!emu_block((nkb + a.kgroup - 1) / a.kgroup, a.B * a.H, grp, bh)) return;
   const int b = bh / a.H, head = bh - b * a.H;
-  const int key = ktile * 128 + wave * 32 + c;
-  const bool kvalid = key < a.kv_len;
-  const int nq = ktile * 128 < a.kv_len ? (a.Lq + 31) / 32 : 0;
   const int dhalf = wave & 1, khalf = wave >> 1;
   f16_saturate_on();
   const int hw_ = head * a.B + b;
@@ -68,8 +65,15 @@
   const float k2a = mag_scale(ad_) * 0x1p-18f, k2b = mag_scale(av_) * 0x1p-18f;
   const float dk_scale = (LN2 * 0x1p23f * id) * (iv * iq);
   const float dv_scale = 0x1p-13f * id;
-  if (ktile == 0 && tid == 0 && a.dq_scale) a.dq_scale[bh] = (0.125f * 0x1p23f * id) * (ik * iv);
-
+  if (grp == 0 && tid == 0 && a.dq_scale) a.dq_scale[bh] = (0.125f * 0x1p23f * id) * (ik * iv);
+
+  float* const part = a.dq_part + ((size_t)grp * a.B * a.H + bh) * a.Lq * D;
+  const int kt0 = grp * a.kgroup, kt1 = min(kt0 + a.kgroup, nkb);
+  for (int ktile = kt0; ktile < kt1; ++ktile) {
+  const bool kfirst = ktile == kt0;
+  const int key = ktile * 128 + wave * 32 + c;
+  const bool kvalid = key < a.kv_len;
+  const int nq = ktile * 128 < a.kv_len ? (a.Lq + 31) / 32 : 0;
   bf16x8 kf[4][2], vf[4][2], ktf[4][2];
   {
     const size_t ro = ((size_t)bh * a.Lkp + key) * D;
@@ -146,7 +150,6 @@
 #define B4_STOREP(i_, BUF_) do { *reinterpret_cast<u32x4*>(lds + (BUF_) + (i_) * QD_PLANE + st_o) = sg[i_]; } while (0)
 #define B4_STORES(SB_) do { if (tid < 64) stats[(SB_) + tid] = rstat; } while (0)
 
-  float* const part = a.dq_part + ((size_t)ktile * a.B * a.H + bh) * a.Lq * D;
   if (nq > 0) {
 #pragma unroll
     for (int pt = 0; pt < 2; ++pt) {
@@ -177,7 +180,7 @@
     if (DROP) hb = drop_rowkey(a.seed, (uint32_t)(bh * a.Lq + 4 * h)) + (uint32_t)(key >> 1) * 0x9E3779B9U + (kodd ? 16u * 0x85EBCA77U : 0u);
 
     f32x16 s, dp, dq;
-    f32x4 xo0[2], xo1[2];
+    f32x4 xo0[2], xo1[2], xp[2];
     bf16x8 fr[2][2], ft[4][3];
     u32x4 pwv[2][2], gwv[3][2];
     f32x2 pe[8], pd[8], xx[8], ff[8];
@@ -214,7 +217,17 @@
 #define XOS(i_)                                                                                                        \
   do {                                                                                                                 \
     const int q_ = (t - 2) * 32 + 8 * wave + 4 * (i_) + (lane >> 4);                                                   \
-    if (t >= 2 && q_ < a.Lq) *reinterpret_cast<f32x4*>(part + (unsigned)(q_ * D + 4 * (lane & 15))) = xo0[i_] + xo1[i_]; \
+    if (t >= 2 && q_ < a.Lq) {                                                                                         \
+      f32x4 r_ = xo0[i_] + xo1[i_];                                                                                    \
+      if (!kfirst) r_ = xp[i_] + r_;                                                                                   \
+      *reinterpret_cast<f32x4*>(part + (unsigned)(q_ * D + 4 * (lane & 15))) = r_;                                     \
+    }                                                                                                                  \
+  } while (0)
+#define XPL(i_)                                                                                                        \
+  do {                                                                                                                 \
+    const int q_ = (t - 1) * 32 + 8 * wave + 4 * (i_) + (lane >> 4);                                                   \
+    if (!kfirst && t >= 1 && q_ < a.Lq)                                                                                \
+      xp[i_] = __builtin_nontemporal_load(reinterpret_cast<const f32x4*>(part + (unsigned)(q_ * D + 4 * (lane & 15)))); \
   } while (0)
 #define CRC(r_) (((r_) & 3) + 8 * ((r_) >> 2))
 #define HA(q_) do { if (DROP) { _Pragma("unroll") for (int i_ = 0; i_ < 4; ++i_) { const int e_ = 4 * (q_) + i_; uint32_t x_ = hbn + (uint32_t)CRC(e_) * 0x85EBCA77U; x_ ^= x_ >> 15; hy[e_] = x_; PIN2(hy[e_]); } } } while (0)
@@ -374,9 +387,11 @@
     gmax = max(gmax, (uint32_t)__shfl_xor((int)gmax, 32, 64));
     if (h == 0 && key < a.Lk) atomicMax(a.mag + (size_t)b * a.Lk + key, gmax);
   }
+  }
 }
 
 int attention_bwd4h_emu_launch(const EmuAttn& a, hipStream_t st) {
+  if (a.kgroup < 1) { set_error("attention_bwd_emu (f16x2): kgroup = %d", a.kgroup); return HOISDF_ERR_INVALID; }
   static bool attr_set = false;
   if (!attr_set) {
     const void* ks[2] = {reinterpret_cast<const void*>(emu_attn_bwd4h_kernel<true>), reinterpret_cast<const void*>(emu_attn_bwd4h_kernel<false>)};
@@ -387,7 +402,7 @@
       }
     attr_set = true;
   }
-  const dim3 grid(cdiv(a.Lk, 128) * 8 * cdiv(a.B * a.H, 8));
+  const dim3 grid(cdiv(cdiv(a.Lk, 128), a.kgroup) * 8 * cdiv(a.B * a.H, 8));
   if (a.drop_p > 0.f) hipLaunchKernelGGL((emu_attn_bwd4h_kernel<true>), grid, dim3(256), B4H_LDS_BYTES, st, a);
   else hipLaunchKernelGGL((emu_attn_bwd4h_kernel<false>), grid, dim3(256), B4H_LDS_BYTES, st, a);
   return check_launch("attention_bwd_emu (bwd4h)");
diff --git a/hoisdf_amd/csrc/attn_bwd4h_phase.inc b/hoisdf_amd/csrc/attn_bwd4h_phase.inc
--- a/hoisdf_amd/csrc/attn_bwd4h_phase.inc
+++ b/hoisdf_amd/csrc/attn_bwd4h_phase.inc
@@ -26,11 +26,11 @@
     MFMA_SP(dp, fr[1][0], vf[3][0]); ft[3][2] = FRT(2, 3); DL(0); SB();                       \
     MFMA_Q0(dq, ktf[0][1], ft[0][1]); PC(0); DL(1); DL(2); DL(3); SB();                       \
     MFMA_Q(dq, ktf[0][0], ft[0][2]); XOS(0); SB();                                            \
-    MFMA_Q(dq, ktf[0][1], ft[0][0]); fr[0][0] = FRA(2 + 0, 0, 0); SB();                       \
+    MFMA_Q(dq, ktf[0][1], ft[0][0]); fr[0][0] = FRA(2 + 0, 0, 0); XPL(0); SB();               \
     MFMA_Q(dq, ktf[0][0], ft[0][1]); fr[0][1] = FRA(2 + 1, 0, 0); SB();                       \
     MFMA_Q(dq, ktf[1][1], ft[1][1]); XOS(1); SB();                                            \
     MFMA_Q(dq, ktf[1][0], ft[1][2]); PC(1); SB();                                             \
-    MFMA_Q(dq, ktf[1][1], ft[1][0]); PD(0); SB();                                             \
+    MFMA_Q(dq, ktf[1][1], ft[1][0]); PD(0); XPL(1); SB();                                     \
     MFMA_Q(dq, ktf[1][0], ft[1][1]); PD(1); QA(0); SB();                                      \
     MFMA_Q(dq, ktf[2][1], ft[2][1]); PA(2); SB();                                             \
     MFMA_Q(dq, ktf[2][0], ft[2][2]); PA(3); SB();                                             \
diff --git a/hoisdf_amd/csrc/layers.hip b/hoisdf_amd/csrc/layers.hip
--- a/hoisdf_amd/csrc/layers.hip
+++ b/hoisdf_amd/csrc/layers.hip
@@ -225,7 +225,7 @@
   const bool amag = mags && g.att_bwd_emu && g.full;
   auto attn_bwd = [&](const float* q, int ldq, const float* k, const float* v, int ldkv, float* dq, float* dk, float* dv) {
     if (g.att_bwd_emu) {
-      const long ab = hoisdf_attention_bwd_emu_workspace(g.B, g.H, g.nq, g.S, s.planes ? 1 : 0);
+      const long ab = hoisdf_attention_bwd_emu_workspace(g.B, g.H, g.nq, g.S, (s.planes ? 1 : 0) | (g.att_h2 ? 2 : 0));
       void* aw = ws.take(ab);
       if (dry || !c.ok()) return;
       if (!aw) { c.rc = HOISDF_ERR_WORKSPACE; return; }
diff --git a/hoisdf_amd/ops.py b/hoisdf_amd/ops.py
--- a/hoisdf_amd/ops.py
+++ b/hoisdf_amd/ops.py
@@ -894,7 +894,7 @@
     Lk = k.shape[1]
     assert dq.stride(1) == q.stride(1) and dk.stride(1) == k.stride(1) and dv.stride(1) == v.stride(1)
     kept = _EMU_PLANES.pop(_planes_key(q, k, v, H, kv_len), None)
-    nbytes = lib().hoisdf_attention_bwd_emu_workspace(B, H, Lq, Lk, int(kept is not None))
+    nbytes = lib().hoisdf_attention_bwd_emu_workspace(B, H, Lq, Lk, int(kept is not None) | (2 if heads is not None else 0))
     ws = torch.empty(nbytes, device=q.device, dtype=torch.uint8)
     delta = torch.empty(B, H, Lq, device=q.device, dtype=torch.float32)
     if kept is not None:
diff --git a/include/hoisdf.h b/include/hoisdf.h
--- a/include/hoisdf.h
+++ b/include/hoisdf.h
@@ -217,6 +217,7 @@
                                  long workspace_bytes, int keep, const uint32_t* q_mag, const uint32_t* k_mag, const uint32_t* v_mag,
                                  uint32_t* o_mag, void* stream);
 long hoisdf_attention_bwd_emu_workspace(int B, int H, int Lq, int Lk, int kept);
+void hoisdf_set_attention_bwd_kgroup(int g);
 int hoisdf_attention_bwd_emu(const float* q, int ldq, const float* k, int ldk, const float* v, int ldv, const float* o, int ldo,
                              const float* dout, int lddo, const float* lse, float* delta, float* dq, float* dk, float* dv, int B,
                              int H, int Lq, int Lk, int kv_len, float drop_p, uint64_t seed, const void* fwd_workspace,
```
